# AOADMM-DataFusionFramework/Matlab-Code

Hardware: AMD Instinct MI355X
Metric: AO-ADMM outer iters/sec (+ mode-1 MTTKRP GFLOP/s), 2000^3 rank-20 CP (higher is better)
Workload: dtype f32

## Files before the change

### matlab-code_amd/csrc/contract.h

```cpp
#pragma once
#include "common.h"

namespace aoadmm {

struct DenseTensor {
  int prec = AOADMM_PREC_F64;
  int nd = 0;
  int64_t dims[8] = {0};
  int64_t pad0 = 0;
  DevBuf data;
  int64_t elems_padded() const {
    int64_t n = pad0;
    for (int i = 1; i < nd; ++i) n *= dims[i];
    return n;
  }
  size_t elem_size() const { return prec == AOADMM_PREC_F32 ? 4 : 8; }
};

struct ContractPlan {
  int64_t nbatch, batch_stride, M, ld, C;
  int R;
  int tprec = AOADMM_PREC_F64;
  int nchunk;
  bool lead = false;
  bool on_xp = false;
  bool on_xq = false;
  bool on_xc = false;
  int64_t trows() const { return nbatch * M; }
  size_t t_bytes() const { return (size_t)nchunk * trows() * R * (tprec == AOADMM_PREC_F32 ? 4 : 8); }
  size_t frag_bytes(int prec) const;
  double algorithmic_bytes(int prec) const {
    return (double)nbatch * M * C * (prec == AOADMM_PREC_F32 ? 4.0 : 8.0) + (double)t_bytes();
  }
  double flops() const { return 2.0 * nbatch * M * C * R; }
};

ContractPlan make_plan(int64_t nbatch, int64_t batch_stride, int64_t M, int64_t ld, int64_t C, int R,
                       int prec);

ContractPlan make_lead_plan(int64_t M, int64_t ld, int64_t C, int R);

void launch_contract(const void* X, int prec, const ContractPlan& pl, const double* F, int64_t ldF,
                     void* frag_ws, void* T, hipStream_t s, hipEvent_t ev0 = nullptr,
                     hipEvent_t ev1 = nullptr);

size_t reduce_factor_scratch_bytes(int64_t rows, int R);
struct SysBuild;
bool launch_reduce_inner(const void* T, int tprec, int nchunk, int64_t trows, int64_t A, int64_t Apad,
                         int64_t B, int R, const double* Fa, int64_t ldFa, double scale,
                         double* out, int64_t ldOut, double* ft_scratch, hipStream_t s,
                         const double* FaT = nullptr,
                         int rowmajor_out = 0,
                         const SysBuild* sys = nullptr);
size_t reduce_outer_scratch_bytes(int64_t A, int64_t B, int R);
bool launch_reduce_outer(const void* T, int tprec, int nchunk, int64_t trows, int64_t A, int64_t Apad,
                         int64_t B, int R, const double* Fb, int64_t ldFb, double scale,
                         double* out, int64_t ldOut, double* scratch, double* ft_scratch, hipStream_t s,
                         const double* FbT = nullptr, int rowmajor_out = 0, const SysBuild* sys = nullptr);
void launch_t_to_colmajor(const void* T, int tprec, int nchunk, int64_t trows, int64_t A, int R, double scale,
                          double* out, int64_t ldOut, hipStream_t s);

constexpr int64_t kSmallMttkrpElems = (int64_t)1 << 19;
struct SmallMttkrp {
  const void* X;
  int64_t sn, sa, sb;
  int Na, Nb, R;
  const double *Fa, *Fb;
  int64_t lda, ldb;
  double scale;
  double* out;
  int64_t ldOut;
};
bool small_mttkrp_ok(int64_t elems, int nd, const int64_t* dims, int R);
bool small_mttkrp(const SmallMttkrp& a, int prec, int64_t rows, hipStream_t s, const SysBuild* sys = nullptr);

}
```

### matlab-code_amd/csrc/contract.hip

```cpp
#include "contract.h"
#include "device_utils.h"
#include "small_dev.h"

#include <algorithm>
#include <cstdlib>

namespace aoadmm {

typedef float f32x4 __attribute__((ext_vector_type(4)));
typedef double f64x2 __attribute__((ext_vector_type(2)));
typedef double f64x4 __attribute__((ext_vector_type(4)));

static constexpr int kTileRows = 128;
static constexpr int kGroup = 8;

struct KArgs {
  const void* X;
  const void* frag;
  void* T;
  int64_t tiles_per_batch, ntiles, batch_stride, M, ld, C, Cg, trows;
  int groups_per_chunk, R;
  int flush_every;
};

typedef float f32x2 __attribute__((ext_vector_type(2)));

__global__ void pack_frag16_f32(const double* __restrict__ F, int64_t ldF, int64_t C, int R, int NT, int EX,
                                int64_t Cg, float* __restrict__ frag) {
  const int64_t idx = (int64_t)blockIdx.x * blockDim.x + threadIdx.x;
  const int64_t nmain = (int64_t)NT * Cg * 128;
  if (idx < nmain) {
    const int kk = idx & 1;
    const int lane = (idx >> 1) & 63;
    const int64_t g = (idx >> 7) % Cg;
    const int nt = (int)((idx >> 7) / Cg);
    const int64_t c = 8 * g + 4 * kk + (lane >> 4);
    const int r = 16 * nt + (lane & 15);
    frag[idx] = (c < C && r < R) ? (float)F[c + ldF * r] : 0.f;
  } else if (EX && idx < nmain + Cg * 32) {
    const int64_t j = idx - nmain;
    const int e = j & 3, q = (j >> 2) & 3, kk = (j >> 4) & 1;
    const int64_t g = j >> 5;
    const int64_t c = 8 * g + 4 * kk + q;
    const int r = 16 * NT + e;
    frag[idx] = (c < C && r < R) ? (float)F[c + ldF * r] : 0.f;
  }
}

__device__ __forceinline__ float quarter_sum4(float a, float b, float c, float d) {
  const auto ab = __builtin_amdgcn_permlane16_swap(__float_as_uint(a), __float_as_uint(b), false, false);
  const auto cd = __builtin_amdgcn_permlane16_swap(__float_as_uint(c), __float_as_uint(d), false, false);
  const float s_ab = __uint_as_float(ab[0]) + __uint_as_float(ab[1]);
  const float s_cd = __uint_as_float(cd[0]) + __uint_as_float(cd[1]);
  const auto x = __builtin_amdgcn_permlane32_swap(__float_as_uint(s_ab), __float_as_uint(s_cd), false, false);
  return __uint_as_float(x[0]) + __uint_as_float(x[1]);
}

constexpr int kFlushEvery = 3;
template <int NT, bool EX, bool L2 = false>
__global__ __launch_bounds__(256, NT <= 2 ? 2 : 1) void contract16_f32(KArgs a) {
  static_assert(!L2 || NT == 1, "two-level accumulation exists for one 16-column tile (R <= 20)");
  const int lane = threadIdx.x & 63;
  const int64_t wt = (int64_t)blockIdx.x * 4 + (threadIdx.x >> 6);
  if (wt >= a.ntiles) return;
  const int chunk = blockIdx.y;
  const int64_t b = wt / a.tiles_per_batch;
  const int64_t m0 = (wt - b * a.tiles_per_batch) * kTileRows;
  const int r16 = lane & 15, q = lane >> 4;
  int64_t row0 = m0 + 4 * r16, row1 = m0 + 64 + 4 * r16;
  if (row0 >= a.M) row0 = m0;
  if (row1 >= a.M) row1 = m0;
  const int64_t g0 = (int64_t)chunk * a.groups_per_chunk;
  int64_t g1 = g0 + a.groups_per_chunk;
  if (g1 > a.Cg) g1 = a.Cg;
  const int64_t gfull = (a.C / kGroup < g1) ? a.C / kGroup : g1;
  const float* X = reinterpret_cast<const float*>(a.X) + b * a.batch_stride;
  const float* xp0 = X + row0 + (kGroup * g0 + q) * a.ld;
  const float* xp1 = X + row1 + (kGroup * g0 + q) * a.ld;
  const int64_t ld4 = 4 * a.ld;
  const f32x2* fp = reinterpret_cast<const f32x2*>(a.frag) + g0 * 64 + lane;
  const int64_t fnt = a.Cg * 64;
  const f32x4* fe = reinterpret_cast<const f32x4*>(reinterpret_cast<const f32x2*>(a.frag) + (int64_t)NT * a.Cg * 64) + g0 * 8 + q;

  f32x4 acc[NT][2][4];
  f32x2 accE[2][4][2];
#define AO_PKFMA_LO(ACC, X2, E2) asm("v_pk_fma_f32 %0, %1, %2, %0 op_sel:[0,0,0] op_sel_hi:[0,1,1]" : "+v"(ACC) : "v"(X2), "v"(E2));
#define AO_PKFMA_HI(ACC, X2, E2) asm("v_pk_fma_f32 %0, %1, %2, %0 op_sel:[1,0,0] op_sel_hi:[1,1,1]" : "+v"(ACC) : "v"(X2), "v"(E2));
#pragma unroll
  for (int h = 0; h < 2; ++h)
#pragma unroll
    for (int v = 0; v < 4; ++v) {
      accE[h][v][0] = f32x2{0.f, 0.f};
      accE[h][v][1] = f32x2{0.f, 0.f};
#pragma unroll
      for (int nt = 0; nt < NT; ++nt) acc[nt][h][v] = f32x4{0.f, 0.f, 0.f, 0.f};
    }

  extern __shared__ __attribute__((aligned(16))) float t_lds[];
  double* l2 = reinterpret_cast<double*>(t_lds) + (threadIdx.x >> 6) * 2048 + lane;
  double accE2[2][4];
  if (L2) {
#pragma unroll
    for (int k = 0; k < 32; ++k) l2[k * 64] = 0.0;
#pragma unroll
    for (int h = 0; h < 2; ++h)
#pragma unroll
      for (int v = 0; v < 4; ++v) accE2[h][v] = 0.0;
  }
#define AO_FLUSH()                                                                                   \
  {                                                                                                  \
    _Pragma("unroll") for (int h = 0; h < 2; ++h) {                                                  \
      _Pragma("unroll") for (int vb = 0; vb < 4; vb += 2) {                                          \
        _Pragma("unroll") for (int v = vb; v < vb + 2; ++v)                                          \
          _Pragma("unroll") for (int i = 0; i < 4; ++i) {                                            \
            l2[((h * 4 + v) * 4 + i) * 64] += (double)acc[0][h][v][i];                               \
            acc[0][h][v][i] = 0.f;                                                                   \
          }                                                                                          \
        __builtin_amdgcn_sched_barrier(0);                                                           \
      }                                                                                              \
    }                                                                                                \
    if (EX) {       \
      _Pragma("unroll") for (int h = 0; h < 2; ++h)                                                  \
        _Pragma("unroll") for (int v = 0; v < 4; ++v) {                                              \
          accE2[h][v] += (double)quarter_sum4(accE[h][v][0][0], accE[h][v][0][1], accE[h][v][1][0], accE[h][v][1][1]); \
          accE[h][v][0] = f32x2{0.f, 0.f};                                                           \
          accE[h][v][1] = f32x2{0.f, 0.f};                                                           \
        }                                                                                            \
    }                                                                                                \
  }
  f32x4 x0[4], x1[4], x2[4], e0[2], e1[2], e2[2];
  f32x2 f0[NT], f1[NT], f2[NT];
  const int64_t ng = gfull > g0 ? gfull - g0 : 0;
  const int64_t gstep = kGroup * a.ld;
#define AO_LOAD1(XS, GI, S)                                                                          \
  XS[S] = __builtin_nontemporal_load(reinterpret_cast<const f32x4*>((((S) & 1) ? xp1 : xp0) + (GI) * gstep + ((S) >> 1) * ld4));
#define AO_LOADF(FS, ES, GI)                                                                         \
  {                                                                                                  \
    _Pragma("unroll") for (int nt = 0; nt < NT; ++nt) FS[nt] = fp[(GI) * 64 + nt * fnt];            \
    if (EX) { ES[0] = fe[(GI) * 8]; ES[1] = fe[(GI) * 8 + 4]; }                                      \
  }
#define AO_LOAD_STAGE(XS, FS, ES, GI)                                                                \
  { AO_LOAD1(XS, GI, 0) AO_LOAD1(XS, GI, 1) AO_LOAD1(XS, GI, 2) AO_LOAD1(XS, GI, 3) AO_LOADF(FS, ES, GI) }
#define AO_FMA_S(XS, FS, ES, S)                                                                      \
  {                                                                                                  \
    _Pragma("unroll") for (int v = 0; v < 4; ++v) {                                                  \
      _Pragma("unroll") for (int nt = 0; nt < NT; ++nt)                                              \
        acc[nt][(S) & 1][v] = __builtin_amdgcn_mfma_f32_16x16x4f32(XS[S][v], FS[nt][(S) >> 1], acc[nt][(S) & 1][v], 0, 0, 0); \
    }                                                                                                \
    if (EX) {       \
      const f32x2 xlo_ = __builtin_shufflevector(XS[S], XS[S], 0, 1), xhi_ = __builtin_shufflevector(XS[S], XS[S], 2, 3); \
      const f32x2 ea_ = __builtin_shufflevector(ES[(S) >> 1], ES[(S) >> 1], 0, 1);                   \
      const f32x2 eb_ = __builtin_shufflevector(ES[(S) >> 1], ES[(S) >> 1], 2, 3);                   \
      AO_PKFMA_LO(accE[(S) & 1][0][0], xlo_, ea_) AO_PKFMA_LO(accE[(S) & 1][0][1], xlo_, eb_)        \
      AO_PKFMA_HI(accE[(S) & 1][1][0], xlo_, ea_) AO_PKFMA_HI(accE[(S) & 1][1][1], xlo_, eb_)        \
      AO_PKFMA_LO(accE[(S) & 1][2][0], xhi_, ea_) AO_PKFMA_LO(accE[(S) & 1][2][1], xhi_, eb_)        \
      AO_PKFMA_HI(accE[(S) & 1][3][0], xhi_, ea_) AO_PKFMA_HI(accE[(S) & 1][3][1], xhi_, eb_)        \
    }                                                                                                \
  }
#define AO_COMPUTE_STAGE(XS, FS, ES) { AO_FMA_S(XS, FS, ES, 0) AO_FMA_S(XS, FS, ES, 1) AO_FMA_S(XS, FS, ES, 2) AO_FMA_S(XS, FS, ES, 3) }
#define AO_MIX_STAGE(XC, FC, EC, XL, FL, EL, GI)                                                     \
  {                                                                                                  \
    AO_FMA_S(XC, FC, EC, 0) AO_LOAD1(XL, GI, 0) __builtin_amdgcn_sched_barrier(0);                   \
    AO_FMA_S(XC, FC, EC, 1) AO_LOAD1(XL, GI, 1) __builtin_amdgcn_sched_barrier(0);                   \
    AO_FMA_S(XC, FC, EC, 2) AO_LOAD1(XL, GI, 2) __builtin_amdgcn_sched_barrier(0);                   \
    AO_FMA_S(XC, FC, EC, 3) AO_LOAD1(XL, GI, 3) AO_LOADF(FL, EL, GI) __builtin_amdgcn_sched_barrier(0); \
  }
  if (ng > 0) AO_LOAD_STAGE(x0, f0, e0, 0)
  if (ng > 1) AO_LOAD_STAGE(x1, f1, e1, 1)
  int64_t g = 0;
  int since_flush = 0;
  for (; g + 5 <= ng; g += 3) {
    AO_MIX_STAGE(x0, f0, e0, x2, f2, e2, g + 2)
    AO_MIX_STAGE(x1, f1, e1, x0, f0, e0, g + 3)
    AO_MIX_STAGE(x2, f2, e2, x1, f1, e1, g + 4)
    if (L2 && ++since_flush == a.flush_every) {
      since_flush = 0;
      AO_FLUSH()
    }
  }
  for (; g + 3 <= ng; g += 3) {
    if (g + 2 < ng) AO_LOAD_STAGE(x2, f2, e2, g + 2)
    AO_COMPUTE_STAGE(x0, f0, e0)
    if (g + 3 < ng) AO_LOAD_STAGE(x0, f0, e0, g + 3)
    AO_COMPUTE_STAGE(x1, f1, e1)
    if (g + 4 < ng) AO_LOAD_STAGE(x1, f1, e1, g + 4)
    AO_COMPUTE_STAGE(x2, f2, e2)
  }
  if (g < ng) AO_COMPUTE_STAGE(x0, f0, e0)
  if (g + 1 < ng) AO_COMPUTE_STAGE(x1, f1, e1)
  g = gfull > g0 ? gfull : g0;
  if (g < g1) {
#pragma unroll
    for (int s = 0; s < 4; ++s) {
      int64_t c = kGroup * g + 4 * (s >> 1) + q;
      if (c >= a.C) c = a.C - 1;
      x0[s] = *reinterpret_cast<const f32x4*>(X + ((s & 1) ? row1 : row0) + c * a.ld);
    }
    {
      const f32x2* fpt = reinterpret_cast<const f32x2*>(a.frag) + g * 64 + lane;
#pragma unroll
      for (int nt = 0; nt < NT; ++nt) f0[nt] = fpt[nt * fnt];
      if (EX) {
        const f32x4* fet = reinterpret_cast<const f32x4*>(reinterpret_cast<const f32x2*>(a.frag) + (int64_t)NT * a.Cg * 64) + g * 8 + q;
        e0[0] = fet[0]; e0[1] = fet[4];
      }
    }
    AO_COMPUTE_STAGE(x0, f0, e0)
  }
  if (L2) AO_FLUSH()
#undef AO_FLUSH
#undef AO_PKFMA_LO
#undef AO_PKFMA_HI
#undef AO_LOAD1
#undef AO_LOADF
#undef AO_LOAD_STAGE
#undef AO_FMA_S
#undef AO_COMPUTE_STAGE
#undef AO_MIX_STAGE
  float* tl = L2 ? t_lds + (threadIdx.x >> 6) * 4096 : t_lds + (threadIdx.x >> 6) * (kTileRows * a.R);
  if (L2) {
    double d2[32];
#pragma unroll
    for (int k = 0; k < 32; ++k) d2[k] = l2[k * 64];
    __builtin_amdgcn_sched_barrier(0);
#pragma unroll
    for (int h = 0; h < 2; ++h)
#pragma unroll
      for (int v = 0; v < 4; ++v)
#pragma unroll
        for (int i = 0; i < 4; ++i) acc[0][h][v][i] = (float)d2[(h * 4 + v) * 4 + i];
  }
#pragma unroll
  for (int nt = 0; nt < NT; ++nt) {
    const int r = 16 * nt + r16;
    if (r < a.R) {
#pragma unroll
      for (int h = 0; h < 2; ++h)
#pragma unroll
        for (int v = 0; v < 4; ++v)
#pragma unroll
          for (int i = 0; i < 4; ++i) tl[(64 * h + 4 * (4 * q + i) + v) * a.R + r] = acc[nt][h][v][i];
    }
  }
  if (EX) {
#pragma unroll
    for (int h = 0; h < 2; ++h)
#pragma unroll
      for (int v = 0; v < 4; ++v)
#pragma unroll
        for (int e = 0; e < 4; ++e) {
          if (L2) continue;
          float t = accE[h][v][e >> 1][e & 1];
          t += __shfl_xor(t, 16);
          t += __shfl_xor(t, 32);
          accE[h][v][e >> 1][e & 1] = t;
        }
    const int ne = a.R - 16 * NT;
    if (L2) {
      if (q < ne) {
#pragma unroll
        for (int h = 0; h < 2; ++h)
#pragma unroll
          for (int v = 0; v < 4; ++v) tl[(64 * h + 4 * r16 + v) * a.R + 16 * NT + q] = (float)accE2[h][v];
      }
    } else if (q == 0) {
#pragma unroll
      for (int h = 0; h < 2; ++h)
#pragma unroll
        for (int v = 0; v < 4; ++v)
#pragma unroll
          for (int e = 0; e < 4; ++e)
            if (e < ne) tl[(64 * h + 4 * r16 + v) * a.R + 16 * NT + e] = accE[h][v][e >> 1][e & 1];
    }
  }
  {
    const int64_t rows_here = (a.M - m0 < kTileRows) ? a.M - m0 : kTileRows;
    const int n16 = (int)(rows_here * a.R / 4);
    f32x4* dst = reinterpret_cast<f32x4*>(reinterpret_cast<float*>(a.T) + ((int64_t)chunk * a.trows + b * a.M + m0) * a.R);
    const f32x4* src = reinterpret_cast<const f32x4*>(tl);
    for (int c = lane; c < n16; c += 64) __builtin_nontemporal_store(src[c], dst + c);
  }
}

static constexpr int kLeadRows = 128;
static constexpr int kLeadKC = 64;
static constexpr int kLeadStride = 68;

struct LArgs {
  const float* X;
  const float* frag;
  float* T;
  int64_t M, ld, C, Cg;
  int chunks_per_slice;
  int R;
};

__global__ void pack_frag_lead16_f32(const double* __restrict__ F, int64_t ldF, int64_t C, int R, int NT,
                                     int64_t Cg16, float* __restrict__ frag) {
  const int64_t idx = (int64_t)blockIdx.x * blockDim.x + threadIdx.x;
  const int64_t nmain = (int64_t)NT * Cg16 * 256;
  if (idx < nmain) {
    const int t = idx & 3;
    const int lane = (idx >> 2) & 63;
    const int64_t g = (idx >> 8) % Cg16;
    const int nt = (int)((idx >> 8) / Cg16);
    const int64_t c = 16 * g + 4 * (lane >> 4) + t;
    const int r = 16 * nt + (lane & 15);
    frag[idx] = (c < C && r < R) ? (float)F[c + ldF * r] : 0.f;
  }
}

template <int NT>
__global__ __launch_bounds__(256, NT <= 2 ? 2 : 1) void contract_lead16_f32(LArgs a) {
  extern __shared__ __attribute__((aligned(16))) float lds[];
  const int tid = threadIdx.x, lane = tid & 63, w = tid >> 6;
  const int64_t m0 = (int64_t)blockIdx.x * kLeadRows;
  const int slice = blockIdx.y;
  const int64_t nchunks_total = (a.C + kLeadKC - 1) / kLeadKC;
  const int64_t c0 = (int64_t)slice * a.chunks_per_slice;
  int64_t c1 = c0 + a.chunks_per_slice;
  if (c1 > nchunks_total) c1 = nchunks_total;
  const int64_t Cg16 = (a.C + 15) / 16;
  const int srow = tid >> 4, scol = 4 * (tid & 15);
  const unsigned mlast = (unsigned)((a.M - 1 - m0 < kLeadRows - 1) ? (a.M - 1 - m0) : (kLeadRows - 1));
  const float* xblk = a.X + m0 * a.ld;
  const int64_t last4 = a.ld - 4;
  f32x4 acc[NT][8];
#pragma unroll
  for (int tl = 0; tl < 8; ++tl)
#pragma unroll
    for (int nt = 0; nt < NT; ++nt) acc[nt][tl] = f32x4{0.f, 0.f, 0.f, 0.f};
  const int r16 = lane & 15, q4 = lane >> 4;
  const f32x4* fbase = reinterpret_cast<const f32x4*>(a.frag) + lane;
  const int64_t fnt = (Cg16 + 1) * 64;
  f32x4 sA[8], sB[8];
  f32x4 fA[NT], fB[NT];
#define AO_LEAD_LOAD1(ST, CH, Q)                                                                     \
  {                                                                                                  \
    int64_t i_ = (CH) * kLeadKC + scol;                                                              \
    if (i_ > last4) i_ = last4;                                                                      \
    unsigned mq_ = srow + 16 * (Q);                                                                  \
    if (mq_ > mlast) mq_ = mlast;                                                                    \
    unsigned ldo_ = (unsigned)a.ld;                                                                  \
    asm volatile("" : "+s"(ldo_));                                                                   \
    ST[Q] = __builtin_nontemporal_load(reinterpret_cast<const f32x4*>(xblk + (uint64_t)mq_ * ldo_ + i_)); \
  }
#define AO_LEAD_LOAD(ST, CH) { _Pragma("unroll") for (int q_ = 0; q_ < 8; ++q_) AO_LEAD_LOAD1(ST, CH, q_) }
#define AO_LEAD_WRITE(ST, BUF)                                                                       \
  {                                                                                                  \
    float* base_ = lds + (BUF) * (kLeadRows * kLeadStride);                                          \
    _Pragma("unroll") for (int q_ = 0; q_ < 8; ++q_)                                                 \
      *reinterpret_cast<f32x4*>(base_ + (srow + 16 * q_) * kLeadStride + scol) = ST[q_];             \
  }
#define AO_LEAD_FRAG(FV, CH)                                                                         \
  {                                                                                                  \
    int64_t gg = (CH) * (kLeadKC / 16) + w;                                                          \
    if (gg > Cg16) gg = Cg16;                                           \
    _Pragma("unroll") for (int nt = 0; nt < NT; ++nt) FV[nt] = fbase[nt * fnt + gg * 64];            \
  }
#define AO_LEAD_TILE(XV, TL, FV)                                                                     \
  {                                                                                                  \
    _Pragma("unroll") for (int t = 0; t < 4; ++t)                                                    \
      _Pragma("unroll") for (int nt = 0; nt < NT; ++nt)                                              \
        acc[nt][TL] = __builtin_amdgcn_mfma_f32_16x16x4f32(XV[t], FV[nt][t], acc[nt][TL], 0, 0, 0);  \
  }
#define AO_LEAD_COMPUTE(BUF, CH, FV, FVN, NF, ST, CHN, PF)                                           \
  {                                                                                                  \
    const float* xs_ = lds + (BUF) * (kLeadRows * kLeadStride) + r16 * kLeadStride + 16 * w + 4 * q4; \
    if (NF) AO_LEAD_FRAG(FVN, (CH) + 1)                                                              \
    _Pragma("unroll") for (int hb = 0; hb < 2; ++hb) {                                               \
      f32x4 xv_[4];                                                                                  \
      _Pragma("unroll") for (int j_ = 0; j_ < 4; ++j_)            \
        xv_[j_] = *reinterpret_cast<const f32x4*>(xs_ + 16 * (4 * hb + j_) * kLeadStride);           \
      __builtin_amdgcn_sched_barrier(0);                                                             \
      _Pragma("unroll") for (int j_ = 0; j_ < 4; ++j_) {                                             \
        AO_LEAD_TILE(xv_[j_], 4 * hb + j_, FV)                                                       \
        if (PF) AO_LEAD_LOAD1(ST, CHN, 4 * hb + j_)                                                  \
        __builtin_amdgcn_sched_barrier(0);                                                           \
      }                                                                                              \
    }                                                                                                \
  }
  const int64_t n = c1 > c0 ? c1 - c0 : 0;
  if (n > 0) {
    AO_LEAD_LOAD(sA, c0)
    AO_LEAD_FRAG(fA, c0)
    AO_LEAD_WRITE(sA, 0)
  }
  if (n > 1) AO_LEAD_LOAD(sA, c0 + 1)
  if (n > 2) AO_LEAD_LOAD(sB, c0 + 2)
  __syncthreads();
#pragma nounroll
  for (int64_t k = 0; k < n; k += 2) {
    if (k + 1 < n) AO_LEAD_WRITE(sA, 1)
    if (k + 3 < n) AO_LEAD_COMPUTE(0, c0 + k, fA, fB, true, sA, c0 + k + 3, true)
    else if (k + 1 < n) AO_LEAD_COMPUTE(0, c0 + k, fA, fB, true, sA, c0, false)
    else AO_LEAD_COMPUTE(0, c0 + k, fA, fB, false, sA, c0, false)
    __syncthreads();
    if (k + 1 >= n) break;
    if (k + 2 < n) AO_LEAD_WRITE(sB, 0)
    if (k + 4 < n) AO_LEAD_COMPUTE(1, c0 + k + 1, fB, fA, true, sB, c0 + k + 4, true)
    else if (k + 2 < n) AO_LEAD_COMPUTE(1, c0 + k + 1, fB, fA, true, sB, c0, false)
    else AO_LEAD_COMPUTE(1, c0 + k + 1, fB, fA, false, sB, c0, false)
    __syncthreads();
  }
#undef AO_LEAD_LOAD1
#undef AO_LEAD_LOAD
#undef AO_LEAD_WRITE
#undef AO_LEAD_FRAG
#undef AO_LEAD_TILE
#undef AO_LEAD_COMPUTE
  __syncthreads();
  constexpr int kEpiStride = 17;
  float* Tc = a.T + (int64_t)slice * a.M * a.R + m0 * a.R;
  const int64_t rows_here = (a.M - m0 < kLeadRows) ? (a.M - m0) : kLeadRows;
#pragma unroll
  for (int nt = 0; nt < NT; ++nt) {
    float* reg = lds + w * (kLeadRows * kEpiStride);
#pragma unroll
    for (int tl = 0; tl < 8; ++tl)
#pragma unroll
      for (int i = 0; i < 4; ++i) reg[(16 * tl + 4 * q4 + i) * kEpiStride + r16] = acc[nt][tl][i];
    __syncthreads();
    int ncol = a.R - 16 * nt;
    if (ncol > 16) ncol = 16;
    const int total = (int)rows_here * ncol;
    for (int e = tid; e < total; e += 256) {
      const int row = e / ncol, col = e - row * ncol;
      const float* p = lds + row * kEpiStride + col;
      const float v = (p[0] + p[kLeadRows * kEpiStride]) + (p[2 * kLeadRows * kEpiStride] + p[3 * kLeadRows * kEpiStride]);
      Tc[(int64_t)row * a.R + 16 * nt + col] = v;
    }
    __syncthreads();
  }
// ... 116 lines not shown
    for (; g + 2 <= ng; g += 2) {
      AO_LOAD_STAGE(x1, f1, e1, g + 1)
      AO_COMPUTE_STAGE(x0, f0, e0)
      if (g + 2 < ng) AO_LOAD_STAGE(x0, f0, e0, g + 2)
      AO_COMPUTE_STAGE(x1, f1, e1)
    }
    if (g < ng) AO_COMPUTE_STAGE(x0, f0, e0)
  }
  g = gfull > g0 ? gfull : g0;
  if (g < g1) {
#pragma unroll
    for (int s = 0; s < 4; ++s) {
      int64_t c = kGroup * g + 4 * (s >> 1) + q;
      if (c >= a.C) c = a.C - 1;
      x0[s] = *reinterpret_cast<const f64x2*>(X + ((s & 1) ? row1 : row0) + c * a.ld);
    }
    {
      const f64x2* fpt = reinterpret_cast<const f64x2*>(a.frag) + g * 64 + lane;
#pragma unroll
      for (int nt = 0; nt < NT; ++nt) f0[nt] = fpt[nt * fnt];
      if (EX) {
        const f64x4* fet = reinterpret_cast<const f64x4*>(reinterpret_cast<const f64x2*>(a.frag) + (int64_t)NT * a.Cg * 64) + g * 8 + q;
        e0[0] = fet[0]; e0[1] = fet[4];
      }
    }
    AO_COMPUTE_STAGE(x0, f0, e0)
  }
#undef AO_LOAD1
#undef AO_LOADF
#undef AO_LOAD_STAGE
#undef AO_FMA_S
#undef AO_COMPUTE_STAGE
#undef AO_MIX_STAGE
  extern __shared__ __attribute__((aligned(16))) double t_lds64[];
  double* tl = t_lds64 + (threadIdx.x >> 6) * (kTileRows64 * a.R);
#pragma unroll
  for (int nt = 0; nt < NT; ++nt) {
    const int r = 16 * nt + r2;
    if (r < a.R) {
#pragma unroll
      for (int j = 0; j < 2; ++j)
#pragma unroll
        for (int v = 0; v < 2; ++v)
#pragma unroll
          for (int i = 0; i < 4; ++i) tl[(32 * j + 2 * (q + 4 * i) + v) * a.R + r] = acc[nt][j][v][i];
    }
  }
  if (EX) {
#pragma unroll
    for (int j = 0; j < 2; ++j)
#pragma unroll
      for (int v = 0; v < 2; ++v)
#pragma unroll
        for (int c = 0; c < 4; ++c) {
          double t = accE[j][v][c];
          t += __shfl_xor(t, 16);
          t += __shfl_xor(t, 32);
          accE[j][v][c] = t;
        }
    if (q == 0) {
      const int ne = a.R - 16 * NT;
#pragma unroll
      for (int j = 0; j < 2; ++j)
#pragma unroll
        for (int v = 0; v < 2; ++v)
#pragma unroll
          for (int c = 0; c < 4; ++c)
            if (c < ne) tl[(32 * j + 2 * r2 + v) * a.R + 16 * NT + c] = accE[j][v][c];
    }
  }
  {
    const int64_t rows_here = (a.M - m0 < kTileRows64) ? a.M - m0 : kTileRows64;
    const int n16 = (int)(rows_here * a.R / 2);
    f64x2* dst = reinterpret_cast<f64x2*>(reinterpret_cast<double*>(a.T) + ((int64_t)chunk * a.trows + b * a.M + m0) * a.R);
    const f64x2* src = reinterpret_cast<const f64x2*>(tl);
    for (int c = lane; c < n16; c += 64) __builtin_nontemporal_store(src[c], dst + c);
  }
}

static int nt_of(int R, int prec) {
  const int w = prec == AOADMM_PREC_F32 ? 32 : 16;
  return (R + w - 1) / w;
}
static int tile_rows(int prec) { return prec == AOADMM_PREC_F32 ? kTileRows : kTileRows64; }

size_t ContractPlan::frag_bytes(int prec) const {
  const int64_t Cg = cdiv(C, kGroup);
  return (size_t)(nt_of(R, prec) * 1024 + 1152) * Cg + 8192;
}

ContractPlan make_plan(int64_t nbatch, int64_t batch_stride, int64_t M, int64_t ld, int64_t C, int R,
                       int prec) {
  ContractPlan p;
  p.tprec = prec;
  p.nbatch = nbatch; p.batch_stride = batch_stride; p.M = M; p.ld = ld; p.C = C; p.R = R;
  const int64_t Cg = cdiv(C, kGroup);
  const int64_t ntiles = nbatch * cdiv(M, tile_rows(prec));
  int64_t nchunk = 1;
  if (prec == AOADMM_PREC_F32) nchunk = cdiv(Cg, 256);
  if (ntiles < 2048) {
    int64_t want = cdiv(2048, ntiles);
    int64_t maxc = Cg / 16 > 0 ? Cg / 16 : 1;
    if (want > maxc) want = maxc;
    if (want > nchunk) nchunk = want;
  }
  if (nchunk > 65535) nchunk = 65535;
  p.nchunk = (int)nchunk;
  return p;
}

ContractPlan make_lead_plan(int64_t M, int64_t ld, int64_t C, int R) {
  ContractPlan p;
  p.tprec = AOADMM_PREC_F32;
  p.nbatch = 1; p.batch_stride = 0; p.M = M; p.ld = ld; p.C = C; p.R = R;
  p.lead = true;
  const int64_t nch = cdiv(C, kLeadKC);
  p.nchunk = (int)cdiv(nch, 2048 / kLeadKC);
  return p;
}

static void launch_contract_lead(const void* X, const ContractPlan& pl, const double* F, int64_t ldF, void* frag_ws,
                                 void* T, hipStream_t s, hipEvent_t ev0, hipEvent_t ev1) {
  const int64_t Cg = cdiv(pl.C, kGroup);
  AO_REQUIRE(pl.ld % 4 == 0 && pl.ld >= 4, "f32 layout must be padded to 4");
  LArgs a;
  a.X = (const float*)X; a.frag = (const float*)frag_ws; a.T = (float*)T;
  a.M = pl.M; a.ld = pl.ld; a.C = pl.C; a.Cg = Cg; a.R = pl.R;
  a.chunks_per_slice = (int)cdiv(cdiv(pl.C, kLeadKC), pl.nchunk);
  const int64_t nblk = cdiv(pl.M, kLeadRows);
  AO_REQUIRE(nblk < (int64_t)2147483647, "tensor too large for one launch");
  dim3 grid((unsigned)nblk, (unsigned)pl.nchunk);
  const size_t sh = (size_t)2 * kLeadRows * kLeadStride * sizeof(float);
  const int nt16 = (pl.R + 15) / 16;
  const int64_t Cg16 = cdiv(pl.C, 16) + 1;
  const int64_t total = (int64_t)nt16 * Cg16 * 256;
  pack_frag_lead16_f32<<<(unsigned)cdiv(total, 256), 256, 0, s>>>(F, ldF, pl.C, pl.R, nt16, Cg16, (float*)frag_ws);
  AO_KERNEL_CHECK();
#define AO_SET(K) ensure_dynamic_lds(reinterpret_cast<const void*>(K), (int)sh);
  if (nt16 == 1) AO_SET(contract_lead16_f32<1>)
  else if (nt16 == 2) AO_SET(contract_lead16_f32<2>)
  else if (nt16 == 3) AO_SET(contract_lead16_f32<3>)
  else if (nt16 == 4) AO_SET(contract_lead16_f32<4>)
#undef AO_SET
  if (ev0) AO_HIP(hipEventRecord(ev0, s));
  if (nt16 == 1) contract_lead16_f32<1><<<grid, 256, sh, s>>>(a);
  else if (nt16 == 2) contract_lead16_f32<2><<<grid, 256, sh, s>>>(a);
  else if (nt16 == 3) contract_lead16_f32<3><<<grid, 256, sh, s>>>(a);
  else if (nt16 == 4) contract_lead16_f32<4><<<grid, 256, sh, s>>>(a);
  else throw Error(AOADMM_ERR_UNSUPPORTED, "rank > 64 not supported");
  if (ev1) AO_HIP(hipEventRecord(ev1, s));
  AO_KERNEL_CHECK();
}

void launch_contract(const void* X, int prec, const ContractPlan& pl, const double* F, int64_t ldF,
                     void* frag_ws, void* T, hipStream_t s, hipEvent_t ev0, hipEvent_t ev1) {
  AO_REQUIRE(pl.tprec == prec, "contraction plan and tensor precision disagree");
  AO_REQUIRE(pl.R >= 1 && pl.R <= kMaxRank, "rank %d outside [1,%d]", pl.R, kMaxRank);
  if (pl.lead) {
    AO_REQUIRE(prec == AOADMM_PREC_F32, "leading-mode contraction exists for fp32 tensors only");
    launch_contract_lead(X, pl, F, ldF, frag_ws, T, s, ev0, ev1);
    return;
  }
  const int64_t Cg = cdiv(pl.C, kGroup);
  KArgs a;
  a.X = X; a.frag = frag_ws; a.T = T;
  a.tiles_per_batch = cdiv(pl.M, tile_rows(prec));
  a.ntiles = pl.nbatch * a.tiles_per_batch;
  a.batch_stride = pl.batch_stride; a.M = pl.M; a.ld = pl.ld; a.C = pl.C; a.Cg = Cg;
  a.trows = pl.trows();
  a.groups_per_chunk = (int)cdiv(Cg, pl.nchunk);
  a.R = pl.R;
  AO_REQUIRE(a.ntiles > 0 && pl.C > 0, "empty contraction");
  dim3 grid((unsigned)cdiv(a.ntiles, 4), (unsigned)pl.nchunk);
  AO_REQUIRE(cdiv(a.ntiles, 4) < (int64_t)2147483647, "tensor too large for one launch");
  if (prec == AOADMM_PREC_F32) {
    AO_REQUIRE(pl.ld % 4 == 0 && pl.M % 4 == 0 && pl.batch_stride % 4 == 0, "f32 layout must be padded to 4");
    const int rem = pl.R % 16;
    const bool ex = pl.R > 16 && rem >= 1 && rem <= 4;
    const int nt16 = ex ? pl.R / 16 : (pl.R + 15) / 16;
    const int64_t total = (int64_t)nt16 * Cg * 128 + (ex ? Cg * 32 : 0);
    pack_frag16_f32<<<(unsigned)cdiv(total, 256), 256, 0, s>>>(F, ldF, pl.C, pl.R, nt16, ex ? 1 : 0, Cg, (float*)frag_ws);
    AO_KERNEL_CHECK();
    size_t tsh = (size_t)4 * kTileRows * pl.R * sizeof(float);
    a.flush_every = kFlushEvery;
    if (nt16 == 1) tsh = (size_t)4 * 16384;
#define AO_GO(K) { if (tsh > 65536) ensure_dynamic_lds(reinterpret_cast<const void*>(K), (int)tsh); if (ev0) AO_HIP(hipEventRecord(ev0, s)); K<<<grid, 256, tsh, s>>>(a); }
    if (nt16 == 1 && !ex) AO_GO((contract16_f32<1, false, true>))
    else if (nt16 == 1) AO_GO((contract16_f32<1, true, true>))
    else if (nt16 == 2 && !ex) AO_GO((contract16_f32<2, false>))
    else if (nt16 == 2) AO_GO((contract16_f32<2, true>))
    else if (nt16 == 3 && !ex) AO_GO((contract16_f32<3, false>))
    else if (nt16 == 3) AO_GO((contract16_f32<3, true>))
    else if (nt16 == 4) AO_GO((contract16_f32<4, false>))
    else throw Error(AOADMM_ERR_UNSUPPORTED, "rank > 64 not supported");
#undef AO_GO
  } else {
    AO_REQUIRE(pl.ld % 2 == 0 && pl.M % 2 == 0 && pl.batch_stride % 2 == 0, "f64 layout must be padded to 2");
    const int rem = pl.R % 16;
    const bool ex = pl.R > 16 && rem >= 1 && rem <= 4;
    const int nt16 = ex ? pl.R / 16 : (pl.R + 15) / 16;
    const int64_t total = (int64_t)nt16 * Cg * 128 + (ex ? Cg * 32 : 0);
    pack_frag_f64<<<(unsigned)cdiv(total, 256), 256, 0, s>>>(F, ldF, pl.C, pl.R, nt16, ex ? 1 : 0, Cg, (double*)frag_ws);
    AO_KERNEL_CHECK();
    const size_t tsh = (size_t)4 * kTileRows64 * pl.R * sizeof(double);
#define AO_GO(K) { if (tsh > 65536) ensure_dynamic_lds(reinterpret_cast<const void*>(K), (int)tsh); if (ev0) AO_HIP(hipEventRecord(ev0, s)); K<<<grid, 256, tsh, s>>>(a); }
    if (nt16 == 1 && !ex) AO_GO((contract_f64<1, false>))
    else if (nt16 == 1) AO_GO((contract_f64<1, true>))
    else if (nt16 == 2 && !ex) AO_GO((contract_f64<2, false>))
    else if (nt16 == 2) AO_GO((contract_f64<2, true>))
    else if (nt16 == 3 && !ex) AO_GO((contract_f64<3, false>))
    else if (nt16 == 3) AO_GO((contract_f64<3, true>))
    else if (nt16 == 4) AO_GO((contract_f64<4, false>))
    else throw Error(AOADMM_ERR_UNSUPPORTED, "rank > 64 not supported");
#undef AO_GO
  }
  if (ev1) AO_HIP(hipEventRecord(ev1, s));
  AO_KERNEL_CHECK();
}

__global__ void factor_rowmajor_k(const double* __restrict__ F, int64_t ldF, int64_t rows, int R,
                                  double* __restrict__ Ft) {
  const int64_t idx = (int64_t)blockIdx.x * blockDim.x + threadIdx.x;
  if (idx >= rows * R) return;
  const int r = (int)(idx / rows);
  const int64_t a = idx - (int64_t)r * rows;
  Ft[a * R + r] = F[a + ldF * r];
}
static void factor_rowmajor(const double* F, int64_t ldF, int64_t rows, int R, double* Ft, hipStream_t s) {
  factor_rowmajor_k<<<(unsigned)cdiv(rows * R, 256), 256, 0, s>>>(F, ldF, rows, R, Ft);
  AO_KERNEL_CHECK();
}

template <typename TT, int VEC> struct TVec;
template <> struct TVec<float, 4> { typedef float type __attribute__((ext_vector_type(4))); };
template <> struct TVec<float, 1> { typedef float type; };
template <> struct TVec<double, 2> { typedef double type __attribute__((ext_vector_type(2))); };
template <> struct TVec<double, 1> { typedef double type; };
template <typename TT, int VEC>
__device__ __forceinline__ void fma_vec(double (&acc)[VEC], const TT* __restrict__ tp, const double* __restrict__ fp) {
  typedef typename TVec<TT, VEC>::type V;
  const V tv = __builtin_nontemporal_load(reinterpret_cast<const V*>(tp));
  if constexpr (VEC == 1) {
    acc[0] += (double)tv * fp[0];
  } else {
#pragma unroll
    for (int v = 0; v < VEC; ++v) acc[v] += (double)tv[v] * fp[v];
  }
}

template <typename TT, int VEC>
struct RVec {
  typename TVec<TT, VEC>::type t;
  double f[VEC];
  __device__ __forceinline__ void load(const TT* __restrict__ tp, const double* __restrict__ fp) {
    t = __builtin_nontemporal_load(reinterpret_cast<const typename TVec<TT, VEC>::type*>(tp));
#pragma unroll
    for (int v = 0; v < VEC; ++v) f[v] = fp[v];
  }
  __device__ __forceinline__ void fma(double (&acc)[VEC]) const {
    if constexpr (VEC == 1) {
      acc[0] += (double)t * f[0];
    } else {
#pragma unroll
      for (int v = 0; v < VEC; ++v) acc[v] += (double)t[v] * f[v];
    }
  }
};

template <typename TT, int VEC>
__global__ void reduce_inner_k(const TT* __restrict__ T, int nchunk, int64_t trows, int64_t A, int64_t Apad, int R,
                               const double* __restrict__ FaT, double scale, double* __restrict__ out,
                               int64_t ldOut, int rowmajor, int has_sys, SysBuild sys) {
  extern __shared__ double sh[];
  if (has_sys && blockIdx.x == 0) { sys_build_rider(sys); return; }
  const int64_t b = (int64_t)blockIdx.x - has_sys;
  const int t = threadIdx.x;
  const int64_t n = A * R, step = (int64_t)blockDim.x * VEC;
  double s0[VEC], s1[VEC], s2[VEC], s3[VEC];
#pragma unroll
  for (int v = 0; v < VEC; ++v) { s0[v] = 0; s1[v] = 0; s2[v] = 0; s3[v] = 0; }
  for (int ch = 0; ch < nchunk; ++ch) {
    const TT* Tb = T + ((int64_t)ch * trows + Apad * b) * R;
    int64_t e = (int64_t)t * VEC;
    for (; e + 3 * step < n; e += 4 * step) {
      RVec<TT, VEC> q0, q1, q2, q3;
      q0.load(Tb + e, FaT + e);
      q1.load(Tb + e + step, FaT + e + step);
      q2.load(Tb + e + 2 * step, FaT + e + 2 * step);
      q3.load(Tb + e + 3 * step, FaT + e + 3 * step);
      __builtin_amdgcn_sched_barrier(0);
      q0.fma(s0); q1.fma(s1); q2.fma(s2); q3.fma(s3);
    }
    for (; e < n; e += step) fma_vec<TT, VEC>(s0, Tb + e, FaT + e);
  }
#pragma unroll
  for (int v = 0; v < VEC; ++v) sh[t * VEC + v] = (s0[v] + s1[v]) + (s2[v] + s3[v]);
  __syncthreads();
  if (t < R) {
    const int nA = blockDim.x * VEC / R;
    double tot = 0.0;
    for (int i = 0; i < nA; ++i) tot += sh[i * R + t];
    if (rowmajor) out[b * R + t] = scale * tot;
    else out[b + ldOut * t] = scale * tot;
  }
}

template <typename TT, int VEC>
__global__ void reduce_inner2_k(const TT* __restrict__ T, int nchunk, int64_t trows, int64_t A, int64_t Apad, int64_t B,
                                int R, const double* __restrict__ FaT, double scale, double* __restrict__ out,
                                int64_t ldOut, int rowmajor, int has_sys, SysBuild sys) {
  extern __shared__ double sh[];
  if (has_sys && blockIdx.x == 0) { sys_build_rider(sys); return; }
  const int64_t b0 = 2 * ((int64_t)blockIdx.x - has_sys);
  const bool two = b0 + 1 < B;
  const int64_t b1 = two ? b0 + 1 : b0;
  const int t = threadIdx.x;
  const int64_t n = A * R, step = (int64_t)blockDim.x * VEC;
  double a0[VEC], a1[VEC], c0[VEC], c1[VEC];
#pragma unroll
  for (int v = 0; v < VEC; ++v) { a0[v] = 0; a1[v] = 0; c0[v] = 0; c1[v] = 0; }
  for (int ch = 0; ch < nchunk; ++ch) {
    const TT* Ta = T + ((int64_t)ch * trows + Apad * b0) * R;
    const TT* Tc = T + ((int64_t)ch * trows + Apad * b1) * R;
    int64_t e = (int64_t)t * VEC;
    for (; e + step < n; e += 2 * step) {
      RVec<TT, VEC> q0, q1, p0, p1;
      q0.load(Ta + e, FaT + e);
      q1.load(Ta + e + step, FaT + e + step);
      p0.t = __builtin_nontemporal_load(reinterpret_cast<const typename TVec<TT, VEC>::type*>(Tc + e));
      p1.t = __builtin_nontemporal_load(reinterpret_cast<const typename TVec<TT, VEC>::type*>(Tc + e + step));
      __builtin_amdgcn_sched_barrier(0);
#pragma unroll
      for (int v = 0; v < VEC; ++v) { p0.f[v] = q0.f[v]; p1.f[v] = q1.f[v]; }
      q0.fma(a0); q1.fma(a1); p0.fma(c0); p1.fma(c1);
    }
    for (; e < n; e += step) {
      RVec<TT, VEC> q0, p0;
      q0.load(Ta + e, FaT + e);
      p0.t = __builtin_nontemporal_load(reinterpret_cast<const typename TVec<TT, VEC>::type*>(Tc + e));
#pragma unroll
      for (int v = 0; v < VEC; ++v) p0.f[v] = q0.f[v];
      q0.fma(a0); p0.fma(c0);
    }
  }
  const int nt = blockDim.x * VEC;
#pragma unroll
  for (int v = 0; v < VEC; ++v) { sh[t * VEC + v] = a0[v] + a1[v]; sh[nt + t * VEC + v] = c0[v] + c1[v]; }
  __syncthreads();
  if (t < 2 * R) {
    const int which = t / R, r = t % R;
    if (which == 0 || two) {
      const int nA = nt / R;
      double tot = 0.0;
      for (int i = 0; i < nA; ++i) tot += sh[which * nt + i * R + r];
      const int64_t b = which ? b1 : b0;
      if (rowmajor) out[b * R + r] = scale * tot;
      else out[b + ldOut * r] = scale * tot;
    }
  }
}

size_t reduce_factor_scratch_bytes(int64_t rows, int R) { return (size_t)rows * R * sizeof(double); }

template <typename TT, int VEC>
static void launch_inner_t(const void* T, int nchunk, int64_t trows, int64_t A, int64_t Apad, int64_t B, int R,
                           const double* FaT, double scale, double* out, int64_t ldOut, hipStream_t s, int rowmajor,
                           const SysBuild* sys) {
  const int hs = sys ? 1 : 0;
  const SysBuild sb = sys ? *sys : SysBuild();
  const int rq = R / VEC;
  int threads = 256 / rq * rq;
  if (threads < rq) threads = rq;
  if (threads * VEC < R) threads = (R + VEC - 1) / VEC;
  if (B >= 1024 && 2 * R <= threads) {
    reduce_inner2_k<TT, VEC><<<(unsigned)((B + 1) / 2 + hs), threads, (size_t)2 * threads * VEC * sizeof(double), s>>>(
        (const TT*)T, nchunk, trows, A, Apad, B, R, FaT, scale, out, ldOut, rowmajor, hs, sb);
    return;
  }
  reduce_inner_k<TT, VEC><<<(unsigned)(B + hs), threads, (size_t)threads * VEC * sizeof(double), s>>>(
      (const TT*)T, nchunk, trows, A, Apad, R, FaT, scale, out, ldOut, rowmajor, hs, sb);
}
// ... 4 lines not shown

bool launch_reduce_inner(const void* T, int tprec, int nchunk, int64_t trows, int64_t A, int64_t Apad,
                         int64_t B, int R, const double* Fa, int64_t ldFa, double scale,
                         double* out, int64_t ldOut, double* ft_scratch, hipStream_t s, const double* FaT,
                         int rowmajor_out, const SysBuild* sys) {
  AO_REQUIRE((int64_t)B < 2147483647ll, "reduce_inner: too many output rows for one launch");
  {
    const int vec = tprec == AOADMM_PREC_F32 ? (R % 4 == 0 ? 4 : 1) : (R % 2 == 0 ? 2 : 1);
    const int rq = R / vec;
    int threads = 256 / rq * rq;
    if (threads < rq) threads = rq;
    if (threads * vec < R) threads = (R + vec - 1) / vec;
    if (!sys_can_ride(sys, threads)) sys = nullptr;
  }
  if (FaT) ft_scratch = const_cast<double*>(FaT);
  else factor_rowmajor(Fa, ldFa, A, R, ft_scratch, s);
  if (tprec == AOADMM_PREC_F32) {
    if (R % 4 == 0) launch_inner_t<float, 4>(T, nchunk, trows, A, Apad, B, R, ft_scratch, scale, out, ldOut, s, rowmajor_out, sys);
    else launch_inner_t<float, 1>(T, nchunk, trows, A, Apad, B, R, ft_scratch, scale, out, ldOut, s, rowmajor_out, sys);
  } else {
    if (R % 2 == 0) launch_inner_t<double, 2>(T, nchunk, trows, A, Apad, B, R, ft_scratch, scale, out, ldOut, s, rowmajor_out, sys);
    else launch_inner_t<double, 1>(T, nchunk, trows, A, Apad, B, R, ft_scratch, scale, out, ldOut, s, rowmajor_out, sys);
  }
  AO_KERNEL_CHECK();
  return sys != nullptr;
}

static void outer_geometry(int64_t A, int64_t B, int R, int vec, int& TA, int64_t& nblkA, int& SB) {
  const int rq = (R + vec - 1) / vec;
  TA = 256 / rq;
  if (TA < 1) TA = 1;
  nblkA = cdiv(A, TA);
  int64_t sb = cdiv(2048, nblkA);
  if (sb > 64) sb = 64;
  if (sb > B) sb = B;
  if (sb < 1) sb = 1;
  SB = (int)sb;
}
static int outer_vec(int tprec, int R) {
  if (tprec == AOADMM_PREC_F32) return R % 4 == 0 ? 4 : 1;
  return R % 2 == 0 ? 2 : 1;
}

size_t reduce_outer_scratch_bytes(int64_t A, int64_t B, int R) {
  size_t worst = 0;
  for (int vec : {1, 2, 4}) {
    int TA, SB; int64_t nb;
    outer_geometry(A, B, R, vec, TA, nb, SB);
    worst = std::max(worst, (size_t)SB * A * R * sizeof(double));
  }
  return worst;
}

template <typename TT, int VEC>
__global__ void reduce_outer_k(const TT* __restrict__ T, int nchunk, int64_t trows, int64_t A,
                               int64_t Apad, int64_t B, int R, int TA, const double* __restrict__ FbT,
                               double* __restrict__ part, int has_sys, SysBuild sys) {
  if (has_sys && blockIdx.x == 0) {
    if (blockIdx.y == 0) sys_build_rider(sys);
    return;
  }
  const int t = threadIdx.x;
  const int rq = R / VEC;
  const int al = t / rq, r = (t - al * rq) * VEC;
  const int64_t a = ((int64_t)blockIdx.x - has_sys) * TA + al;
  const int SB = gridDim.y, sb = blockIdx.y;
  const int64_t bper = (B + SB - 1) / SB;
  const int64_t b0 = sb * bper;
  int64_t b1 = b0 + bper;
  if (b1 > B) b1 = B;
  if (al >= TA || a >= A) return;
  const int64_t bs = Apad * R;
  double s0[VEC], s1[VEC], s2[VEC], s3[VEC];
#pragma unroll
  for (int v = 0; v < VEC; ++v) { s0[v] = 0; s1[v] = 0; s2[v] = 0; s3[v] = 0; }
  for (int ch = 0; ch < nchunk; ++ch) {
    const TT* Tc = T + (int64_t)ch * trows * R + a * R + r;
    const double* Fr = FbT + r;
    int64_t b = b0;
    for (; b + 3 < b1; b += 4) {
      RVec<TT, VEC> q0, q1, q2, q3;
      q0.load(Tc + bs * b, Fr + b * R);
      q1.load(Tc + bs * (b + 1), Fr + (b + 1) * R);
      q2.load(Tc + bs * (b + 2), Fr + (b + 2) * R);
      q3.load(Tc + bs * (b + 3), Fr + (b + 3) * R);
      __builtin_amdgcn_sched_barrier(0);
      q0.fma(s0); q1.fma(s1); q2.fma(s2); q3.fma(s3);
    }
    for (; b < b1; ++b) fma_vec<TT, VEC>(s0, Tc + bs * b, Fr + b * R);
  }
#pragma unroll
  for (int v = 0; v < VEC; ++v) part[((int64_t)sb * A + a) * R + r + v] = (s0[v] + s1[v]) + (s2[v] + s3[v]);
}

__global__ void reduce_outer_fin(const double* __restrict__ part, int SB, int64_t A, int R, double scale,
                                 double* __restrict__ out, int64_t ldOut, int rowmajor) {
  int64_t idx = (int64_t)blockIdx.x * blockDim.x + threadIdx.x;
  if (idx >= A * R) return;
  const int64_t a = idx / R;
  const int r = (int)(idx - a * R);
  double t0 = 0.0, t1 = 0.0;
  int s = 0;
  const int64_t ar = A * R;
  for (; s + 7 < SB; s += 8) {
    const double v0 = part[(int64_t)s * ar + idx], v1 = part[(int64_t)(s + 1) * ar + idx];
    const double v2 = part[(int64_t)(s + 2) * ar + idx], v3 = part[(int64_t)(s + 3) * ar + idx];
    const double v4 = part[(int64_t)(s + 4) * ar + idx], v5 = part[(int64_t)(s + 5) * ar + idx];
    const double v6 = part[(int64_t)(s + 6) * ar + idx], v7 = part[(int64_t)(s + 7) * ar + idx];
    t0 += v0; t1 += v1; t0 += v2; t1 += v3; t0 += v4; t1 += v5; t0 += v6; t1 += v7;
  }
  for (; s + 1 < SB; s += 2) {
    t0 += part[(int64_t)s * ar + idx];
    t1 += part[(int64_t)(s + 1) * ar + idx];
  }
  if (s < SB) t0 += part[(int64_t)s * ar + idx];
  if (rowmajor) out[idx] = scale * (t0 + t1);
  else out[a + ldOut * r] = scale * (t0 + t1);
}

template <typename TT, int VEC>
static void launch_outer_t(const void* T, int nchunk, int64_t trows, int64_t A, int64_t Apad, int64_t B, int R,
                           const double* FbT, double* scratch, int& SB, hipStream_t s, const SysBuild* sys) {
  int TA; int64_t nb;
  outer_geometry(A, B, R, VEC, TA, nb, SB);
  int threads = TA * (R / VEC);
  threads = (threads + 63) / 64 * 64;
  const int hs = sys ? 1 : 0;
  reduce_outer_k<TT, VEC><<<dim3((unsigned)(nb + hs), (unsigned)SB), threads, 0, s>>>((const TT*)T, nchunk, trows, A, Apad, B,
                                                                                    R, TA, FbT, scratch, hs, sys ? *sys : SysBuild());
}

bool launch_reduce_outer(const void* T, int tprec, int nchunk, int64_t trows, int64_t A, int64_t Apad,
                         int64_t B, int R, const double* Fb, int64_t ldFb, double scale,
                         double* out, int64_t ldOut, double* scratch, double* ft_scratch, hipStream_t s,
                         const double* FbT, int rowmajor_out, const SysBuild* sys) {
  if (!sys_can_ride(sys)) sys = nullptr;
  if (FbT) ft_scratch = const_cast<double*>(FbT);
  else factor_rowmajor(Fb, ldFb, B, R, ft_scratch, s);
  int SB = 1;
  const int vec = outer_vec(tprec, R);
  if (tprec == AOADMM_PREC_F32) {
    if (vec == 4) launch_outer_t<float, 4>(T, nchunk, trows, A, Apad, B, R, ft_scratch, scratch, SB, s, sys);
    else launch_outer_t<float, 1>(T, nchunk, trows, A, Apad, B, R, ft_scratch, scratch, SB, s, sys);
  } else {
    if (vec == 2) launch_outer_t<double, 2>(T, nchunk, trows, A, Apad, B, R, ft_scratch, scratch, SB, s, sys);
    else launch_outer_t<double, 1>(T, nchunk, trows, A, Apad, B, R, ft_scratch, scratch, SB, s, sys);
  }
  AO_KERNEL_CHECK();
  reduce_outer_fin<<<(unsigned)cdiv(A * R, 256), 256, 0, s>>>(scratch, SB, A, R, scale, out, ldOut, rowmajor_out);
  AO_KERNEL_CHECK();
  return sys != nullptr;
}

template <typename TT, int RMAX>
__global__ __launch_bounds__(256) void small_mttkrp_k(SmallMttkrp a, int has_sys, SysBuild sys) {
  extern __shared__ double sf[];
  if (has_sys && blockIdx.x == 0) { sys_build_rider(sys); return; }
  const int row = (int)blockIdx.x - has_sys;
  const int R = a.R, Na = a.Na, Nb = a.Nb;
  double* fa = sf;
  double* fb = sf + (size_t)Na * R;
  double* red = fb + (size_t)(Nb > 0 ? Nb : 1) * R;
  for (int e = threadIdx.x; e < Na * R; e += 256) { const int i = e / R, r = e - i * R; fa[e] = a.Fa[i + a.lda * r]; }
  for (int e = threadIdx.x; e < Nb * R; e += 256) { const int i = e / R, r = e - i * R; fb[e] = a.Fb ? a.Fb[i + a.ldb * r] : 1.0; }
  __syncthreads();
  const TT* X = reinterpret_cast<const TT*>(a.X) + (int64_t)row * a.sn;
  double acc[RMAX];
#pragma unroll
  for (int r = 0; r < RMAX; ++r) acc[r] = 0.0;
  const int npairs = Na * Nb;
  for (int p = threadIdx.x; p < npairs; p += 256) {
    const int ia = p % Na, ib = p / Na;
    const double x = (double)X[(int64_t)ia * a.sa + (int64_t)ib * a.sb];
#pragma unroll
    for (int r = 0; r < RMAX; ++r)
      if (r < R) acc[r] += x * (fa[ia * R + r] * fb[ib * R + r]);
  }
  const int lane = threadIdx.x & 63, w = threadIdx.x >> 6;
#pragma unroll
  for (int r = 0; r < RMAX; ++r) {
    const double v = wave_sum(acc[r]);
    if (lane == 0) red[w * RMAX + r] = v;
  }
  __syncthreads();
  if ((int)threadIdx.x < R) {
    const int r = threadIdx.x;
    const double tot = (red[r] + red[RMAX + r]) + (red[2 * RMAX + r] + red[3 * RMAX + r]);
    a.out[row + a.ldOut * r] = a.scale * tot;
  }
}

bool small_mttkrp_ok(int64_t elems, int nd, const int64_t* dims, int R) {
  const bool off = getenv("AOADMM_NO_SMALL_MTTKRP") != nullptr;
  if (off || elems > kSmallMttkrpElems || !(nd == 2 || nd == 3) || R > 16) return false;
  int64_t sum = 0;
  for (int i = 0; i < nd; ++i) sum += dims[i];
  return (size_t)(sum * R + 64) * sizeof(double) <= 40 * 1024;
}

bool small_mttkrp(const SmallMttkrp& a, int prec, int64_t rows, hipStream_t s, const SysBuild* sys) {
  if (!sys_can_ride(sys)) sys = nullptr;
  const int hs = sys ? 1 : 0;
  const SysBuild sb = sys ? *sys : SysBuild();
  AO_REQUIRE(a.R >= 1 && a.R <= 16 && rows >= 1 && a.Na >= 1 && a.Nb >= 1, "small_mttkrp: bad sizes");
  const int rmax = a.R <= 4 ? 4 : (a.R <= 8 ? 8 : 16);
  const size_t lds = ((size_t)(a.Na + a.Nb) * a.R + 4 * rmax) * sizeof(double);
  AO_REQUIRE(lds <= 48 * 1024, "small_mttkrp: factors do not fit LDS");
#define AO_SM(TT, RM) small_mttkrp_k<TT, RM><<<(unsigned)(rows + hs), 256, lds, s>>>(a, hs, sb)
  if (prec == AOADMM_PREC_F32) { if (rmax == 4) AO_SM(float, 4); else if (rmax == 8) AO_SM(float, 8); else AO_SM(float, 16); }
  else { if (rmax == 4) AO_SM(double, 4); else if (rmax == 8) AO_SM(double, 8); else AO_SM(double, 16); }
#undef AO_SM
  AO_KERNEL_CHECK();
  return sys != nullptr;
}

template <typename TT>
__global__ void t_to_colmajor_k(const TT* __restrict__ T, int nchunk, int64_t trows, int64_t A, int R,
                                double scale, double* __restrict__ out, int64_t ldOut) {
  int64_t idx = (int64_t)blockIdx.x * blockDim.x + threadIdx.x;
  if (idx >= A * R) return;
  const int64_t a = idx / R;
  const int r = (int)(idx - a * R);
  double tot = 0.0;
  for (int ch = 0; ch < nchunk; ++ch) tot += (double)T[(int64_t)ch * trows * R + idx];
  out[a + ldOut * r] = scale * tot;
}

void launch_t_to_colmajor(const void* T, int tprec, int nchunk, int64_t trows, int64_t A, int R, double scale,
                          double* out, int64_t ldOut, hipStream_t s) {
  const unsigned nb = (unsigned)cdiv(A * R, 256);
  if (tprec == AOADMM_PREC_F32) t_to_colmajor_k<float><<<nb, 256, 0, s>>>((const float*)T, nchunk, trows, A, R, scale, out, ldOut);
  else t_to_colmajor_k<double><<<nb, 256, 0, s>>>((const double*)T, nchunk, trows, A, R, scale, out, ldOut);
  AO_KERNEL_CHECK();
}

}
```

### matlab-code_amd/csrc/misc.hip

```cpp
#include "misc.h"

#include <map>
#include <mutex>
#include <utility>

namespace aoadmm {

void ensure_dynamic_lds(const void* kernel, int bytes) {
  static std::mutex mu;
  static std::map<std::pair<int, const void*>, int> granted;
  int dev = 0;
  AO_HIP(hipGetDevice(&dev));
  std::lock_guard<std::mutex> lk(mu);
  int& have = granted[std::make_pair(dev, kernel)];
  if (have >= bytes) return;
  AO_HIP(hipFuncSetAttribute(kernel, hipFuncAttributeMaxDynamicSharedMemorySize, bytes));
  have = bytes;
}


template <typename T>
__global__ void pad_convert_k(T* dst, int64_t pad_rows, const double* src, int64_t rows, int64_t cols,
                              int64_t dst_col0) {
  const int64_t total = pad_rows * cols;
// ... 74 lines not shown
  const double t = block_reduce256(acc, sh);
  if (threadIdx.x == 0) ws[blockIdx.x] = t;
}
__global__ void sum_ws_k(double* slot, const double* ws, int nb, int stride, int nout) {
  if ((int)threadIdx.x < nout) {
    double t = 0.0;
    for (int b = 0; b < nb; ++b) t += ws[(int64_t)b * stride + threadIdx.x];
    slot[threadIdx.x] = t;
  }
}
void tensor_sumsq(double* slot, const void* X, int prec, int64_t n, double* ws, hipStream_t s) {
  if (prec == AOADMM_PREC_F32) tensor_sumsq_k<float><<<kNormBlocks, 256, 0, s>>>(ws, (const float*)X, n);
  else tensor_sumsq_k<double><<<kNormBlocks, 256, 0, s>>>(ws, (const double*)X, n);
  AO_KERNEL_CHECK();
  sum_ws_k<<<1, 64, 0, s>>>(slot, ws, kNormBlocks, 1, 1);
  AO_KERNEL_CHECK();
}

__device__ __forceinline__ uint64_t mix64(uint64_t z) {
  z += 0x9E3779B97F4A7C15ull;
  z = (z ^ (z >> 30)) * 0xBF58476D1CE4E5B9ull;
  z = (z ^ (z >> 27)) * 0x94D049BB133111EBull;
  return z ^ (z >> 31);
}
__device__ __forceinline__ double u01(uint64_t seed, uint64_t stream, uint64_t idx) {
  const uint64_t h = mix64(mix64(seed ^ (stream * 0xD1B54A32D192ED03ull)) + idx);
  return (double)(h >> 11) * (1.0 / 9007199254740992.0);
}
__device__ __forceinline__ double gauss01(uint64_t seed, uint64_t idx) {
  const double u1 = 1.0 - u01(seed, 101, idx);
  const double u2 = u01(seed, 102, idx);
  return sqrt(-2.0 * log(u1)) * cospi(2.0 * u2);
}

__global__ void fill_uniform_k(double* x, int64_t n, uint64_t seed, uint64_t stream) {
  for (int64_t i = (int64_t)blockIdx.x * blockDim.x + threadIdx.x; i < n; i += (int64_t)gridDim.x * blockDim.x)
    x[i] = u01(seed, stream, (uint64_t)i);
}
void synth_factors(double* A, double* B, double* C, const SynthArgs& a, hipStream_t s) {
  fill_uniform_k<<<256, 256, 0, s>>>(A, a.I_full * a.R, a.seed, 1);
  fill_uniform_k<<<256, 256, 0, s>>>(B, a.J * a.R, a.seed, 2);
  fill_uniform_k<<<256, 256, 0, s>>>(C, a.K * a.R, a.seed, 3);
  AO_KERNEL_CHECK();
}

static constexpr int kSynthBlocks = 4096;
size_t synth_ws_bytes() { return (size_t)kSynthBlocks * 3 * sizeof(double); }

template <int PASS, typename T>
__global__ void synth_k(T* X, double* ws, const double* A, const double* B, const double* C, SynthArgs a,
                        double sigma, double inv_norm) {
  __shared__ double bc[kMaxRank];
  __shared__ double sh[256];
  double s_cc = 0, s_nn = 0, s_cn = 0;
  const int64_t Kl = a.K_loc < 0 ? a.K : a.K_loc;
  const int64_t ncol = a.J * Kl;
  for (int64_t lcol = blockIdx.x; lcol < ncol; lcol += gridDim.x) {
    const int64_t j = lcol % a.J, k = lcol / a.J + a.k0;
    const int64_t col = j + a.J * k;
    __syncthreads();
    if ((int)threadIdx.x < a.R) bc[threadIdx.x] = B[j + a.J * threadIdx.x] * C[k + a.K * threadIdx.x];
    __syncthreads();
    for (int64_t i = threadIdx.x; i < a.I_pad; i += blockDim.x) {
      double clean = 0.0, nz = 0.0;
      if (i < a.I_loc) {
        const int64_t ig = i + a.row0;
        for (int r = 0; r < a.R; ++r) clean += A[ig + a.I_full * r] * bc[r];
        nz = gauss01(a.seed, (uint64_t)(ig + a.I_full * col));
      }
      if (PASS == 1) {
        s_cc += clean * clean; s_nn += nz * nz; s_cn += clean * nz;
      } else {
        X[i + a.I_pad * lcol] = (T)((clean + sigma * nz) * inv_norm);
      }
    }
  }
  if (PASS == 1) {
    const double t0 = block_reduce256(s_cc, sh);
    const double t1 = block_reduce256(s_nn, sh);
    const double t2 = block_reduce256(s_cn, sh);
    if (threadIdx.x == 0) {
      ws[(int64_t)blockIdx.x * 3 + 0] = t0;
      ws[(int64_t)blockIdx.x * 3 + 1] = t1;
      ws[(int64_t)blockIdx.x * 3 + 2] = t2;
    }
  }
}
void synth_norms(double* out3, const double* A, const double* B, const double* C, const SynthArgs& a,
                 double* ws, hipStream_t s) {
  synth_k<1, double><<<kSynthBlocks, 256, 0, s>>>(nullptr, ws, A, B, C, a, 0.0, 1.0);
  AO_KERNEL_CHECK();
  sum_ws_k<<<1, 64, 0, s>>>(out3, ws, kSynthBlocks, 3, 3);
  AO_KERNEL_CHECK();
}
void synth_write(void* X, int prec, const double* A, const double* B, const double* C, const SynthArgs& a,
                  double sigma, double inv_norm, hipStream_t s) {
  if (prec == AOADMM_PREC_F32)
    synth_k<2, float><<<kSynthBlocks * 4, 256, 0, s>>>((float*)X, nullptr, A, B, C, a, sigma, inv_norm);
  else
    synth_k<2, double><<<kSynthBlocks * 4, 256, 0, s>>>((double*)X, nullptr, A, B, C, a, sigma, inv_norm);
  AO_KERNEL_CHECK();
}

__global__ __launch_bounds__(1024) void reg_value_k(double* slot, int type, double eta, const double* X, int64_t rows, int R) {
  __shared__ double sh[1024];
  double acc = 0.0;
  const int64_t n = rows * R;
  if (type == AOADMM_C_L2_REG) {
    double tot = 0.0;
    for (int r = 0; r < R; ++r) {
      double a = 0.0;
      for (int64_t i = threadIdx.x; i < rows; i += blockDim.x) { const double v = X[i + rows * r]; a += v * v; }
      tot += sqrt(block_reduce_n(a, sh));
    }
    if (threadIdx.x == 0) slot[0] = eta * tot;
    return;
  }
  for (int64_t e = threadIdx.x; e < n; e += blockDim.x) {
    const double v = X[e];
    const int64_t i = e % rows;
    switch (type) {
      case AOADMM_C_L1_REG: acc += fabs(v); break;
      case AOADMM_C_L0_REG: acc += (v != 0.0) ? 1.0 : 0.0; break;
      case AOADMM_C_RIDGE: acc += v * v; break;
      case AOADMM_C_TV: if (i + 1 < rows) acc += X[e + 1] - v; break;
      case AOADMM_C_GL_SMOOTH: if (i + 1 < rows) { const double d = X[e + 1] - v; acc += d * d; } break;
      default: break;
    }
  }
  const double t = block_reduce_n(acc, sh);
  if (threadIdx.x == 0) slot[0] = eta * t;
}
void reg_value(double* slot, int type, double p0, const double* X, int64_t rows, int R, double* ws,
               hipStream_t s) {
  (void)ws;
  reg_value_k<<<1, 1024, 0, s>>>(slot, type, p0, X, rows, R);
  AO_KERNEL_CHECK();
}

template <typename T>
__global__ __launch_bounds__(256) void block_copy_k(const T* __restrict__ X, T* __restrict__ D, int64_t M, int64_t Mpad,
                                                   int64_t K, int64_t MB) {
  const int64_t k = blockIdx.y;
  constexpr int V = 16 / sizeof(T);
  typedef T VT __attribute__((ext_vector_type(V)));
  for (int64_t m = ((int64_t)blockIdx.x * 256 + threadIdx.x) * V; m < Mpad; m += (int64_t)gridDim.x * 256 * V) {
    VT v;
#pragma unroll
    for (int e = 0; e < V; ++e) v[e] = (T)0;
    if (m < M) v = *reinterpret_cast<const VT*>(X + M * k + m);
    *reinterpret_cast<VT*>(D + (m / MB) * MB * K + k * MB + m % MB) = v;
  }
}
template <typename T, int WHICH>
__global__ __launch_bounds__(256) void block_permute_k(const T* __restrict__ X, T* __restrict__ D, int64_t I, int64_t Ip,
                                                      int64_t J, int64_t K, int64_t Tp, int64_t MB) {
  __shared__ T tile[32][33];
  const int64_t u = blockIdx.z;
  const int64_t i0 = (int64_t)blockIdx.x * 32, t0 = (int64_t)blockIdx.y * 32;
  const int tx = threadIdx.x & 31, ty = threadIdx.x >> 5;
  const int64_t nT = WHICH == 1 ? J : K;
  const int64_t st = WHICH == 1 ? Ip : Ip * J, su = WHICH == 1 ? Ip * J : Ip;
#pragma unroll
  for (int q = 0; q < 4; ++q) {
    const int64_t i = i0 + tx, t = t0 + ty + 8 * q;
    tile[ty + 8 * q][tx] = (i < I && t < nT) ? X[i + st * t + su * u] : (T)0;
  }
  __syncthreads();
  const int64_t C = WHICH == 1 ? I : J;
#pragma unroll
  for (int q = 0; q < 4; ++q) {
    const int64_t t = t0 + tx, i = i0 + ty + 8 * q;
    if (t < Tp && i < I) {
      const int64_t m = WHICH == 1 ? t + Tp * u : t + Tp * i;
      const int64_t c = WHICH == 1 ? i : u;
      D[(m / MB) * MB * C + c * MB + m % MB] = tile[tx][ty + 8 * q];
    }
  }
}
bool block_layout_copy(const void* X, void* D, int which, int prec, int64_t I, int64_t Ip, int64_t J, int64_t K,
                       int64_t Tp, hipStream_t s) {
  const int64_t MB = kRowBlockElems;
  const size_t es = prec == AOADMM_PREC_F32 ? 4 : 8;
  if (which == 0) {
    if (K > 65535) return false;
    const int64_t M = Ip * J, Mpad = round_up(M, MB);
    const int V = (int)(16 / es);
    int64_t gx = cdiv(Mpad, (int64_t)256 * V);
    if (gx > 65535) gx = 65535;
    const dim3 grid((unsigned)gx, (unsigned)K);
    if (prec == AOADMM_PREC_F32) block_copy_k<float><<<grid, 256, 0, s>>>((const float*)X, (float*)D, M, Mpad, K, MB);
    else block_copy_k<double><<<grid, 256, 0, s>>>((const double*)X, (double*)D, M, Mpad, K, MB);
    AO_KERNEL_CHECK();
    return true;
  }
  const int64_t nU = which == 1 ? K : J, C = which == 1 ? I : J;
  const int64_t M = which == 1 ? Tp * K : Tp * I, Mpad = round_up(M, MB);
  if (nU > 65535 || cdiv(Tp, 32) > 65535) return false;
  if (Mpad > M)
    AO_HIP(hipMemsetAsync((char*)D + (size_t)(Mpad / MB - 1) * MB * C * es, 0, (size_t)MB * C * es, s));
  const dim3 grid((unsigned)cdiv(I, 32), (unsigned)cdiv(Tp, 32), (unsigned)nU);
#define AO_BP(TT, W) block_permute_k<TT, W><<<grid, 256, 0, s>>>((const TT*)X, (TT*)D, I, Ip, J, K, Tp, MB)
  if (prec == AOADMM_PREC_F32) { if (which == 1) AO_BP(float, 1); else AO_BP(float, 2); }
  else { if (which == 1) AO_BP(double, 1); else AO_BP(double, 2); }
#undef AO_BP
  AO_KERNEL_CHECK();
  return true;
}

template <typename T>
__global__ __launch_bounds__(256) void unfold_gram_k(UnfoldGramArgs a, double* ws) {
  __shared__ double As[16][65], Bs[16][65];
  const T* X = reinterpret_cast<const T*>(a.X);
  const int tid = threadIdx.x, tx = tid & 15, ty = tid >> 4;
  const int64_t a0 = (int64_t)blockIdx.x * 64, b0 = (int64_t)blockIdx.y * 64;
  const int64_t nch1 = (a.n1 + 15) / 16, nchunks = nch1 * a.n2;
  const int64_t per = (nchunks + gridDim.z - 1) / gridDim.z;
  const int64_t c_lo = (int64_t)blockIdx.z * per;
  int64_t c_hi = c_lo + per;
  if (c_hi > nchunks) c_hi = nchunks;
  double acc[4][4];
#pragma unroll
  for (int i = 0; i < 4; ++i)
#pragma unroll
    for (int j = 0; j < 4; ++j) acc[i][j] = 0.0;
  const bool row_contig = a.sa == 1;
  for (int64_t c = c_lo; c < c_hi; ++c) {
    const int64_t t2 = c / nch1, t1_0 = (c - t2 * nch1) * 16;
    const int64_t base = t2 * a.s2;
#pragma unroll
    for (int q = 0; q < 4; ++q) {
      int aa, tt;
      if (row_contig) { aa = tid & 63; tt = (tid >> 6) + 4 * q; }
      else { tt = tid & 15; aa = (tid >> 4) + 16 * q; }
      const int64_t t1 = t1_0 + tt;
      const bool tv = t1 < a.n1;
      const int64_t off = base + (tv ? t1 : 0) * a.s1;
      const int64_t ra = a0 + aa, rb = b0 + aa;
      As[tt][aa] = (tv && ra < a.n) ? (double)X[ra * a.sa + off] : 0.0;
      Bs[tt][aa] = (tv && rb < a.n) ? (double)X[rb * a.sa + off] : 0.0;
    }
    __syncthreads();
#pragma unroll
    for (int tt = 0; tt < 16; ++tt) {
      double av[4], bv[4];
#pragma unroll
      for (int i = 0; i < 4; ++i) { av[i] = As[tt][ty * 4 + i]; bv[i] = Bs[tt][tx * 4 + i]; }
#pragma unroll
      for (int i = 0; i < 4; ++i)
#pragma unroll
        for (int j = 0; j < 4; ++j) acc[i][j] += av[i] * bv[j];
    }
    __syncthreads();
  }
  double* W = ws + (int64_t)blockIdx.z * a.n * a.n;
#pragma unroll
  for (int i = 0; i < 4; ++i)
#pragma unroll
    for (int j = 0; j < 4; ++j) {
      const int64_t ra = a0 + ty * 4 + i, rb = b0 + tx * 4 + j;
      if (ra < a.n && rb < a.n) W[ra + a.n * rb] = acc[i][j];
    }
}
__global__ void unfold_gram_sum_k(const double* ws, int64_t nn, int nz, double* out) {
  const int64_t e = (int64_t)blockIdx.x * blockDim.x + threadIdx.x;
  if (e >= nn) return;
  double t = 0.0;
  for (int z = 0; z < nz; ++z) t += ws[(int64_t)z * nn + e];
  out[e] = t;
}
static int unfold_gram_splits(const UnfoldGramArgs& a) {
  const int64_t tiles = cdiv(a.n, 64) * cdiv(a.n, 64);
  const int64_t nchunks = cdiv(a.n1, 16) * a.n2;
  int64_t z = cdiv(2048, tiles);
  if (z > nchunks) z = nchunks;
  if (z > 1024) z = 1024;
  while (z > 1 && z * a.n * a.n * 8 > (int64_t)(1ll << 30)) z /= 2;
  return (int)(z < 1 ? 1 : z);
}
size_t unfold_gram_ws_bytes(const UnfoldGramArgs& a) { return (size_t)unfold_gram_splits(a) * a.n * a.n * sizeof(double); }
void unfold_gram(const UnfoldGramArgs& a, int prec, double* ws, double* out, hipStream_t s) {
  AO_REQUIRE(a.n > 0 && a.n1 > 0 && a.n2 > 0, "unfold_gram: bad sizes");
  AO_REQUIRE(cdiv(a.n, 64) <= 65535, "unfold_gram: mode too long");
  const int nz = unfold_gram_splits(a);
  const dim3 grid((unsigned)cdiv(a.n, 64), (unsigned)cdiv(a.n, 64), (unsigned)nz);
  if (prec == AOADMM_PREC_F32) unfold_gram_k<float><<<grid, 256, 0, s>>>(a, ws);
  else unfold_gram_k<double><<<grid, 256, 0, s>>>(a, ws);
  AO_KERNEL_CHECK();
  unfold_gram_sum_k<<<(unsigned)cdiv(a.n * a.n, 256), 256, 0, s>>>(ws, a.n * a.n, nz, out);
  AO_KERNEL_CHECK();
}

__global__ void kr_merge_k(double* out, const double* Fa, int64_t lda, int64_t A, const double* Fb, int64_t ldb, int64_t B,
                           int R) {
  const int64_t n = A * B * R;
  for (int64_t e = (int64_t)blockIdx.x * blockDim.x + threadIdx.x; e < n; e += (int64_t)gridDim.x * blockDim.x) {
    const int64_t ab = e % (A * B);
    const int r = (int)(e / (A * B));
    out[e] = Fa[ab % A + lda * r] * Fb[ab / A + ldb * r];
  }
}
void kr_merge(double* out, const double* Fa, int64_t lda, int64_t A, const double* Fb, int64_t ldb, int64_t B, int R,
              hipStream_t s) {
  int64_t nb = cdiv(A * B * R, 256);
  if (nb > 4096) nb = 4096;
  kr_merge_k<<<(unsigned)nb, 256, 0, s>>>(out, Fa, lda, A, Fb, ldb, B, R);
  AO_KERNEL_CHECK();
}

}
```

### matlab-code_amd/csrc/solver.h

```cpp
#pragma once
#include <atomic>
#include <memory>
#include <mutex>
#include <vector>

#include "admm.h"
#include "common.h"
#include "contract.h"
#include "misc.h"
#include "par2.h"
#include "small.h"
#include "sparse.h"

typedef struct ncclComm* ncclComm_t;

namespace aoadmm {

struct FactorRef {
  const double* p;
  int64_t ld;
  uint64_t version;
  const double* pT = nullptr;
};

struct CpBlock {
  DenseTensor X;
  DenseTensor Xt;
  DevBuf Xp;
  DevBuf emkr, emkr2;
  int64_t Jp = 0;
  bool has_xp = false, xp_refused = false;
  bool xp_ksharded = false;
  int64_t xp_k0 = 0, xp_kloc = 0;
  DevBuf Xq;
  int64_t Kp = 0;
  bool has_xq = false, xq_refused = false;
  DevBuf Xc;
  bool has_xc = false, xc_refused = false;
  int nd = 0;
  int64_t dims[8] = {0};
  int64_t full0 = 0;
  int64_t row0 = 0;
  bool has_data = false;
  bool x_released = false;
  int cached_mode = -1;
  uint64_t cached_version = 0;
  ContractPlan plan;
  DevBuf T, frag, scratch, ft, tmpA, tmpB;
  DevBuf own[2];
  size_t own_bytes[2] = {0, 0};
  int64_t own_row0[2] = {-1, -1};
  DevBuf mask, maskT;
  bool has_mask = false;
  bool sparse = false;
  CooBlock coo;
};

struct ModeInfo {
  bool defined = false;
  int64_t rows = 0;
  int R = 0;
  bool slabs = false;
  int K = 0;
  std::vector<int64_t> rows_k, off_k;
  int tensor = -1, pos = -1;
  int coupling = -1;
  bool constrained = false;
  ProxSpec prox;
  DevBuf H, H2, Ht, H2t;
  DevBuf HHt;
  DevBuf eU, eUt, eLam;
  DevBuf eV, eMu;
  std::vector<double> H_host;
  int64_t img_rows = 0, img_cols = 0;
  QuadPrep quad;
  int64_t hr = 0, hc = 0, h2r = 0, h2c = 0;
  double ridge = 0.0;
  DevBuf fac, Z, mu, muD;
  DevBuf facT;
  uint64_t facT_version = 0;
  bool has_fac = false, has_Z = false, has_mu = false, has_muD = false;
  int64_t muD_rows = 0, muD_cols = 0;
  uint64_t version = 1;
  DevBuf A, Ab, gram, C, Bsys, L, Binv, rho, Zold, V, Znew, part, proxws, RHS, TD, TF, tmp, W1, W2;
  const double* Aeff = nullptr;
};

struct Par2Block {
  int K = 0, I = 0, R = 0;
  std::vector<int64_t> off_h;
  DevBuf off_d;
  int64_t Jtot = 0;
  int Jmax = 0;
  DevBuf X;
  DevBuf mask;
  bool has_mask = false;
  std::vector<char> have_slab;
  DevBuf DeltaB, DeltaBold, P, Pold, muDB;
  bool has_DeltaB = false;
  std::vector<char> have_P, have_mu;
  DevBuf W, T1, GB, Ak, Lk, rhok, part, norms, res, q, regv, Csys, ac, Lc, rhoc, rhomax;
  DevBuf Jrot;
  bool slab_sharded = false;
  int k0 = 0, k1 = 0;
  DevBuf psum;
  DevBuf rhosum, HtH, Mbig, Minv, Hs;
  bool have_HtH = false, hth_diag = false;
  P2Dims dims() const {
    P2Dims d;
    d.K = K; d.I = I; d.R = R; d.off = off_d.as<int64_t>(); d.off_h = off_h.data(); d.Jtot = Jtot; d.Jmax = Jmax;
    d.k0 = slab_sharded ? k0 : 0; d.k1 = slab_sharded ? k1 : K;
    return d;
  }
  P2Dims dims_all() const {
    P2Dims d = dims();
    d.k0 = 0; d.k1 = K;
    return d;
  }
};

struct TensorInfo {
  bool defined = false;
  bool par2 = false;
  Par2Block p2;
  int nmodes = 0;
  int modes[8] = {0};
  double weight = 1.0;
  CpBlock blk;
  double normsq = 0.0;
  bool normsq_valid = false;
  int last_pos = -1;
  bool eval_shortcut = false;
};

struct CouplingInfo {
  int type = -1;
  std::vector<int> modes;
  DevBuf Delta, DeltaOld, BB, AA, LAA, dD, tmp, coef, rho_ptrs;
  std::vector<const double*> rho_ptrs_host;
  int64_t rows = 0, cols = 0;
  bool has_state = false;
};

struct KernelStats {
  std::vector<std::pair<hipEvent_t, hipEvent_t>> pending;
  double ms = 0.0, bytes = 0.0, flops = 0.0;
  int64_t launches = 0, timed = 0;
};

struct LocalGroup;

class Engine {
 public:
  explicit Engine(int device);
  ~Engine();

  void model_begin(int n_modes, int n_tensors, int n_couplings);
  void set_mode(int mode, int64_t rows, int rank);
  void set_mode_slabs(int mode, int K, const int64_t* rows_k, int rank);
  void add_cp(int p, int n, const int* modes, double weight);
  void add_par2(int p, const int* modes3, double weight);
  void set_constraint(int mode, int type, const double* params, int np, const double* Lmat);
  void set_coupling(int mode, int coupling, const double* H, int64_t hr, int64_t hc, const double* H2,
                    int64_t h2r, int64_t h2c);
  void set_coupling_type(int coupling, int type);
  void set_ridge(const double* ridge);
  void model_end();

  void tensor_upload(int p, const double* data, int prec, int64_t row0, int64_t local_rows);
  void tensor_upload_coo(int p, int64_t nnz, const int64_t* subs, const double* vals);
  void tensor_synth(int p, int rank, uint64_t seed, double noise, int prec);
  void par2_slab_upload(int p, int k, const double* Xk);
  void tensor_mask_upload(int p, const uint8_t* mask);
  void par2_slab_mask_upload(int p, int k, const uint8_t* mask);
  double tensor_normsq(int p);

  void state_set(int field, int index, int slab, const double* host, int64_t rows, int64_t cols);
  void state_get(int field, int index, int slab, double* host, int64_t rows, int64_t cols);

  void solve(const aoadmm_options& opt, aoadmm_result* out);
  void resident_mttkrp(int p, int pos, double* out_host, float* ms);
  void resident_unfold_gram(int p, int pos, int slab, double* out_host);
  void kernel_stats(int which, int reset, double* ms, int64_t* launches, double* bytes, double* flops);

  void comm_init(const char id[128], int rank, int world, bool share_only = false);
  void comm_init_local(int key, int rank, int world);
  void comm_abort();
  void comm_info(int* nccl_version, int* comm_ranks, char* lib_path, int cap) const;
  void set_progress(aoadmm_progress_fn fn, void* user, int every) { progress_fn_ = fn; progress_user_ = user; progress_every_ = every; }
  void par2_gather_slabs(TensorInfo& t);
  bool sharded() const { return world_ > 1 || comm_ != nullptr || local_ != nullptr; }
  void require_usable() const;
  bool share_only() const { return share_only_; }
  bool small_direct(const CpBlock& b, int R) const { return !sharded() && small_mttkrp_ok(b.X.elems_padded(), b.nd, b.dims, R); }
  int rank() const { return rank_; }
  int world() const { return world_; }

  hipStream_t stream() const { return stream_; }
  int device() const { return device_; }

  void ensure_contraction(CpBlock& b, int pos, const FactorRef* facs, int R, bool use_cache, const int* update_seq,
                          int nseq);
  bool ensure_permuted_copy(CpBlock& b);
  bool ensure_permuted_copy2(CpBlock& b);
  bool ensure_blocked_copy(CpBlock& b);
  void adopt_ksharded_xp(CpBlock& b, const void* slab, int64_t k0, int64_t kloc);
  bool want_ksharded_xp(const CpBlock& b, int64_t K, int64_t* k0, int64_t* kloc) const;
  void drop_permuted_copies(CpBlock& b);
  void maybe_release_natural(TensorInfo& t);
  bool prefetch_next_contraction(const aoadmm_options& opt);
  void block_mttkrp(CpBlock& b, int pos, const FactorRef* facs, int R, double scale, double* out,
                    int64_t ldOut, bool use_cache, const int* update_seq, int nseq, bool collective = true,
                    bool tensor_pass = false, const SysBuild* sys = nullptr, bool* sys_done = nullptr);
  void block_upload(CpBlock& b, int nd, const int64_t* dims, const double* host, int prec, int64_t row0,
                    int64_t local_rows, const double* full_array = nullptr);
  void allreduce(double* buf, int64_t n);
  void allreduce_from(const double* send, double* recv, int64_t n);
  double* scratch_slots() { return slots_.d(); }
  double* red_ws() { return redws_.d(); }

 private:
  void check_mode(int m) const;
  void compute_gram(ModeInfo& mi, const LoopEnd* close = nullptr);
  FactorRef factor_ref(const ModeInfo& o) const {
    return FactorRef{o.fac.d(), o.rows, o.version, o.facT_version == o.version ? o.facT.d() : nullptr};
  }
  void update_uncoupled_cp_mode(int m, const aoadmm_options& opt);
  void prepare_mode_system(int m, int nrho, const aoadmm_options& opt);
  void coupled_admm(int c, const aoadmm_options& opt);
  void eval_objective_enqueue(bool first);
  bool has_missing() const;
  void em_pass_enqueue(int p, int update, bool fuse_next_pass = false);
  void prepare_next_first_mode(const aoadmm_options& opt);
  double* em_slot(int p) const;
  void ensure_mode_work(ModeInfo& mi);
  void par2_ensure_work(TensorInfo& t);
  void par2_prepare_modeA(int m, int nrho, const aoadmm_options& opt);
  void par2_update_B(int m, const aoadmm_options& opt, int iter);
  void par2_update_C(int m, const aoadmm_options& opt);
  void par2_prepare_C_coupled(int m, int ctype, const aoadmm_options& opt);
  void par2_objective_enqueue(TensorInfo& t);
  double* resid_slots(int m);
  std::vector<int> update_sequence(int p) const;

  int device_ = 0;
  hipStream_t stream_ = nullptr;
  hipStream_t side_ = nullptr;
  hipEvent_t side_ev_ = nullptr;
  int n_modes_ = 0, n_tensors_ = 0, n_couplings_ = 0;
  bool model_done_ = false;
  bool has_ridge_ = false;
  std::vector<ModeInfo> modes_;
  std::vector<TensorInfo> tensors_;
  std::vector<CouplingInfo> couplings_;
  DevBuf readback_;
  DevBuf ctls_;
  DevBuf slots_;
  DevBuf redws_;
  DevBuf ones_;
  DevBuf emws_;
  bool allow_xp_ = true;
  DevBuf atbws_;
  DevBuf staging_;
  std::vector<hipEvent_t> event_pool_;
  hipEvent_t take_event();
  void fold_finished(KernelStats& ks);
  KernelStats kstats_[4];
  int prepared_mode_ = -1;
  bool profile_ = true;
  bool profile_reductions_ = false;
  ncclComm_t comm_ = nullptr;
  mutable std::mutex comm_mu_;
  std::atomic<bool> aborted_{false};
  std::shared_ptr<LocalGroup> local_;
  int rank_ = 0, world_ = 1;
  bool share_only_ = false;
  aoadmm_progress_fn progress_fn_ = nullptr;
  void* progress_user_ = nullptr;
  int progress_every_ = 0;

  AdmmCtl* ctl_of_mode(int m) { return ctls_.as<AdmmCtl>() + m; }
  AdmmCtl* ctl_of_coupling(int c) { return ctls_.as<AdmmCtl>() + n_modes_ + c; }
  void sparse_mttkrp(CpBlock& b, int pos, const FactorRef* facs, int R, double scale, double* out, int64_t ldOut);
  void timed_contract(const void* X, int prec, const ContractPlan& pl, const double* F, int64_t ldF,
                      void* frag, void* T);
};

}
```

### matlab-code_amd/csrc/solver.hip

```cpp
#include "solver.h"
#include "device_utils.h"
#include "em.h"
#include "hosteig.h"
#include "prox_dev.h"

#include <rccl/rccl.h>
#include <dlfcn.h>

#include <algorithm>
#include <chrono>
#include <cmath>
#include <cstdlib>
#include <condition_variable>
#include <cstring>
#include <map>
#include <mutex>
#include <set>

namespace aoadmm {

#define AO_NCCL(expr)                                                                          \
  do {                                                                                         \
    ncclResult_t r__ = (expr);                                                                 \
    if (r__ != ncclSuccess)                                                                    \
      throw Error(AOADMM_ERR_RCCL, fmt("%s failed: %s", #expr, ncclGetErrorString(r__)));      \
  } while (0)

static constexpr int kSlotsPerMode = 8;
static constexpr int kResidPerMode = 8;

Engine::Engine(int device) : device_(device) {
  int n = 0;
  hipError_t e = hipGetDeviceCount(&n);
  if (e != hipSuccess || n <= 0)
    throw Error(AOADMM_ERR_HIP, "no HIP device available: this library has no CPU fallback");
  if (device < 0 || device >= n) throw Error(AOADMM_ERR_INVALID, fmt("device %d out of range [0,%d)", device, n));
  AO_HIP(hipSetDevice(device));
  AO_HIP(hipStreamCreateWithFlags(&stream_, hipStreamNonBlocking));
  AO_HIP(hipStreamCreateWithFlags(&side_, hipStreamNonBlocking));
  AO_HIP(hipEventCreateWithFlags(&side_ev_, hipEventDisableTiming));
  redws_.alloc(4096 * sizeof(double));
  ones_.alloc(sizeof(double));
  const double one = 1.0;
  AO_HIP(hipMemcpy(ones_.p, &one, sizeof one, hipMemcpyHostToDevice));
}

Engine::~Engine() {
  (void)hipSetDevice(device_);
  for (auto& ks : kstats_)
    for (auto& pr : ks.pending) { (void)hipEventDestroy(pr.first); (void)hipEventDestroy(pr.second); }
  for (hipEvent_t e : event_pool_) (void)hipEventDestroy(e);
  if (comm_) (void)ncclCommDestroy(comm_);
  if (side_ev_) (void)hipEventDestroy(side_ev_);
  if (side_) (void)hipStreamDestroy(side_);
  if (stream_) (void)hipStreamDestroy(stream_);
}

void Engine::comm_init(const char id[128], int rank, int world, bool share_only) {
  AO_REQUIRE(world >= 1 && rank >= 0 && rank < world, "bad rank/world %d/%d", rank, world);
  AO_REQUIRE(id != nullptr || world == 1, "a communicator of %d ranks needs the id from aoadmm_comm_unique_id", world);
  AO_HIP(hipSetDevice(device_));
  if (comm_) { (void)ncclCommDestroy(comm_); comm_ = nullptr; }
  local_.reset();
  if (id != nullptr) {
    ncclUniqueId uid;
    static_assert(sizeof(uid) <= 128, "unique id larger than the ABI buffer");
    std::memcpy(&uid, id, sizeof(uid));
    if (share_only) AO_NCCL(ncclCommInitRank(&comm_, 1, uid, 0));
    else AO_NCCL(ncclCommInitRank(&comm_, world, uid, rank));
  }
  rank_ = rank;
  world_ = world;
  share_only_ = share_only;
  aborted_ = false;
}

struct LocalGroup {
  std::mutex m;
  std::condition_variable cv;
  int world = 0, arrived = 0, joined = 0;
  uint64_t gen = 0;
  bool aborted = false;
  std::vector<std::vector<double>> stage;
  void barrier() {
    std::unique_lock<std::mutex> lk(m);
    if (aborted) throw Error(AOADMM_ERR_RCCL, "local group: aborted after a failure on another rank");
    const uint64_t g = gen;
    if (++arrived == world) {
      arrived = 0;
      ++gen;
      cv.notify_all();
      return;
    }
    if (!cv.wait_for(lk, std::chrono::seconds(120), [&] { return gen != g || aborted; }))
      throw Error(AOADMM_ERR_RCCL, "local group: a rank did not reach the collective within 120 s");
    if (gen == g) throw Error(AOADMM_ERR_RCCL, "local group: aborted after a failure on another rank");
  }
  void abort() {
    std::lock_guard<std::mutex> lk(m);
    aborted = true;
    cv.notify_all();
  }
};
static std::mutex g_groups_mutex;
static std::map<int, std::shared_ptr<LocalGroup>> g_groups;

void Engine::comm_init_local(int key, int rank, int world) {
  AO_REQUIRE(world >= 1 && rank >= 0 && rank < world, "bad rank/world %d/%d", rank, world);
  if (comm_) { (void)ncclCommDestroy(comm_); comm_ = nullptr; }
  std::lock_guard<std::mutex> lk(g_groups_mutex);
  std::shared_ptr<LocalGroup>& g = g_groups[key];
  if (!g || g->joined == g->world) {
    g = std::make_shared<LocalGroup>();
    g->world = world;
    g->stage.resize(world);
  }
  AO_REQUIRE(g->world == world, "local group %d was created for %d ranks, not %d", key, g->world, world);
  g->joined++;
  local_ = g;
  rank_ = rank;
  world_ = world;
  aborted_ = false;
}

void Engine::comm_abort() {
  aborted_ = true;
  if (local_) local_->abort();
  ncclComm_t c = nullptr;
  {
    std::lock_guard<std::mutex> lk(comm_mu_);
    c = comm_;
    comm_ = nullptr;
  }
  if (c) (void)ncclCommAbort(c);
}

void Engine::require_usable() const {
  if (aborted_) throw Error(AOADMM_ERR_RCCL, "context unusable: its communicator was aborted after a failure on another rank");
}

void Engine::comm_info(int* nccl_version, int* comm_ranks, char* lib_path, int cap) const {
  if (nccl_version) {
    int v = 0;
    AO_NCCL(ncclGetVersion(&v));
    *nccl_version = v;
  }
  if (comm_ranks) {
    int n = local_ ? world_ : 0;
    std::lock_guard<std::mutex> lk(comm_mu_);
    if (comm_) AO_NCCL(ncclCommCount(comm_, &n));
    *comm_ranks = n;
  }
  if (lib_path && cap > 0) {
    lib_path[0] = 0;
    Dl_info di;
    if (dladdr(reinterpret_cast<const void*>(&ncclGetVersion), &di) && di.dli_fname) {
      std::strncpy(lib_path, di.dli_fname, (size_t)cap - 1);
      lib_path[cap - 1] = 0;
    }
  }
}

void Engine::allreduce(double* buf, int64_t n) { allreduce_from(buf, buf, n); }

void Engine::allreduce_from(const double* send, double* buf, int64_t n) {
  if (n <= 0) return;
  if (aborted_) throw Error(AOADMM_ERR_RCCL, "communicator aborted after a failure on another rank");
  if (local_) {
    LocalGroup& g = *local_;
    std::vector<double>& mine = g.stage[rank_];
    mine.resize((size_t)n);
    AO_HIP(hipMemcpyAsync(mine.data(), send, (size_t)n * sizeof(double), hipMemcpyDeviceToHost, stream_));
    AO_HIP(hipStreamSynchronize(stream_));
    g.barrier();
    std::vector<double> tot((size_t)n, 0.0);
    for (int r = 0; r < g.world; ++r) {
      AO_REQUIRE((int64_t)g.stage[r].size() == n, "local group: rank %d brought %lld values, rank %d brought %lld", r,
                 (long long)g.stage[r].size(), rank_, (long long)n);
      for (int64_t i = 0; i < n; ++i) tot[i] += g.stage[r][i];
    }
    g.barrier();
    AO_HIP(hipMemcpyAsync(buf, tot.data(), (size_t)n * sizeof(double), hipMemcpyHostToDevice, stream_));
    AO_HIP(hipStreamSynchronize(stream_));
    return;
  }
  ncclComm_t c = nullptr;
  {
    std::lock_guard<std::mutex> lk(comm_mu_);
    if (aborted_) throw Error(AOADMM_ERR_RCCL, "communicator aborted after a failure on another rank");
    c = comm_;
  }
  if (!c) {
    if (world_ > 1) throw Error(AOADMM_ERR_RCCL, fmt("rank %d of %d has no communicator", rank_, world_));
    if (send != buf) AO_HIP(hipMemcpyAsync(buf, send, (size_t)n * sizeof(double), hipMemcpyDeviceToDevice, stream_));
    return;
  }
  AO_NCCL(ncclAllReduce(send, buf, (size_t)n, ncclDouble, ncclSum, c, stream_));
}

void Engine::check_mode(int m) const {
  AO_REQUIRE(m >= 0 && m < n_modes_, "mode %d out of range [0,%d)", m, n_modes_);
}

void Engine::model_begin(int n_modes, int n_tensors, int n_couplings) {
  AO_REQUIRE(n_modes > 0 && n_tensors > 0 && n_couplings >= 0, "model_begin: bad counts");
  AO_HIP(hipSetDevice(device_));
// ... 195 lines not shown
        need_H(ci.modes[0]);
        ci.rows = m0.rows; ci.cols = m0.hr;
        for (int m : ci.modes) {
          need_H(m);
          AO_REQUIRE(modes_[m].rows == ci.rows && modes_[m].hr == ci.cols && modes_[m].hc == modes_[m].R,
                     "coupling type 4: transformation matrix of mode %d has the wrong shape", m + 1);
          modes_[m].img_rows = modes_[m].rows; modes_[m].img_cols = modes_[m].R;
        }
        AO_REQUIRE(ci.cols <= kMaxRank, "coupling type 4: Delta has more than %d columns", kMaxRank);
        break;
      default:
        need_H(ci.modes[0]);
        AO_REQUIRE(m0.h2r > 0, "Coupling matrix H2 for mode %d is missing.", ci.modes[0] + 1);
        ci.rows = m0.hr; ci.cols = m0.h2r;
        for (int m : ci.modes) {
          need_H(m);
          AO_REQUIRE(modes_[m].h2r > 0, "Coupling matrix H2 for mode %d is missing.", m + 1);
          AO_REQUIRE(modes_[m].hc == modes_[m].rows && modes_[m].hr == ci.rows && modes_[m].h2r == ci.cols &&
                     modes_[m].h2c == modes_[m].R, "coupling type 5: transformation matrices of mode %d have the wrong shape", m + 1);
          modes_[m].img_rows = ci.rows; modes_[m].img_cols = modes_[m].R;
        }
        AO_REQUIRE(ci.cols <= kMaxRank, "coupling type 5: Delta has more than %d columns", kMaxRank);
        break;
    }
    for (int m : ci.modes) {
      ModeInfo& mi = modes_[m];
      if (ci.type == 2) {
        std::vector<double> hh((size_t)mi.R * mi.R, 0.0);
        for (int a = 0; a < mi.R; ++a)
          for (int b2 = 0; b2 < mi.R; ++b2) {
            double acc = 0.0;
            for (int64_t c2 = 0; c2 < mi.hc; ++c2) acc += mi.H_host[(size_t)a + (size_t)mi.hr * c2] * mi.H_host[(size_t)b2 + (size_t)mi.hr * c2];
            hh[(size_t)a + (size_t)mi.R * b2] = acc;
          }
        upload_small(mi.HHt, hh.data(), (int64_t)mi.R * mi.R, stream_);
      }
      if (ci.type == 1 || ci.type == 5) {
        const int64_t n = mi.rows;
        if (n > 4096) throw Error(AOADMM_ERR_UNSUPPORTED, "coupling types 1/5: modes beyond 4096 rows are not diagonalised on the host");
        std::vector<double> hth((size_t)n * n, 0.0), lam, U;
        for (int64_t a = 0; a < n; ++a)
          for (int64_t b2 = a; b2 < n; ++b2) {
            double acc = 0.0;
            for (int64_t q = 0; q < mi.hr; ++q) acc += mi.H_host[(size_t)q + (size_t)mi.hr * a] * mi.H_host[(size_t)q + (size_t)mi.hr * b2];
            hth[(size_t)a + (size_t)n * b2] = acc; hth[(size_t)b2 + (size_t)n * a] = acc;
          }
        AO_REQUIRE(host_sym_eig(n, hth, lam, U) >= 0, "eigendecomposition of H'*H (mode %d) did not converge", m + 1);
        std::vector<double> Ut((size_t)n * n);
        for (int64_t j = 0; j < n; ++j)
          for (int64_t i = 0; i < n; ++i) Ut[(size_t)j + (size_t)n * i] = U[(size_t)i + (size_t)n * j];
        upload_small(mi.eU, U.data(), n * n, stream_);
        upload_small(mi.eUt, Ut.data(), n * n, stream_);
        upload_small(mi.eLam, lam.data(), n, stream_);
      }
    }
  }
  {
    const size_t nsl = (size_t)(n_modes_ * (kSlotsPerMode + kResidPerMode) + 2 * n_tensors_ + 16 + 4 * n_tensors_) * sizeof(double);
    const size_t nct = (size_t)(n_modes_ + n_couplings_ + 1) * sizeof(AdmmCtl);
    const size_t off_ctl = (size_t)round_up((int64_t)nsl, 64);
    size_t tot = (size_t)round_up((int64_t)(off_ctl + nct), 64);
    std::vector<size_t> off_p2(n_tensors_, 0);
    for (int p = 0; p < n_tensors_; ++p)
      if (tensors_[p].par2) { off_p2[p] = tot; tot += ((size_t)6 * tensors_[p].p2.K + 1) * sizeof(double); }
    for (int p = 0; p < n_tensors_; ++p)
      if (tensors_[p].par2) { tensors_[p].p2.res.release(); tensors_[p].p2.q.release(); tensors_[p].p2.regv.release(); }
    ctls_.release(); slots_.release();
    readback_.alloc(tot);
    AO_HIP(hipMemsetAsync(readback_.p, 0, readback_.bytes, stream_));
    char* base = readback_.as<char>();
    slots_.view(base, nsl);
    ctls_.view(base + off_ctl, nct);
    for (int p = 0; p < n_tensors_; ++p) {
      if (!tensors_[p].par2) continue;
      Par2Block& b = tensors_[p].p2;
      char* q = base + off_p2[p];
      b.res.view(q, (size_t)(b.K + 1) * 8);
      b.q.view(q + (size_t)(b.K + 1) * 8, (size_t)b.K * 4 * 8);
      b.regv.view(q + (size_t)(5 * b.K + 1) * 8, (size_t)b.K * 8);
    }
  }
  AO_HIP(hipStreamSynchronize(stream_));
  model_done_ = true;
}

static int64_t pad_of(int prec, int64_t n) { return round_up(n, prec == AOADMM_PREC_F32 ? 4 : 2); }
static size_t blocked_bytes(int64_t M, int64_t C, size_t es) { return (size_t)round_up(M, kRowBlockElems) * C * es; }

void Engine::block_upload(CpBlock& b, int nd, const int64_t* dims, const double* host, int prec, int64_t row0,
                          int64_t local_rows, const double* full_array) {
  AO_REQUIRE(nd >= 2 && nd <= 8, "tensor order %d unsupported", nd);
  AO_REQUIRE(prec == AOADMM_PREC_F64 || prec == AOADMM_PREC_F32, "bad precision id %d", prec);
  AO_REQUIRE(row0 >= 0 && local_rows > 0 && row0 + local_rows <= dims[0], "bad row block [%lld,+%lld) of %lld",
             (long long)row0, (long long)local_rows, (long long)dims[0]);
  AO_HIP(hipSetDevice(device_));
  b.nd = nd;
  b.full0 = dims[0];
  b.row0 = row0;
  b.dims[0] = local_rows;
  int64_t ncols = 1;
  for (int i = 1; i < nd; ++i) { b.dims[i] = dims[i]; ncols *= dims[i]; }
  b.X.prec = prec; b.X.nd = nd;
  for (int i = 0; i < nd; ++i) b.X.dims[i] = b.dims[i];
  b.X.pad0 = pad_of(prec, local_rows);
  b.X.data.alloc((size_t)b.X.elems_padded() * b.X.elem_size());
  const int64_t chunk_cols = std::max<int64_t>(1, (int64_t)(64ll << 20) / local_rows);
  staging_.ensure((size_t)std::min(chunk_cols, ncols) * local_rows * sizeof(double));
  for (int64_t c0 = 0; c0 < ncols; c0 += chunk_cols) {
    const int64_t nc = std::min(chunk_cols, ncols - c0);
    AO_HIP(hipMemcpyAsync(staging_.p, host + c0 * local_rows, (size_t)nc * local_rows * sizeof(double),
                          hipMemcpyHostToDevice, stream_));
    pad_convert(b.X.data.p, prec, b.X.pad0, staging_.d(), local_rows, nc, c0, stream_);
    AO_HIP(hipStreamSynchronize(stream_));
  }
  if (nd == 2) {
    b.Xt.prec = prec; b.Xt.nd = 2;
    b.Xt.dims[0] = dims[1]; b.Xt.dims[1] = local_rows;
    b.Xt.pad0 = pad_of(prec, dims[1]);
    b.Xt.data.alloc((size_t)b.Xt.pad0 * local_rows * b.Xt.elem_size());
    AO_REQUIRE(ncols * local_rows <= (int64_t)(1ll << 28), "matrix block too large for the transposed copy");
    staging_.ensure((size_t)ncols * local_rows * sizeof(double));
    AO_HIP(hipMemcpyAsync(staging_.p, host, (size_t)ncols * local_rows * sizeof(double), hipMemcpyHostToDevice, stream_));
    transpose_convert(b.Xt.data.p, prec, b.Xt.pad0, staging_.d(), local_rows, ncols, stream_);
    AO_HIP(hipStreamSynchronize(stream_));
  }
  b.has_data = true;
  b.x_released = false;
  b.cached_mode = -1;
  b.has_xp = false; b.xp_refused = false; b.has_xq = false; b.xq_refused = false; b.has_xc = false; b.xc_refused = false;
  b.xp_ksharded = false;
  if (nd == 3 && full_array != nullptr) {
    int64_t k0 = 0, kloc = 0;
    if (want_ksharded_xp(b, dims[2], &k0, &kloc)) {
      const int64_t I = dims[0], J = dims[1], Ipf = pad_of(prec, I);
      DevBuf slab;
      slab.alloc((size_t)Ipf * J * kloc * b.X.elem_size());
      const double* src = full_array + (size_t)I * J * k0;
      const int64_t ncs = J * kloc;
      const int64_t cc = std::max<int64_t>(1, (int64_t)(64ll << 20) / I);
      staging_.ensure((size_t)std::min(cc, ncs) * I * sizeof(double));
      for (int64_t c0 = 0; c0 < ncs; c0 += cc) {
        const int64_t nc = std::min(cc, ncs - c0);
        AO_HIP(hipMemcpyAsync(staging_.p, src + c0 * I, (size_t)nc * I * sizeof(double), hipMemcpyHostToDevice, stream_));
        pad_convert(slab.p, prec, Ipf, staging_.d(), I, nc, c0, stream_);
        AO_HIP(hipStreamSynchronize(stream_));
      }
      adopt_ksharded_xp(b, slab.p, k0, kloc);
      AO_HIP(hipStreamSynchronize(stream_));
    }
  }
  if (nd == 3) { (void)ensure_permuted_copy2(b); (void)ensure_blocked_copy(b); }
}

void Engine::tensor_upload(int p, const double* data, int prec, int64_t row0, int64_t local_rows) {
  require_usable();
  AO_REQUIRE(model_done_, "call aoadmm_model_end first");
  AO_REQUIRE(p >= 0 && p < n_tensors_, "tensor %d out of range", p);
  TensorInfo& t = tensors_[p];
  AO_REQUIRE(!t.par2, "tensor %d is PARAFAC2: use aoadmm_par2_slab_upload", p);
  AO_REQUIRE(local_rows < 0 || !t.blk.sparse, "tensor %d holds sparse data: a row block cannot replace it (use aoadmm_tensor_upload)", p);
  if (t.blk.sparse) { t.blk.coo.clear(); t.blk.sparse = false; }
  int64_t dims[8];
  for (int i = 0; i < t.nmodes; ++i) dims[i] = modes_[t.modes[i]].rows;
  if (local_rows < 0) {
    int64_t I = dims[0];
    int64_t per = cdiv(I, world_);
    row0 = std::min<int64_t>(I, per * rank_);
    local_rows = std::min<int64_t>(I, row0 + per) - row0;
    AO_REQUIRE(per * (world_ - 1) < I, "tensor %d: first mode of %lld rows cannot be split over %d ranks (the last rank would own no rows)",
               p, (long long)I, world_);
    if (world_ == 1) {
      block_upload(t.blk, t.nmodes, dims, data, prec, 0, I);
    } else {
      int64_t ncols = 1;
      for (int i = 1; i < t.nmodes; ++i) ncols *= dims[i];
      std::vector<double> blk((size_t)local_rows * ncols);
      for (int64_t c = 0; c < ncols; ++c)
        std::memcpy(&blk[(size_t)c * local_rows], data + c * I + row0, (size_t)local_rows * sizeof(double));
      block_upload(t.blk, t.nmodes, dims, blk.data(), prec, row0, local_rows, data);
    }
  } else {
    block_upload(t.blk, t.nmodes, dims, data, prec, row0, local_rows);
  }
  t.normsq_valid = false;
}

void Engine::tensor_upload_coo(int p, int64_t nnz, const int64_t* subs, const double* vals) {
  require_usable();
  AO_REQUIRE(model_done_, "call aoadmm_model_end first");
  AO_REQUIRE(p >= 0 && p < n_tensors_, "tensor %d out of range", p);
  TensorInfo& t = tensors_[p];
  AO_REQUIRE(!t.par2, "tensor %d is PARAFAC2: sparse slabs are not supported", p);
  AO_REQUIRE(t.nmodes >= 2 && t.nmodes <= kCooMaxModes, "tensor %d: order %d unsupported for sparse data", p, t.nmodes);
  int64_t dims[8];
  for (int i = 0; i < t.nmodes; ++i) dims[i] = modes_[t.modes[i]].rows;
  AO_HIP(hipSetDevice(device_));
  CooBlock coo;
  coo_build(coo, t.nmodes, dims, nnz, subs, vals, stream_);
  CpBlock& b = t.blk;
  drop_permuted_copies(b);
  b.X.data.release(); b.Xt.data.release();
  b.emkr.release(); b.emkr2.release(); b.T.release(); b.frag.release(); b.scratch.release(); b.ft.release();
  b.tmpA.release(); b.tmpB.release(); b.mask.release(); b.maskT.release();
  for (int i = 0; i < 2; ++i) { b.own[i].release(); b.own_bytes[i] = 0; b.own_row0[i] = -1; }
  b.coo = std::move(coo);
  b.sparse = true;
  b.nd = t.nmodes;
  for (int i = 0; i < t.nmodes; ++i) b.dims[i] = dims[i];
  b.full0 = dims[0]; b.row0 = 0;
  b.has_data = true; b.has_mask = false; b.x_released = false;
  b.cached_mode = -1;
  b.has_xp = b.xp_refused = b.has_xq = b.xq_refused = b.has_xc = b.xc_refused = false;
  b.xp_ksharded = false;
  t.normsq_valid = false;
}

double Engine::tensor_normsq(int p) {
  require_usable();
  AO_REQUIRE(p >= 0 && p < n_tensors_, "tensor %d out of range", p);
  if (const char* fi = getenv("AOADMM_FAULT_INJECT"))
    if (std::strncmp(fi, "normsq:", 7) == 0 && std::atoi(fi + 7) == rank_ && world_ > 1)
      throw Error(AOADMM_ERR_HIP, "injected fault (AOADMM_FAULT_INJECT)");
  TensorInfo& t = tensors_[p];
  AO_REQUIRE(t.blk.has_data, "tensor %d has no data", p);
  if (!t.normsq_valid) {
    AO_HIP(hipSetDevice(device_));
    DevBuf ws;
    ws.alloc(1024 * sizeof(double) + 64);
    double* slot = slots_.d() + n_modes_ * (kSlotsPerMode + kResidPerMode) + 2 * n_tensors_;
    if (t.par2 ? t.p2.has_mask : t.blk.has_mask) {
      em_pass_enqueue(p, 0);
      double h4[4];
      AO_HIP(hipMemcpyAsync(h4, em_slot(p), sizeof h4, hipMemcpyDeviceToHost, stream_));
      AO_HIP(hipStreamSynchronize(stream_));
      t.normsq = h4[3];
      t.normsq_valid = true;
      return t.normsq;
    }
    if (t.par2) {
      tensor_sumsq(slot, t.p2.X.p, AOADMM_PREC_F64, (int64_t)t.p2.I * t.p2.Jtot, ws.d(), stream_);
    } else if (t.blk.sparse) {
      tensor_sumsq(slot, t.blk.coo.mode[0].val.p, AOADMM_PREC_F64, t.blk.coo.nnz, ws.d(), stream_);
    } else {
      AO_REQUIRE(!t.blk.x_released, "internal: ||X||^2 of tensor %d asked for after its natural-layout array was released", p);
      tensor_sumsq(slot, t.blk.X.data.p, t.blk.X.prec, t.blk.X.elems_padded(), ws.d(), stream_);
      allreduce(slot, 1);
    }
    double v = 0;
    AO_HIP(hipMemcpyAsync(&v, slot, sizeof(double), hipMemcpyDeviceToHost, stream_));
    AO_HIP(hipStreamSynchronize(stream_));
    t.normsq = v;
    t.normsq_valid = true;
  }
  return t.normsq;
}

void Engine::tensor_synth(int p, int rank, uint64_t seed, double noise, int prec) {
  require_usable();
  AO_REQUIRE(model_done_, "call aoadmm_model_end first");
  AO_REQUIRE(p >= 0 && p < n_tensors_, "tensor %d out of range", p);
  TensorInfo& t = tensors_[p];
  AO_REQUIRE(!t.par2 && t.nmodes == 3, "synthetic generator handles 3-way CP blocks");
  AO_REQUIRE(!t.blk.sparse, "tensor %d holds sparse data: the synthetic generator writes dense blocks (upload dense data first)", p);
  AO_REQUIRE(rank > 0 && rank <= kMaxRank, "bad rank");
  AO_HIP(hipSetDevice(device_));
  const int64_t I = modes_[t.modes[0]].rows, J = modes_[t.modes[1]].rows, K = modes_[t.modes[2]].rows;
  const int64_t per = cdiv(I, world_);
  const int64_t row0 = std::min<int64_t>(I, per * rank_);
  const int64_t loc = std::min<int64_t>(I, row0 + per) - row0;
  AO_REQUIRE(per * (world_ - 1) < I, "tensor %d: first mode of %lld rows cannot be split over %d ranks (the last rank would own no rows)",
             p, (long long)I, world_);
  CpBlock& b = t.blk;
  b.nd = 3; b.full0 = I; b.row0 = row0;
  b.dims[0] = loc; b.dims[1] = J; b.dims[2] = K;
  b.X.prec = prec; b.X.nd = 3;
  b.X.dims[0] = loc; b.X.dims[1] = J; b.X.dims[2] = K;
  b.X.pad0 = pad_of(prec, loc);
  b.X.data.alloc((size_t)b.X.elems_padded() * b.X.elem_size());
  DevBuf A, B, C, ws;
  A.alloc((size_t)I * rank * 8); B.alloc((size_t)J * rank * 8); C.alloc((size_t)K * rank * 8);
  ws.alloc(synth_ws_bytes());
  SynthArgs a;
  a.I_loc = loc; a.I_pad = b.X.pad0; a.J = J; a.K = K; a.row0 = row0; a.I_full = I; a.R = rank; a.seed = seed;
  synth_factors(A.d(), B.d(), C.d(), a, stream_);
  double* slot = slots_.d() + n_modes_ * (kSlotsPerMode + kResidPerMode) + 2 * n_tensors_;
  synth_norms(slot, A.d(), B.d(), C.d(), a, ws.d(), stream_);
  allreduce(slot, 3);
  double h[3];
  AO_HIP(hipMemcpyAsync(h, slot, 3 * sizeof(double), hipMemcpyDeviceToHost, stream_));
  AO_HIP(hipStreamSynchronize(stream_));
  const double sigma = h[1] > 0 ? noise * std::sqrt(h[0]) / std::sqrt(h[1]) : 0.0;
  const double nsq = h[0] + 2.0 * sigma * h[2] + sigma * sigma * h[1];
  synth_write(b.X.data.p, prec, A.d(), B.d(), C.d(), a, sigma, 1.0 / std::sqrt(nsq), stream_);
  AO_HIP(hipStreamSynchronize(stream_));
  b.has_data = true;
  b.x_released = false;
  b.cached_mode = -1;
  b.has_xp = false; b.xp_refused = false; b.has_xq = false; b.xq_refused = false; b.has_xc = false; b.xc_refused = false;
  b.xp_ksharded = false;
  {
    int64_t k0 = 0, kloc = 0;
    if (want_ksharded_xp(b, K, &k0, &kloc)) {
      SynthArgs ak = a;
      ak.I_loc = I; ak.I_pad = pad_of(prec, I); ak.row0 = 0; ak.k0 = k0; ak.K_loc = kloc;
      DevBuf slab;
      slab.alloc((size_t)ak.I_pad * J * kloc * b.X.elem_size());
      synth_write(slab.p, prec, A.d(), B.d(), C.d(), ak, sigma, 1.0 / std::sqrt(nsq), stream_);
      adopt_ksharded_xp(b, slab.p, k0, kloc);
      AO_HIP(hipStreamSynchronize(stream_));
    }
  }
  (void)ensure_permuted_copy2(b);
  (void)ensure_blocked_copy(b);
  AO_HIP(hipStreamSynchronize(stream_));
  t.normsq_valid = false;
}

void Engine::tensor_mask_upload(int p, const uint8_t* mask) {
  require_usable();
  AO_REQUIRE(p >= 0 && p < n_tensors_ && !tensors_[p].par2, "tensor %d is not a CP block", p);
  AO_REQUIRE(mask != nullptr, "null mask");
  TensorInfo& t = tensors_[p];
  CpBlock& b = t.blk;
  AO_REQUIRE(b.has_data, "upload Z.object{%d} before Z.miss{%d}", p + 1, p + 1);
  AO_REQUIRE(!b.sparse, "Missing data (Z.miss) not supported for sptensor objects. Convert to tensor first. (Z.object{%d}, cmtf_AOADMM.m:78-79)", p + 1);
  AO_REQUIRE(!b.x_released, "Z.object{%d} was released after its pass copies were built: upload it again before Z.miss{%d}", p + 1, p + 1);
  AO_HIP(hipSetDevice(device_));
  const int64_t Iloc = b.dims[0], Ip = b.X.pad0, Ifull = b.full0;
  int64_t ncols = 1;
  for (int i = 1; i < b.nd; ++i) ncols *= b.dims[i];
  DevBuf bytes;
  bytes.alloc((size_t)Ip * ncols);
  AO_HIP(hipMemsetAsync(bytes.p, 1, (size_t)Ip * ncols, stream_));
  AO_HIP(hipMemcpy2DAsync(bytes.p, (size_t)Ip, mask + b.row0, (size_t)Ifull, (size_t)Iloc, (size_t)ncols,
                          hipMemcpyHostToDevice, stream_));
  b.mask.alloc(em_mask_bits_bytes(Ip * ncols));
  em_mask_pack(bytes.as<uint8_t>(), b.mask.as<uint8_t>(), Ip * ncols, stream_);
  if (b.nd == 2) {
    const int64_t J = b.dims[1], Jp = b.Xt.pad0;
    std::vector<uint8_t> mt((size_t)Jp * Iloc, 1);
    for (int64_t i = 0; i < Iloc; ++i)
      for (int64_t j = 0; j < J; ++j) mt[(size_t)j + (size_t)Jp * i] = mask[b.row0 + i + Ifull * j];
    DevBuf bytesT;
    bytesT.alloc(mt.size());
    AO_HIP(hipMemcpyAsync(bytesT.p, mt.data(), mt.size(), hipMemcpyHostToDevice, stream_));
    b.maskT.alloc(em_mask_bits_bytes((int64_t)mt.size()));
    em_mask_pack(bytesT.as<uint8_t>(), b.maskT.as<uint8_t>(), (int64_t)mt.size(), stream_);
    AO_HIP(hipStreamSynchronize(stream_));
  }
  AO_HIP(hipStreamSynchronize(stream_));
  b.has_mask = true;
  drop_permuted_copies(b);
  t.normsq_valid = false;
}

bool Engine::has_missing() const {
  for (int p = 0; p < n_tensors_; ++p)
    if (tensors_[p].par2 ? tensors_[p].p2.has_mask : tensors_[p].blk.has_mask) return true;
  return false;
}

double* Engine::em_slot(int p) const {
  return slots_.d() + n_modes_ * (kSlotsPerMode + kResidPerMode) + 2 * n_tensors_ + 16 + 4 * p;
}

static int next_update_distance(int pos, int c, const int* seq, int n);

void Engine::em_pass_enqueue(int p, int update, bool fuse_next_pass) {
  TensorInfo& t = tensors_[p];
  if (t.par2) {
    Par2Block& b = t.p2;
    EmPar2Args a;
    a.X = b.X.d(); a.mask = b.mask.as<uint8_t>();
    a.A = modes_[t.modes[0]].fac.d(); a.B = modes_[t.modes[1]].fac.d(); a.C = modes_[t.modes[2]].fac.d();
    a.off = b.off_d.as<int64_t>(); a.K = b.K; a.I = b.I; a.R = b.R; a.update = update;
    emws_.ensure((size_t)b.K * 4 * sizeof(double));
    em_par2_pass(a, emws_.d(), em_slot(p), stream_);
    return;
  }
  CpBlock& b = t.blk;
  const ModeInfo& m0 = modes_[t.modes[0]];
  const ModeInfo& m1 = modes_[t.modes[1]];
  EmCpArgs a;
  a.X = b.X.data.p; a.mask = b.mask.as<uint8_t>();
  a.A = m0.fac.d() + (sharded() ? b.row0 : 0); a.ldA = m0.rows;
  a.B = m1.fac.d(); a.ldB = m1.rows;
  a.C = nullptr; a.ldC = 0;
  a.I = b.dims[0]; a.Ipad = b.X.pad0; a.J = b.dims[1]; a.K = 1; a.R = m0.R; a.update = update;
  if (b.nd == 3) {
    const ModeInfo& m2 = modes_[t.modes[2]];
    a.C = m2.fac.d(); a.ldC = m2.rows; a.K = b.dims[2];
  } else if (b.nd > 3) {
    int64_t Km = 1;
    for (int i = 2; i < b.nd; ++i) Km *= b.dims[i];
    b.emkr.ensure((size_t)Km * a.R * 8); b.emkr2.ensure((size_t)Km * a.R * 8);
    const ModeInfo& m2 = modes_[t.modes[2]];
    const double* cur = m2.fac.d();
    int64_t curK = b.dims[2], ld = m2.rows;
    double* bufs[2] = {b.emkr.d(), b.emkr2.d()};
    for (int i = 3; i < b.nd; ++i) {
      const ModeInfo& mn = modes_[t.modes[i]];
      double* dst = bufs[(i - 3) & 1];
      kr_merge(dst, cur, ld, curK, mn.fac.d(), mn.rows, b.dims[i], a.R, stream_);
      cur = dst; curK *= b.dims[i]; ld = curK;
    }
    a.C = cur; a.ldC = curK; a.K = curK;
  }
  emws_.ensure(em_cp_ws_bytes(a.Ipad, a.J, a.K));
  int fused_c = -1;
  ContractPlan fpl;
  FactorRef facs[8];
  if (fuse_next_pass && update && b.nd == 3 && em_cp_can_fuse(a, b.X.prec) && b.dims[1] <= 65535 &&
      b.dims[2] <= 65535 && !small_direct(b, a.R)) {
    for (int i = 0; i < t.nmodes; ++i) facs[i] = factor_ref(modes_[t.modes[i]]);
    const std::vector<int> seq = update_sequence(p);
    const int pos0 = seq.empty() ? 0 : seq[0];
    int best = -1;
    for (int cand = 2; cand >= 1; --cand) {
      if (cand == pos0) continue;
      const int dist = next_update_distance(pos0, cand, seq.data(), (int)seq.size());
      if (dist > best) { best = dist; fused_c = cand; }
    }
    if (getenv("AOADMM_EM_FUSE_SECOND_MODE") != nullptr && pos0 != 1) fused_c = 1;
    const int64_t J = b.dims[1], K = b.dims[2];
    a.walk = fused_c == 1 ? 1 : 2;
    fpl = fused_c == 2 ? make_plan(1, 0, a.Ipad * J, a.Ipad * J, K, a.R, b.X.prec)
                       : make_plan(K, a.Ipad * J, a.Ipad, a.Ipad, J, a.R, b.X.prec);
    fpl.nchunk = em_cp_fused_chunks(a, b.X.prec);
    b.T.ensure(fpl.t_bytes());
    a.T = b.T.p;
    a.t_chunk_stride = fpl.trows() * a.R;
  }
  em_cp_pass(a, b.X.prec, emws_.d(), em_slot(p), stream_);
  if (b.nd == 2 && update) {
    EmCpArgs at = a;
    at.X = b.Xt.data.p; at.mask = b.maskT.as<uint8_t>();
    at.A = m1.fac.d(); at.ldA = m1.rows; at.B = m0.fac.d() + (sharded() ? b.row0 : 0); at.ldB = m0.rows;
    at.I = b.dims[1]; at.Ipad = b.Xt.pad0; at.J = b.dims[0];
    const size_t wsb = em_cp_ws_bytes(at.Ipad, at.J, 1);
    emws_.ensure(wsb + 64);
    em_cp_pass(at, b.Xt.prec, emws_.d(), emws_.d() + wsb / sizeof(double), stream_);
  }
  allreduce(em_slot(p), 4);
  if (update) b.cached_mode = -1;
  if (fused_c >= 0) { b.cached_mode = fused_c; b.cached_version = facs[fused_c].version; b.plan = fpl; }
}

struct StateLoc {
  double* p;
  int64_t rows, cols;
};
static StateLoc slab_loc(DevBuf& buf, const ModeInfo& mB, int slab) {
  buf.ensure((size_t)mB.rows * mB.R * sizeof(double));
  if (slab == AOADMM_ALL_SLABS) return StateLoc{buf.d(), mB.rows, (int64_t)mB.R};
  AO_REQUIRE(slab >= 0 && slab < mB.K, "slab %d out of range [0,%d)", slab, mB.K);
  return StateLoc{buf.d() + mB.off_k[slab] * mB.R, mB.rows_k[slab], (int64_t)mB.R};
}

void Engine::state_set(int field, int index, int slab, const double* host, int64_t rows, int64_t cols) {
  AO_REQUIRE(model_done_, "call aoadmm_model_end first");
  AO_REQUIRE(host != nullptr && rows > 0 && cols > 0, "state_set: empty array");
  AO_HIP(hipSetDevice(device_));
  StateLoc loc{nullptr, 0, 0};
  if (field == AOADMM_F_COUPLING_FAC) {
    AO_REQUIRE(index >= 0 && index < n_couplings_, "coupling %d out of range", index);
    CouplingInfo& ci = couplings_[index];
    ci.Delta.ensure((size_t)ci.rows * ci.cols * sizeof(double));
    loc = StateLoc{ci.Delta.d(), ci.rows, ci.cols};
    ci.has_state = true;
  } else if (field == AOADMM_F_DELTAB || field == AOADMM_F_P || field == AOADMM_F_MU_DELTAB) {
    AO_REQUIRE(index >= 0 && index < n_tensors_ && tensors_[index].par2, "tensor %d is not a PARAFAC2 block", index);
    TensorInfo& t = tensors_[index];
    Par2Block& b = t.p2;
    const ModeInfo& mB = modes_[t.modes[1]];
    if (field == AOADMM_F_DELTAB) {
      b.DeltaB.ensure((size_t)b.R * b.R * sizeof(double));
      loc = StateLoc{b.DeltaB.d(), (int64_t)b.R, (int64_t)b.R};
      b.has_DeltaB = true;
    } else if (field == AOADMM_F_P) {
      loc = slab_loc(b.P, mB, slab);
      if (slab == AOADMM_ALL_SLABS) b.have_P.assign(b.K, 1); else b.have_P[slab] = 1;
    } else {
      loc = slab_loc(b.muDB, mB, slab);
      if (slab == AOADMM_ALL_SLABS) b.have_mu.assign(b.K, 1); else b.have_mu[slab] = 1;
    }
  } else {
    check_mode(index);
    ModeInfo& mi = modes_[index];
    auto whole = [&](DevBuf& buf, int64_t r, int64_t c) {
      buf.ensure((size_t)r * c * sizeof(double));
      return StateLoc{buf.d(), r, c};
    };
    switch (field) {
      case AOADMM_F_FAC:
        loc = mi.slabs ? slab_loc(mi.fac, mi, slab) : whole(mi.fac, mi.rows, mi.R);
        mi.has_fac = true; mi.version++;
        break;
      case AOADMM_F_CONSTRAINT_FAC:
        loc = mi.slabs ? slab_loc(mi.Z, mi, slab) : whole(mi.Z, mi.rows, mi.R);
        mi.has_Z = true;
        break;
      case AOADMM_F_CONSTRAINT_DUAL:
        loc = mi.slabs ? slab_loc(mi.mu, mi, slab) : whole(mi.mu, mi.rows, mi.R);
        mi.has_mu = true;
        break;
      case AOADMM_F_COUPLING_DUAL:
        AO_REQUIRE(!mi.slabs, "the PARAFAC2 B_k mode cannot be coupled");
        loc = whole(mi.muD, rows, cols);
        mi.has_muD = true; mi.muD_rows = rows; mi.muD_cols = cols;
        break;
      default: throw Error(AOADMM_ERR_INVALID, fmt("unknown state field %d", field));
    }
  }
  AO_REQUIRE(rows == loc.rows && cols == loc.cols, "state field %d index %d slab %d must be %lld x %lld, got %lld x %lld", field,
             index + 1, slab + 1, (long long)loc.rows, (long long)loc.cols, (long long)rows, (long long)cols);
  AO_HIP(hipMemcpyAsync(loc.p, host, (size_t)rows * cols * sizeof(double), hipMemcpyHostToDevice, stream_));
  AO_HIP(hipStreamSynchronize(stream_));
}

void Engine::state_get(int field, int index, int slab, double* host, int64_t rows, int64_t cols) {
  AO_REQUIRE(host != nullptr, "state_get: null destination");
  AO_HIP(hipSetDevice(device_));
  StateLoc loc{nullptr, 0, 0};
  if (field == AOADMM_F_COUPLING_FAC) {
    AO_REQUIRE(index >= 0 && index < n_couplings_, "coupling %d out of range", index);
    AO_REQUIRE(couplings_[index].has_state, "coupling_fac{%d} was never set", index + 1);
    loc = StateLoc{couplings_[index].Delta.d(), couplings_[index].rows, couplings_[index].cols};
  } else if (field == AOADMM_F_DELTAB || field == AOADMM_F_P || field == AOADMM_F_MU_DELTAB) {
    AO_REQUIRE(index >= 0 && index < n_tensors_ && tensors_[index].par2, "tensor %d is not a PARAFAC2 block", index);
    TensorInfo& t = tensors_[index];
    Par2Block& b = t.p2;
    const ModeInfo& mB = modes_[t.modes[1]];
    AO_REQUIRE(b.has_DeltaB, "DeltaB{%d} was never set", index + 1);
    if (field == AOADMM_F_DELTAB) loc = StateLoc{b.DeltaB.d(), (int64_t)b.R, (int64_t)b.R};
    else if (field == AOADMM_F_P) loc = slab_loc(b.P, mB, slab);
    else loc = slab_loc(b.muDB, mB, slab);
  } else {
    check_mode(index);
    ModeInfo& mi = modes_[index];
    switch (field) {
      case AOADMM_F_FAC:
        AO_REQUIRE(mi.has_fac, "fac{%d} was never set", index + 1);
        loc = mi.slabs ? slab_loc(mi.fac, mi, slab) : StateLoc{mi.fac.d(), mi.rows, (int64_t)mi.R};
        break;
      case AOADMM_F_CONSTRAINT_FAC:
        AO_REQUIRE(mi.has_Z, "constraint_fac{%d} was never set", index + 1);
        loc = mi.slabs ? slab_loc(mi.Z, mi, slab) : StateLoc{mi.Z.d(), mi.rows, (int64_t)mi.R};
        break;
      case AOADMM_F_CONSTRAINT_DUAL:
        AO_REQUIRE(mi.has_mu, "constraint_dual_fac{%d} was never set", index + 1);
        loc = mi.slabs ? slab_loc(mi.mu, mi, slab) : StateLoc{mi.mu.d(), mi.rows, (int64_t)mi.R};
        break;
      case AOADMM_F_COUPLING_DUAL:
        AO_REQUIRE(mi.has_muD, "coupling_dual_fac{%d} was never set", index + 1);
        loc = StateLoc{mi.muD.d(), mi.muD_rows, mi.muD_cols};
        break;
      default: throw Error(AOADMM_ERR_UNSUPPORTED, fmt("state field %d not available", field));
    }
  }
  AO_REQUIRE(rows == loc.rows && cols == loc.cols, "state_get: destination is %lld x %lld, field is %lld x %lld", (long long)rows,
             (long long)cols, (long long)loc.rows, (long long)loc.cols);
  AO_HIP(hipMemcpyAsync(host, loc.p, (size_t)rows * cols * sizeof(double), hipMemcpyDeviceToHost, stream_));
  AO_HIP(hipStreamSynchronize(stream_));
}

hipEvent_t Engine::take_event() {
  if (event_pool_.empty()) {
    for (int i = 0; i < 64; ++i) {
      hipEvent_t e = nullptr;
      AO_HIP(hipEventCreate(&e));
      event_pool_.push_back(e);
    }
  }
  hipEvent_t e = event_pool_.back();
  event_pool_.pop_back();
  return e;
}

void Engine::timed_contract(const void* X, int prec, const ContractPlan& pl, const double* F, int64_t ldF,
                            void* frag, void* T) {
  KernelStats& ks = kstats_[pl.lead ? 1 : 0];
  hipEvent_t e0 = nullptr, e1 = nullptr;
  static const bool no_events = getenv("AOADMM_NO_PASS_EVENTS") != nullptr;
  static const int every = [] { const char* e = getenv("AOADMM_PASS_EVENT_EVERY"); const int v = e ? atoi(e) : 4; return v < 1 ? 1 : v; }();
  if (profile_ && !no_events && ks.launches % every == 0) {
    if (ks.pending.size() >= 512) fold_finished(ks);
    if (ks.pending.size() < 4096) {
      e0 = take_event();
      e1 = take_event();
    }
  }
  launch_contract(X, prec, pl, F, ldF, frag, T, stream_, e0, e1);
  if (e0) { ks.pending.emplace_back(e0, e1); ks.timed++; }
  ks.launches++;
  ks.bytes += pl.algorithmic_bytes(prec);
  ks.flops += pl.flops();
}

void Engine::fold_finished(KernelStats& ks) {
  size_t keep = 0;
  for (size_t i = 0; i < ks.pending.size(); ++i) {
    auto& pr = ks.pending[i];
    float t = 0.f;
    if (hipEventQuery(pr.second) == hipSuccess && hipEventElapsedTime(&t, pr.first, pr.second) == hipSuccess) {
      ks.ms += t;
      event_pool_.push_back(pr.first);
      event_pool_.push_back(pr.second);
    } else {
      ks.pending[keep++] = pr;
    }
  }
  ks.pending.resize(keep);
}

void Engine::kernel_stats(int which, int reset, double* ms, int64_t* launches, double* bytes, double* flops) {
  AO_REQUIRE(which >= 0 && which <= 3, "kernel_stats: which must be 0, 1, 2 or 3");
  if (which == 2) profile_reductions_ = true;
  AO_HIP(hipSetDevice(device_));
  AO_HIP(hipStreamSynchronize(stream_));
  KernelStats& ks = kstats_[which];
  for (auto& pr : ks.pending) {
    float t = 0.f;
    AO_HIP(hipEventElapsedTime(&t, pr.first, pr.second));
    ks.ms += t;
    event_pool_.push_back(pr.first);
    event_pool_.push_back(pr.second);
  }
  ks.pending.clear();
  if (ms) *ms = (ks.timed > 0 && ks.timed < ks.launches) ? ks.ms * (double)ks.launches / (double)ks.timed : ks.ms;
  if (launches) *launches = ks.launches;
  if (bytes) *bytes = ks.bytes;
  if (flops) *flops = ks.flops;
  if (reset) { ks.ms = 0; ks.launches = 0; ks.timed = 0; ks.bytes = 0; ks.flops = 0; }
}

static int next_update_distance(int pos, int c, const int* seq, int n) {
  if (!seq || n <= 0) return c;
  int at = -1;
  for (int i = 0; i < n; ++i)
    if (seq[i] == pos) at = i;
  if (at < 0) return c;
  for (int d = 1; d <= n; ++d)
    if (seq[(at + d) % n] == c) return d;
  return n + 1;
}


static bool room_for(size_t bytes) {
  size_t free_b = 0, total_b = 0;
  return hipMemGetInfo(&free_b, &total_b) == hipSuccess && free_b >= bytes + (size_t)(4ull << 30);
}

bool Engine::want_ksharded_xp(const CpBlock& b, int64_t K, int64_t* k0, int64_t* kloc) const {
  if (!sharded() || world_ <= 1 || !allow_xp_ || b.has_mask || b.nd != 3) return false;
  const int64_t per = cdiv(K, world_);
  if (per * (world_ - 1) >= K) return false;
  *k0 = per * rank_;
  *kloc = std::min<int64_t>(K, *k0 + per) - *k0;
  return true;
}
void Engine::adopt_ksharded_xp(CpBlock& b, const void* slab, int64_t k0, int64_t kloc) {
  const int64_t Ifull = b.full0, J = b.dims[1];
  const int prec = b.X.prec;
  const int64_t Ipf = round_up(Ifull, prec == AOADMM_PREC_F32 ? 4 : 2);
  const int64_t Jp = round_up(J, prec == AOADMM_PREC_F32 ? 4 : 2);
  b.Xp.alloc(blocked_bytes(Jp * kloc, Ifull, b.X.elem_size()));
  b.Jp = Jp;
  AO_REQUIRE(block_layout_copy(slab, b.Xp.p, 1, prec, Ifull, Ipf, J, kloc, Jp, stream_), "tensor mode too long for the copy kernels");
  b.has_xp = true; b.xp_ksharded = true; b.xp_k0 = k0; b.xp_kloc = kloc;
}

bool Engine::ensure_permuted_copy(CpBlock& b) {
  if (b.has_xp) return true;
  if (b.xp_refused || !allow_xp_ || b.has_mask || b.nd != 3) return false;
  const int64_t I = b.dims[0], J = b.dims[1], K = b.dims[2];
  const int64_t Jp = round_up(J, b.X.prec == AOADMM_PREC_F32 ? 4 : 2);
  const size_t bytes = blocked_bytes(Jp * K, I, b.X.elem_size());
  if (!room_for(bytes)) { b.xp_refused = true; return false; }
  b.Xp.alloc(bytes);
  b.Jp = Jp;
  if (!block_layout_copy(b.X.data.p, b.Xp.p, 1, b.X.prec, I, b.X.pad0, J, K, Jp, stream_)) {
    b.Xp.release(); b.xp_refused = true; return false;
  }
  b.has_xp = true;
  return true;
}

bool Engine::ensure_permuted_copy2(CpBlock& b) {
  if (b.has_xq) return true;
  if (b.xq_refused || !ensure_permuted_copy(b)) return false;
  const int64_t I = b.dims[0], J = b.dims[1], K = b.dims[2];
  const int64_t Kp = round_up(K, b.X.prec == AOADMM_PREC_F32 ? 4 : 2);
  const size_t bytes = blocked_bytes(Kp * I, J, b.X.elem_size());
  if (!room_for(bytes)) { b.xq_refused = true; return false; }
  b.Xq.alloc(bytes);
  b.Kp = Kp;
  if (!block_layout_copy(b.X.data.p, b.Xq.p, 2, b.X.prec, I, b.X.pad0, J, K, Kp, stream_)) {
    b.Xq.release(); b.xq_refused = true; return false;
  }
  b.has_xq = true;
  return true;
}

bool Engine::ensure_blocked_copy(CpBlock& b) {
  if (b.has_xc) return true;
  if (b.xc_refused || !allow_xp_ || b.has_mask || b.nd != 3) return false;
  const int64_t I = b.dims[0], J = b.dims[1], K = b.dims[2];
  const size_t bytes = blocked_bytes(b.X.pad0 * J, K, b.X.elem_size());
  if (!room_for(bytes)) { b.xc_refused = true; return false; }
  b.Xc.alloc(bytes);
  if (!block_layout_copy(b.X.data.p, b.Xc.p, 0, b.X.prec, I, b.X.pad0, J, K, 0, stream_)) {
    b.Xc.release(); b.xc_refused = true; return false;
  }
  b.has_xc = true;
  return true;
}
void Engine::maybe_release_natural(TensorInfo& t) {
  CpBlock& b = t.blk;
  if (b.sparse || b.x_released || b.nd != 3 || !(b.has_xc && b.has_xp && b.has_xq) || b.has_mask || !t.normsq_valid || !b.X.data.p) return;
  const char* pe = getenv("AOADMM_RELEASE_NATURAL");
  const int policy = pe ? (atoi(pe) != 0 ? 1 : -1) : 0;
  if (policy < 0) return;
  if (policy == 0) {
    size_t free_b = 0, total_b = 0;
    const size_t mine = (size_t)b.X.elems_padded() * b.X.elem_size();
    if (hipMemGetInfo(&free_b, &total_b) != hipSuccess || free_b >= mine) return;
  }
  AO_HIP(hipStreamSynchronize(stream_));
  b.X.data.release();
  b.x_released = true;
}

void Engine::drop_permuted_copies(CpBlock& b) {
  if (b.has_xp) { b.Xp.release(); b.has_xp = false; b.xp_ksharded = false; b.cached_mode = -1; }
  if (b.has_xq) { b.Xq.release(); b.has_xq = false; b.cached_mode = -1; }
  if (b.has_xc) { b.Xc.release(); b.has_xc = false; b.cached_mode = -1; }
}

void Engine::ensure_contraction(CpBlock& b, int pos, const FactorRef* facs, int R, bool use_cache,
                                const int* update_seq, int nseq) {
  const int prec = b.X.prec;
  const int64_t I = b.dims[0], Ip = b.X.pad0, J = b.dims[1], K = b.dims[2];
  if (b.x_released) use_cache = true;
  const bool hit = use_cache && b.cached_mode >= 0 && b.cached_mode != pos &&
                   facs[b.cached_mode].version == b.cached_version;
  if (hit) return;
  int c = -1, best = -1;
  for (int cand = 2; cand >= 0; --cand) {
    if (cand == pos) continue;
    if (cand == 0 && !(use_cache && (prec == AOADMM_PREC_F32 || ensure_permuted_copy(b)))) continue;
    const int dist = next_update_distance(pos, cand, update_seq, nseq);
    if (dist > best) { best = dist; c = cand; }
  }
  ContractPlan pl;
  const double* Fc = facs[c].p;
  auto blocked_plan = [&](int64_t M, int64_t C) {
    const int64_t MB = kRowBlockElems;
    return make_plan(round_up(M, MB) / MB, MB * C, MB, MB, C, R, prec);
  };
  if (c == 2) {
    if (use_cache && ensure_blocked_copy(b)) {
      pl = blocked_plan(Ip * J, K);
      pl.on_xc = true;
    } else {
      pl = make_plan(1, 0, Ip * J, Ip * J, K, R, prec);
    }
  } else if (c == 1) {
    if (use_cache && ensure_permuted_copy2(b)) {
      pl = blocked_plan(b.Kp * I, J);
      pl.on_xq = true;
    } else {
      pl = make_plan(K, Ip * J, Ip, Ip, J, R, prec);
    }
  } else {
    Fc = facs[0].p + (sharded() ? b.row0 : 0);
    if (ensure_permuted_copy(b)) {
      if (b.xp_ksharded) { pl = blocked_plan(b.Jp * b.xp_kloc, b.full0); Fc = facs[0].p; }
      else pl = blocked_plan(b.Jp * K, I);
      pl.on_xp = true;
    } else {
      pl = make_lead_plan(J * K, Ip, I, R);
    }
  }
  b.T.ensure(pl.t_bytes()); b.frag.ensure(pl.frag_bytes(prec));
  timed_contract(pl.on_xp ? b.Xp.p : (pl.on_xq ? b.Xq.p : (pl.on_xc ? b.Xc.p : b.X.data.p)), prec, pl, Fc, facs[c].ld, b.frag.p,
                 b.T.p);
  b.cached_mode = c; b.cached_version = facs[c].version; b.plan = pl;
}

bool Engine::prefetch_next_contraction(const aoadmm_options& opt) {
  if (!opt.use_dimtree) return false;
  for (int cid = -1; cid < n_couplings_; ++cid) {
    for (int p = 0; p < n_tensors_; ++p)
      for (int m = 0; m < n_modes_; ++m) {
        const ModeInfo& mi = modes_[m];
        if (mi.coupling != cid || mi.tensor != p) continue;
        TensorInfo& t = tensors_[p];
        if (t.par2 || t.blk.sparse || t.blk.nd != 3 || small_direct(t.blk, mi.R)) return false;
        FactorRef facs[8];
        for (int i = 0; i < t.nmodes; ++i) {
          const ModeInfo& o = modes_[t.modes[i]];
          facs[i] = factor_ref(o);
        }
        std::vector<int> seq = update_sequence(p);
        const int64_t before = kstats_[0].launches + kstats_[1].launches;
        ensure_contraction(t.blk, mi.pos, facs, mi.R, true, seq.data(), (int)seq.size());
        return kstats_[0].launches + kstats_[1].launches > before;
      }
  }
  return false;
}

void Engine::block_mttkrp(CpBlock& b, int pos, const FactorRef* facs, int R, double scale, double* out,
                          int64_t ldOut, bool use_cache, const int* update_seq, int nseq, bool collective,
                          bool tensor_pass, const SysBuild* sys, bool* sys_done) {
  if (sys_done) *sys_done = false;
  AO_REQUIRE(b.has_data, "tensor has no data");
  AO_REQUIRE(pos >= 0 && pos < b.nd, "mttkrp: mode %d out of range", pos);
  if (b.sparse) {
    sparse_mttkrp(b, pos, facs, R, scale, out, ldOut);
    return;
  }
  const int prec = b.X.prec;
  const int64_t I = b.dims[0], Ip = b.X.pad0;
  const bool sharded = collective && this->sharded();
  double* out_local = out;
  const int64_t out_rows_full = (pos == 0) ? b.full0 : b.dims[pos];
  const double* send = nullptr;
  int64_t ld_local = ldOut;
  auto own_rows_buffer = [&](int which, int64_t rows_full, int64_t row_first) {
    DevBuf& ob = b.own[which];
    const size_t need = (size_t)rows_full * R * sizeof(double);
    if (b.own_bytes[which] != need || b.own_row0[which] != row_first) {
      if (b.own_bytes[which] != need) ob.alloc(need);
      AO_HIP(hipMemsetAsync(ob.p, 0, need, stream_));
      b.own_bytes[which] = need;
      b.own_row0[which] = row_first;
    }
    send = ob.d();
    ld_local = rows_full;
    out_local = ob.d() + row_first;
  };
  if (sharded && pos == 0) own_rows_buffer(0, out_rows_full, b.row0);
  const double* F0 = facs[0].p + (sharded ? b.row0 : 0);

  if (!tensor_pass && small_direct(b, R)) {
    const int64_t J = b.dims[1], K = b.nd == 3 ? b.dims[2] : 1;
    const int64_t st[3] = {1, Ip, Ip * J};
    const int64_t ext[3] = {I, J, K};
    int ia = pos == 0 ? 1 : 0, ib = pos == 2 ? 1 : 2;
    SmallMttkrp sm;
    sm.X = b.X.data.p;
    sm.sn = st[pos]; sm.sa = st[ia]; sm.Na = (int)ext[ia];
    sm.Fa = facs[ia].p; sm.lda = facs[ia].ld;
    if (b.nd == 3) { sm.sb = st[ib]; sm.Nb = (int)ext[ib]; sm.Fb = facs[ib].p; sm.ldb = facs[ib].ld; }
    else { sm.sb = 0; sm.Nb = 1; sm.Fb = nullptr; sm.ldb = 0; }
    sm.R = R; sm.scale = scale; sm.out = out; sm.ldOut = ldOut;
    const bool rode = small_mttkrp(sm, prec, ext[pos], stream_, sys);
    if (sys_done) *sys_done = rode;
    return;
  }
  if (b.nd == 2) {
    const int64_t J = b.dims[1];
    if (pos == 0) {
      ContractPlan pl = make_plan(1, 0, Ip, Ip, J, R, prec);
      b.T.ensure(pl.t_bytes()); b.frag.ensure(pl.frag_bytes(prec));
      timed_contract(b.X.data.p, prec, pl, facs[1].p, facs[1].ld, b.frag.p, b.T.p);
      launch_t_to_colmajor(b.T.p, pl.tprec, pl.nchunk, pl.trows(), I, R, scale, out_local, ld_local, stream_);
    } else {
      const int64_t Jp = b.Xt.pad0;
      ContractPlan pl = make_plan(1, 0, Jp, Jp, I, R, prec);
      b.T.ensure(pl.t_bytes()); b.frag.ensure(pl.frag_bytes(prec));
      timed_contract(b.Xt.data.p, prec, pl, F0, facs[0].ld, b.frag.p, b.T.p);
      launch_t_to_colmajor(b.T.p, pl.tprec, pl.nchunk, pl.trows(), J, R, scale, out_local, ld_local, stream_);
    }
    b.cached_mode = -1;
  } else if (b.nd == 3) {
    const int64_t J = b.dims[1], K = b.dims[2];
    ensure_contraction(b, pos, facs, R, use_cache, update_seq, nseq);
    const int c = b.cached_mode;
    const ContractPlan& pl = b.plan;
    const bool ksh = sharded && pl.on_xp && b.xp_ksharded;
    int ia = c == 0 ? 1 : 0, ib = c == 2 ? 1 : 2;
    if (pl.on_xq) { ia = 2; ib = 0; }
    const int64_t ext[3] = {I, J, ksh ? b.xp_kloc : K};
    const int64_t An = ext[ia], Bn = ext[ib];
    const int64_t Apad = pl.on_xq ? b.Kp : (ia == 0 ? Ip : (pl.on_xp ? b.Jp : J));
    auto fac_p = [&](int m) { return m == 0 ? F0 : (m == 2 && ksh ? facs[2].p + b.xp_k0 : facs[m].p); };
    auto fac_pT = [&](int m) -> const double* {
      if (!facs[m].pT) return nullptr;
      if (m == 2 && ksh) return facs[2].pT + b.xp_k0 * R;
      return facs[m].pT + ((m == 0 && sharded) ? b.row0 * R : 0);
    };
    if (ksh && pos == 2) own_rows_buffer(1, K, b.xp_k0);
    KernelStats& rs = kstats_[2];
    hipEvent_t e0 = nullptr, e1 = nullptr;
    if (profile_ && profile_reductions_) {
      if (rs.pending.size() >= 512) fold_finished(rs);
      if (rs.pending.size() < 4096) {
        e0 = take_event();
        e1 = take_event();
        AO_HIP(hipEventRecord(e0, stream_));
      }
    }
    if (pos == ia) {
      b.scratch.ensure(reduce_outer_scratch_bytes(An, Bn, R));
      b.ft.ensure(reduce_factor_scratch_bytes(Bn, R));
      const bool rode = launch_reduce_outer(b.T.p, pl.tprec, pl.nchunk, pl.trows(), An, Apad, Bn, R, fac_p(ib), facs[ib].ld, scale,
                                            out_local, ld_local, b.scratch.d(), b.ft.d(), stream_, fac_pT(ib), 0, sys);
      if (sys_done) *sys_done = rode;
    } else {
      AO_REQUIRE(pos == ib, "internal: cached contraction cannot serve this mode");
      b.ft.ensure(reduce_factor_scratch_bytes(An, R));
      const bool rode = launch_reduce_inner(b.T.p, pl.tprec, pl.nchunk, pl.trows(), An, Apad, Bn, R, fac_p(ia), facs[ia].ld, scale,
                                            out_local, ld_local, b.ft.d(), stream_, fac_pT(ia), 0, sys);
      if (sys_done) *sys_done = rode;
    }
    if (e0) {
      AO_HIP(hipEventRecord(e1, stream_));
      rs.pending.emplace_back(e0, e1);
      rs.timed++;
    }
    rs.launches++;
    rs.bytes += (double)pl.t_bytes();
  } else {
    const int N = b.nd;
    const int c = pos == N - 1 ? N - 2 : N - 1;
    int64_t lead = Ip;
    for (int m = 1; m < c; ++m) lead *= b.dims[m];
    ContractPlan pl = (c == N - 1) ? make_plan(1, 0, lead, lead, b.dims[c], R, prec)
                                   : make_plan(b.dims[N - 1], lead * b.dims[c], lead, lead, b.dims[c], R, prec);
    b.T.ensure(pl.t_bytes()); b.frag.ensure(pl.frag_bytes(prec));
    timed_contract(b.X.data.p, prec, pl, c == 0 ? F0 : facs[c].p, facs[c].ld, b.frag.p, b.T.p);
    int rem[8], nrem = 0;
    int64_t ext[8];
    for (int m = 0; m < N; ++m)
      if (m != c) { rem[nrem] = m; ext[nrem] = m == 0 ? Ip : b.dims[m]; ++nrem; }
    const void* Tin = b.T.p;
    int tprec = pl.tprec, nchunk = pl.nchunk;
    int64_t trows = pl.trows();
    int flip = 0;
    auto tbuf = [&](int64_t rows) {
      DevBuf& d = flip ? b.tmpB : b.tmpA;
      flip ^= 1;
      d.ensure((size_t)rows * R * sizeof(double));
      return d.d();
    };
    while (nrem > 1 && rem[nrem - 1] != pos) {
      const int mb = rem[nrem - 1];
      int64_t Arows = 1;
      for (int q = 0; q < nrem - 1; ++q) Arows *= ext[q];
      const bool last = nrem == 2;
      double* dst = last ? out_local : tbuf(Arows);
      const int64_t An = last ? (rem[0] == 0 ? I : b.dims[rem[0]]) : Arows;
      b.scratch.ensure(reduce_outer_scratch_bytes(An, b.dims[mb], R));
      b.ft.ensure(reduce_factor_scratch_bytes(b.dims[mb], R));
      launch_reduce_outer(Tin, tprec, nchunk, trows, An, Arows, b.dims[mb], R, facs[mb].p, facs[mb].ld,
                          last ? scale : 1.0, dst, last ? ld_local : 0, b.scratch.d(), b.ft.d(), stream_, nullptr, last ? 0 : 1);
      if (last) { nrem = 1; break; }
      Tin = dst; tprec = AOADMM_PREC_F64; nchunk = 1; trows = Arows;
      --nrem;
    }
    while (nrem > 1) {
      const int ma = rem[0];
      int64_t Brows = 1;
      for (int q = 1; q < nrem; ++q) Brows *= ext[q];
      const bool last = nrem == 2;
      double* dst = last ? out_local : tbuf(Brows);
      const int64_t An = ma == 0 ? I : b.dims[ma];
      b.ft.ensure(reduce_factor_scratch_bytes(An, R));
      launch_reduce_inner(Tin, tprec, nchunk, trows, An, ext[0], Brows, R, ma == 0 ? F0 : facs[ma].p, facs[ma].ld,
                          last ? scale : 1.0, dst, last ? ld_local : 0, b.ft.d(), stream_, nullptr, last ? 0 : 1);
      Tin = dst; tprec = AOADMM_PREC_F64; nchunk = 1; trows = Brows;
      for (int q = 0; q + 1 < nrem; ++q) { rem[q] = rem[q + 1]; ext[q] = ext[q + 1]; }
      --nrem;
    }
    b.cached_mode = -1;
  }
  if (sharded) {
    if (send) {
      if (ldOut == out_rows_full) allreduce_from(send, out, out_rows_full * R);
      else for (int r = 0; r < R; ++r) allreduce_from(send + out_rows_full * r, out + ldOut * r, out_rows_full);
    } else if (ldOut == out_rows_full) allreduce(out, out_rows_full * R);
    else for (int r = 0; r < R; ++r) allreduce(out + ldOut * r, out_rows_full);
  }
}

void Engine::sparse_mttkrp(CpBlock& b, int pos, const FactorRef* facs, int R, double scale, double* out, int64_t ldOut) {
  CooFactor f[kCooMaxModes];
  int k = 0;
  for (int m = 0; m < b.nd; ++m) {
    if (m == pos) continue;
    f[k++] = facs[m].pT ? CooFactor{facs[m].pT, (int64_t)R, 1} : CooFactor{facs[m].p, 1, facs[m].ld};
  }
  KernelStats& ks = kstats_[3];
  hipEvent_t e0 = nullptr, e1 = nullptr;
  if (profile_) {
    if (ks.pending.size() >= 512) fold_finished(ks);
    if (ks.pending.size() < 4096) {
      e0 = take_event();
      e1 = take_event();
      AO_HIP(hipEventRecord(e0, stream_));
    }
  }
  coo_mttkrp(b.coo, pos, f, R, scale, out, ldOut, stream_);
  if (e0) {
    AO_HIP(hipEventRecord(e1, stream_));
    ks.pending.emplace_back(e0, e1);
    ks.timed++;
  }
  ks.launches++;
  ks.bytes += coo_mttkrp_bytes(b.coo, pos, R);
  ks.flops += coo_mttkrp_flops(b.coo, R);
}

std::vector<int> Engine::update_sequence(int p) const {
  std::vector<int> seq;
  const TensorInfo& t = tensors_[p];
  for (int cid = -1; cid < n_couplings_; ++cid)
    for (int i = 0; i < t.nmodes; ++i)
      if (modes_[t.modes[i]].coupling == cid) seq.push_back(i);
  return seq;
}

void Engine::ensure_mode_work(ModeInfo& mi) {
  const size_t nR = (size_t)mi.rows * mi.R * sizeof(double), RR = (size_t)mi.R * mi.R * sizeof(double);
  mi.A.ensure(nR); mi.Ab.ensure(nR);
  mi.gram.ensure(RR); mi.C.ensure(RR); mi.Bsys.ensure(RR); mi.L.ensure(RR); mi.Binv.ensure(RR);
  mi.rho.ensure(64);
  mi.Zold.ensure(nR); mi.V.ensure(nR); mi.Znew.ensure(nR); mi.RHS.ensure(nR); mi.TD.ensure(nR); mi.tmp.ensure(nR);
  mi.part.ensure((size_t)admm_partials(mi.rows) * 4 * sizeof(double));
  if (mi.constrained) mi.proxws.ensure(prox_ws_bytes(mi.prox.type, mi.rows, mi.R));
  atbws_.ensure(atb_ws_bytes(mi.rows, mi.R, mi.R));
}

void Engine::compute_gram(ModeInfo& mi, const LoopEnd* close) {
  mi.facT.ensure((size_t)mi.rows * mi.R * sizeof(double));
  atb_small(mi.gram.d(), mi.fac.d(), mi.rows, mi.fac.d(), mi.rows, mi.rows, mi.R, mi.R, atbws_.d(), nullptr, stream_,
            mi.facT.d(), close);
  mi.facT_version = mi.version;
}

void Engine::prepare_mode_system(int m, int nrho, const aoadmm_options& opt) {
  ModeInfo& mi = modes_[m];
  TensorInfo& t = tensors_[mi.tensor];
  if (t.par2) {
    AO_REQUIRE(mi.pos == 0, "internal: only the first PARAFAC2 mode goes through the CP-style system");
    par2_prepare_modeA(m, nrho, opt);
    return;
  }
  FactorRef facs[8];
  for (int i = 0; i < t.nmodes; ++i) {
    const ModeInfo& o = modes_[t.modes[i]];
    facs[i] = factor_ref(o);
  }
  std::vector<int> seq = update_sequence(mi.tensor);
  SysBuild sb;
  sb.ngram = 0;
  for (int i = 0; i < t.nmodes; ++i)
    if (i != mi.pos) sb.grams[sb.ngram++] = modes_[t.modes[i]].gram.d();
  sb.Cpre = nullptr;
  sb.w = t.weight;
  sb.ridge = has_ridge_ ? mi.ridge : 0.0;
  sb.bsum_half = opt.bsum ? opt.bsum_weight / 2 : 0.0;
  sb.rho_scale = 1.0;
  sb.nrho = nrho;
  sb.R = mi.R;
  sb.C = mi.C.d(); sb.rho = mi.rho.d(); sb.Bsys = mi.Bsys.d(); sb.L = mi.L.d();
  sb.Binv = nrho > 0 ? mi.Binv.d() : nullptr;
  sb.ctl = ctl_of_mode(m);
  const int cty = mi.coupling >= 0 ? couplings_[mi.coupling].type : -1;
  if (cty == 2) sb.Madd = mi.HHt.d();
  bool rode = false;
  block_mttkrp(t.blk, mi.pos, facs, mi.R, t.weight, mi.A.d(), mi.rows, opt.use_dimtree != 0, seq.data(), (int)seq.size(), true,
               false, &sb, &rode);
  if (!rode) sys_build(sb, stream_);
  if (cty == 1 || cty == 5) {
// ... 1282 lines not shown
    }
    admm_finalize_generic(fa, ctl, stream_);
  }
}

void Engine::eval_objective_enqueue(bool first) {
  double* S = slots_.d();
  ReduceBatch rb;
  auto add = [&](int kind, double* slot, const double* x, const double* y, int64_t n) {
    ReduceTask k;
    k.kind = kind; k.slot = slot; k.x = x; k.y = y; k.n = n;
    rb.add(k);
  };
  for (int p = 0; p < n_tensors_; ++p) {
    TensorInfo& t = tensors_[p];
    const bool masked = t.par2 ? t.p2.has_mask : t.blk.has_mask;
    if (masked && first) em_pass_enqueue(p, 0);
    if (t.par2) {
      par2_objective_enqueue(t);
      t.eval_shortcut = !masked && !first && t.last_pos == 0;
      if (t.eval_shortcut) {
        ModeInfo& lm = modes_[t.modes[0]];
        double* sp = S + n_modes_ * kSlotsPerMode + 2 * p;
        add(RT_DOT, sp + 0, lm.A.d(), lm.fac.d(), lm.rows * lm.R);
        add(RT_DOT, sp + 1, lm.C.d(), lm.gram.d(), (int64_t)lm.R * lm.R);
      }
      continue;
    }
    if (masked) continue;
    if (first) {
      ModeInfo& m0 = modes_[t.modes[0]];
      FactorRef facs[8];
      for (int i = 0; i < t.nmodes; ++i) {
        const ModeInfo& o = modes_[t.modes[i]];
        facs[i] = factor_ref(o);
      }
      std::vector<int> seq = update_sequence(p);
      block_mttkrp(t.blk, 0, facs, m0.R, t.weight, m0.A.d(), m0.rows, true, seq.data(), (int)seq.size());
      SysBuild sb;
      sb.ngram = 0;
      for (int i = 1; i < t.nmodes; ++i) sb.grams[sb.ngram++] = modes_[t.modes[i]].gram.d();
      sb.Cpre = nullptr; sb.w = t.weight; sb.ridge = 0; sb.bsum_half = 0; sb.rho_scale = 1; sb.nrho = 1; sb.R = m0.R;
      sb.C = m0.C.d(); sb.rho = m0.rho.d(); sb.Bsys = m0.Bsys.d(); sb.L = m0.L.d(); sb.ctl = nullptr;
      sys_build(sb, stream_);
      t.last_pos = 0;
    }
    ModeInfo& lm = modes_[t.modes[t.last_pos]];
    double* sp = S + n_modes_ * kSlotsPerMode + 2 * p;
    add(RT_DOT, sp + 0, lm.A.d(), lm.fac.d(), lm.rows * lm.R);
    add(RT_DOT, sp + 1, lm.C.d(), lm.gram.d(), (int64_t)lm.R * lm.R);
  }
  for (int m = 0; m < n_modes_; ++m) {
    ModeInfo& mi = modes_[m];
    if (mi.slabs) continue;
    double* sm = S + (int64_t)m * kSlotsPerMode;
    const int64_t nm = mi.rows * mi.R;
    add(RT_SUMSQ_DIFF, sm + 0, mi.fac.d(), nullptr, nm);
    if (mi.constrained) {
      add(RT_SUMSQ_DIFF, sm + 1, mi.fac.d(), mi.Z.d(), nm);
      const int ty = mi.prox.type;
      if (ty == AOADMM_C_L2_REG) {
        reg_value(sm + 3, ty, mi.prox.p0, mi.fac.d(), mi.rows, mi.R, redws_.d(), stream_);
      } else if (ty == AOADMM_C_QUADRATIC) {
        gemm_small(mi.proxws.d(), mi.rows, mi.prox.Lmat, mi.rows, mi.fac.d(), mi.rows, mi.rows, (int)mi.rows, mi.R, 0,
                   coef(1.0), 0.0, nullptr, stream_);
        ReduceTask k;
        k.kind = RT_DOT; k.slot = sm + 3; k.x = mi.fac.d(); k.y = mi.proxws.d(); k.n = nm; k.scale = mi.prox.p0;
        rb.add(k);
      } else if (ty == AOADMM_C_L1_REG || ty == AOADMM_C_L0_REG || ty == AOADMM_C_RIDGE || ty == AOADMM_C_GL_SMOOTH ||
                 ty == AOADMM_C_TV) {
        ReduceTask k;
        k.kind = RT_REG; k.aux = ty; k.slot = sm + 3; k.x = mi.fac.d(); k.rows = mi.rows; k.R = mi.R; k.scale = mi.prox.p0;
        rb.add(k);
      }
    }
    if (mi.coupling >= 0) {
      CouplingInfo& ci = couplings_[mi.coupling];
      const size_t nimg = (size_t)std::max(nm, mi.img_rows * mi.img_cols) * sizeof(double);
      mi.TD.ensure(nimg); mi.TF.ensure(nimg);
      const double* td = image_d(mi.TD.d(), ci, ci.Delta.d(), mi, nullptr, stream_);
      const double* tf = image_f(mi.TF.d(), ci, mi.fac.d(), mi, nullptr, stream_);
      add(RT_SUMSQ_DIFF, sm + 2, tf, td, mi.img_rows * mi.img_cols);
      if (tf != mi.fac.d()) add(RT_SUMSQ_DIFF, sm + 4, tf, nullptr, mi.img_rows * mi.img_cols);
    }
    if (rb.n >= kReduceBatchMax - 4) {
      reduce_batch(rb, redws_.d(), stream_);
      rb = ReduceBatch();
    }
  }
  reduce_batch(rb, redws_.d(), stream_);
}

static bool stop_one(double f, double fo, const aoadmm_options& o) {
  const double rel = fo > 0 ? std::fabs(fo - f) / fo : std::fabs(fo - f);
  return f < o.AbsFuncTol || rel < o.OuterRelTol;
}

void Engine::solve(const aoadmm_options& opt, aoadmm_result* out) {
  require_usable();
  AO_REQUIRE(model_done_, "call aoadmm_model_end first");
  AO_REQUIRE(out != nullptr, "null result");
  AO_REQUIRE(opt.MaxOuterIters >= 0 && opt.MaxInnerIters >= 1, "bad iteration limits");
  AO_HIP(hipSetDevice(device_));
  prepared_mode_ = -1;
  allow_xp_ = opt.no_permuted_copy == 0;
  if (!allow_xp_)
    for (int p = 0; p < n_tensors_; ++p)
      drop_permuted_copies(tensors_[p].blk);
  for (int p = 0; p < n_tensors_; ++p) {
    AO_REQUIRE(tensors_[p].blk.has_data, "tensor %d has no data (Z.object{%d})", p, p + 1);
  }
  for (int m = 0; m < n_modes_; ++m) {
    ModeInfo& mi = modes_[m];
    AO_REQUIRE(mi.has_fac, "G.fac{%d} missing", m + 1);
    if (mi.constrained) AO_REQUIRE(mi.has_Z && mi.has_mu, "G.constraint_fac{%d} / constraint_dual_fac{%d} missing", m + 1, m + 1);
    if (mi.coupling >= 0) {
      AO_REQUIRE(mi.has_muD && mi.muD_rows == mi.img_rows && mi.muD_cols == mi.img_cols, "G.coupling_dual_fac{%d} missing or mis-sized", m + 1);
      AO_REQUIRE(couplings_[mi.coupling].has_state, "G.coupling_fac{%d} missing", mi.coupling + 1);
    }
    ensure_mode_work(mi);
    if (!mi.slabs) compute_gram(mi);
  }
  for (int p = 0; p < n_tensors_; ++p) {
    TensorInfo& t = tensors_[p];
    if (t.par2) {
      for (int k = 0; k < t.p2.K; ++k)
        AO_REQUIRE(t.p2.have_P[k] && t.p2.have_mu[k], "G.P{%d}{%d} / G.mu_DeltaB{%d}{%d} missing", p + 1, k + 1, p + 1, k + 1);
    }
    (void)tensor_normsq(p);
  }
  const bool has_miss = has_missing();
  for (int p = 0; p < n_tensors_; ++p) {
    TensorInfo& t = tensors_[p];
    if (!t.par2) continue;
    Par2Block& b = t.p2;
    AO_REQUIRE(b.has_DeltaB, "G.DeltaB{%d} missing", p + 1);
    for (int k = 0; k < b.K; ++k) AO_REQUIRE(b.have_P[k] && b.have_mu[k], "G.P{%d}{%d} / G.mu_DeltaB{%d}{%d} missing", p + 1, k + 1, p + 1, k + 1);
    par2_ensure_work(t);
    {
      const ModeInfo& mB = modes_[t.modes[1]];
      const bool can = sharded() && world_ > 1 && !b.has_mask && !(mB.constrained && mB.prox.type == AOADMM_C_TPARAFAC2) &&
                       modes_[t.modes[2]].coupling < 0;
      const bool want = opt.par2_slab_sharding > 0 || (opt.par2_slab_sharding == 0 && b.K / world_ >= 1024);
      const int per = (int)cdiv(b.K, world_);
      b.slab_sharded = can && want && (int64_t)per * (world_ - 1) < b.K;
      b.k0 = std::min(b.K, per * rank_);
      b.k1 = std::min(b.K, b.k0 + per);
    }
    par2_gram(modes_[t.modes[1]].fac.d(), b.dims(), b.GB.d(), stream_);
    t.last_pos = 2;
  }
  const int nctl = n_modes_ + n_couplings_;
  const int nslots = n_modes_ * kSlotsPerMode + 2 * n_tensors_;
  struct Pinned {
    void* p = nullptr; hipEvent_t ev = nullptr;
    ~Pinned() { if (p) (void)hipHostFree(p); if (ev) (void)hipEventDestroy(ev); }
  } pin;
  const char* rb_base = readback_.as<char>();
  auto in_arena = [&](const DevBuf& d) {
    return !d.owned && static_cast<const char*>(d.p) >= rb_base && static_cast<const char*>(d.p) + d.bytes <= rb_base + readback_.bytes;
  };
  AO_REQUIRE(in_arena(slots_) && in_arena(ctls_), "read-back arena: slots / loop-control blocks are not views of it");
  AO_HIP(hipHostMalloc(&pin.p, readback_.bytes, hipHostMallocDefault));
  AO_HIP(hipEventCreateWithFlags(&pin.ev, hipEventDisableTiming));
  char* hb = static_cast<char*>(pin.p);
  double* hs = reinterpret_cast<double*>(hb + (slots_.as<char>() - rb_base));
  double* hem = hs + (em_slot(0) - slots_.d());
  AdmmCtl* hctl = reinterpret_cast<AdmmCtl*>(hb + (ctls_.as<char>() - rb_base));
  std::vector<double*> hp2v(n_tensors_, nullptr);
  for (int p = 0; p < n_tensors_; ++p) {
    if (!tensors_[p].par2) continue;
    Par2Block& b = tensors_[p].p2;
    AO_REQUIRE(in_arena(b.res) && in_arena(b.q) && in_arena(b.regv) && b.q.d() == b.res.d() + b.K + 1 &&
               b.regv.d() == b.res.d() + 5 * b.K + 1, "read-back arena: PARAFAC2 block %d keeps its sums elsewhere", p);
    hp2v[p] = reinterpret_cast<double*>(hb + (b.res.as<char>() - rb_base));
  }
  (void)nslots;

  auto enqueue_readback = [&]() {
    AO_HIP(hipMemcpyAsync(hb, readback_.p, readback_.bytes, hipMemcpyDeviceToHost, stream_));
    AO_HIP(hipEventRecord(pin.ev, stream_));
  };
  auto finish_eval = [&](double f[4]) {
    AO_HIP(hipEventSynchronize(pin.ev));
    for (int i = 0; i < nctl; ++i)
      if (hctl[i].notpd)
        throw Error(AOADMM_ERR_NOT_PD, "Cholesky failed: system matrix is not positive definite (chol in cmtf_fun_AOADMM.m:142/273/362)");
    double ft = 0.0, fpar = 0.0, fcon = 0.0;
    int ncon = 0;
    for (int p = 0; p < n_tensors_; ++p) {
      TensorInfo& t = tensors_[p];
      const double* sp = hs + n_modes_ * kSlotsPerMode + 2 * p;
      const bool masked = t.par2 ? t.p2.has_mask : t.blk.has_mask;
      if (t.par2) {
        Par2Block& b = t.p2;
        const double* res = hp2v[p];
        const double* q = res + b.K + 1;
        if (b.slab_sharded && res[b.K] > 0)
          throw Error(AOADMM_ERR_NOT_PD, "Cholesky failed in a PARAFAC2 slab system on another rank (chol in cmtf_fun_AOADMM.m:212/240)");
        double fp = 0.0;
        if (masked) fp = hem[4 * p + 2];
        else if (t.eval_shortcut) fp = t.normsq - 2.0 * (sp[0] / t.weight) + sp[1];
        else for (int k = 0; k < b.K; ++k) fp += res[k];
        ft += t.weight * fp;
        const ModeInfo& mB = modes_[t.modes[1]];
        double gp = 0.0, gz = 0.0, nb2 = 0.0;
        for (int k = 0; k < b.K; ++k) {
          const double nb = std::sqrt(q[4 * k + 1]);
          gp += std::sqrt(q[4 * k]) / nb;
          gz += std::sqrt(q[4 * k + 2]) / nb;
          nb2 += q[4 * k + 1];
        }
        fpar += gp;
        if (mB.constrained && mB.prox.type == AOADMM_C_TPARAFAC2) {
          double pen = 0.0;
          for (int k = 1; k < b.K; ++k) pen += q[4 * k + 3];
          ft += mB.prox.p0 * pen;
        }
        if (mB.constrained && prox_has_reg_value(mB.prox.type)) {
          const double* rv = res + 5 * b.K + 1;
          for (int k = 0; k < b.K; ++k) ft += rv[k];
        }
        if (mB.constrained) {
          const double g = gz / b.K;
          fcon += g;
          if (g != 0.0) ++ncon;
          if (has_ridge_) ft += mB.ridge * nb2;
        }
      } else if (masked) {
        ft += t.weight * hem[4 * p + 2];
      } else {
        const double f2 = sp[0] / t.weight;
        ft += t.weight * (t.normsq - 2.0 * f2 + sp[1]);
      }
    }
    if (fpar > 0) {
      const TensorInfo& tl = tensors_[n_tensors_ - 1];
      fpar /= tl.par2 ? tl.p2.K : 1;
    }
    std::vector<double> cp(n_couplings_, 0.0);
    for (int m = 0; m < n_modes_; ++m) {
      const ModeInfo& mi = modes_[m];
      if (mi.slabs) continue;
      const double* sm = hs + (int64_t)m * kSlotsPerMode;
      const double nf = std::sqrt(sm[0]);
      if (mi.constrained) {
        const int ty = mi.prox.type;
        if (prox_has_reg_value(ty)) ft += sm[3];
        const double g = std::sqrt(sm[1]) / nf;
        fcon += g;
        if (g != 0.0) ++ncon;
      }
      if (has_ridge_) ft += mi.ridge * sm[0];
      if (mi.coupling >= 0) {
        const int cty = couplings_[mi.coupling].type;
        const double den = (cty == 1 || cty == 2 || cty == 5) ? std::sqrt(sm[4]) : nf;
        cp[mi.coupling] += std::sqrt(sm[2]) / den;
      }
    }
    double fc = 0.0; int nc = 0;
    for (double v : cp) { fc += v; if (v != 0.0) ++nc; }
    if (fc > 0) fc /= nc;
    if (fcon > 0) fcon /= ncon;
    f[0] = ft; f[1] = fc; f[2] = fcon; f[3] = fpar;
  };

  double f[4], fo[4];
  eval_objective_enqueue(true);
  enqueue_readback();
  finish_eval(f);
  if (out->func_val_conv) out->func_val_conv[0] = f[0];
  if (out->func_coupl_conv) out->func_coupl_conv[0] = f[1];
  if (out->func_constr_conv) out->func_constr_conv[0] = f[2];
  if (out->func_PAR2_coupl) out->func_PAR2_coupl[0] = f[3];
  if (out->time_at_it) out->time_at_it[0] = 0.0;
  double f_rel_missing = std::nan("");
  if (out->func_rel_missing) out->func_rel_missing[0] = f_rel_missing;
  const bool report = progress_fn_ != nullptr && progress_every_ > 0;
  if (report) progress_fn_(progress_user_, 0, f, f_rel_missing);
  const auto t0 = std::chrono::steady_clock::now();

  int iter = 1;
  bool stop = false;
  while (iter <= opt.MaxOuterIters && !stop) {
    for (ModeInfo& mq : modes_) mq.quad.dirty = true;
    if (iter == 3)
      for (int p = 0; p < n_tensors_; ++p)
        if (!tensors_[p].par2) maybe_release_natural(tensors_[p]);
    for (int cid = -1; cid < n_couplings_; ++cid) {
      std::vector<int> cm;
      for (int m = 0; m < n_modes_; ++m)
        if (modes_[m].coupling == cid) cm.push_back(m);
      if (cm.empty()) continue;
      std::set<int> ps;
      for (int m : cm) ps.insert(modes_[m].tensor);
      for (int p : ps)
        for (int m : cm)
          if (modes_[m].tensor == p) {
            const bool par2 = tensors_[p].par2;
            if (par2 && modes_[m].pos == 1) par2_update_B(m, opt, iter);
            else if (par2 && modes_[m].pos == 2 && cid < 0) par2_update_C(m, opt);
            else if (par2 && modes_[m].pos == 2) par2_prepare_C_coupled(m, couplings_[cid].type, opt);
            else if (cid < 0) update_uncoupled_cp_mode(m, opt);
            else {
              const int cty = couplings_[cid].type;
              const int con = modes_[m].constrained ? 1 : 0;
              prepare_mode_system(m, (cty == 0 || cty == 3 || cty == 4) ? 1 + con : (cty == 2 ? con : 0), opt);
            }
          }
      if (cid >= 0) {
        coupled_admm(cid, opt);
        for (int m : cm) { modes_[m].version++; compute_gram(modes_[m]); }
      }
    }
    if (has_miss)
      for (int p = 0; p < n_tensors_; ++p)
        if (tensors_[p].par2 ? tensors_[p].p2.has_mask : tensors_[p].blk.has_mask)
// ... 143 lines not shown
```

Before: 129.5.

## Fuse slow-role MTTKRP into contraction epilogue and pick copy orders by update sequence

The contraction kernel's epilogue can now also weight the freshly computed tile of T by the row-major 'fast' factor and write per-tile partial sums. A small finish kernel then reduces those partials into the next mode's MTTKRP, replacing a separate pass that reads T back from memory. Permuted tensor copies now choose between two layouts per mode based on the update sequence, so the fused case lines up with the next mode in the sweep. The pinned readback buffer and event are also cached across calls instead of being allocated each solve. The added register array and shuffle reduction in the epilogue may lower occupancy of the contraction kernel.

```diff
diff --git a/matlab-code_amd/csrc/contract.h b/matlab-code_amd/csrc/contract.h
--- a/matlab-code_amd/csrc/contract.h
+++ b/matlab-code_amd/csrc/contract.h
@@ -17,6 +17,8 @@
   size_t elem_size() const { return prec == AOADMM_PREC_F32 ? 4 : 8; }
 };
 
+struct SysBuild;
+
 struct ContractPlan {
   int64_t nbatch, batch_stride, M, ld, C;
   int R;
@@ -26,6 +28,8 @@
   bool on_xp = false;
   bool on_xq = false;
   bool on_xc = false;
+  int fast = -1, slow = -1;
+  int64_t fpad = 0;
   int64_t trows() const { return nbatch * M; }
   size_t t_bytes() const { return (size_t)nchunk * trows() * R * (tprec == AOADMM_PREC_F32 ? 4 : 8); }
   size_t frag_bytes(int prec) const;
@@ -40,12 +44,23 @@
 
 ContractPlan make_lead_plan(int64_t M, int64_t ld, int64_t C, int R);
 
+struct FusedFirst {
+  const double* WT;
+  double* part;
+  int64_t F, Fpad, S;
+};
+bool fused_first_ok(const ContractPlan& pl, int prec, int64_t Fpad);
+size_t fused_part_bytes(const ContractPlan& pl);
+bool launch_fused_finish(const double* part, const ContractPlan& pl, int64_t Fpad, int64_t S, double scale, double* out,
+                         int64_t ldOut, hipStream_t s, const SysBuild* sys = nullptr);
+
 void launch_contract(const void* X, int prec, const ContractPlan& pl, const double* F, int64_t ldF,
                      void* frag_ws, void* T, hipStream_t s, hipEvent_t ev0 = nullptr,
-                     hipEvent_t ev1 = nullptr);
+                     hipEvent_t ev1 = nullptr,
+                     const FusedFirst* fuse = nullptr);
+void factor_rowmajor(const double* F, int64_t ldF, int64_t rows, int R, double* Ft, hipStream_t s);
 
 size_t reduce_factor_scratch_bytes(int64_t rows, int R);
-struct SysBuild;
 bool launch_reduce_inner(const void* T, int tprec, int nchunk, int64_t trows, int64_t A, int64_t Apad,
                          int64_t B, int R, const double* Fa, int64_t ldFa, double scale,
                          double* out, int64_t ldOut, double* ft_scratch, hipStream_t s,
diff --git a/matlab-code_amd/csrc/contract.hip b/matlab-code_amd/csrc/contract.hip
--- a/matlab-code_amd/csrc/contract.hip
+++ b/matlab-code_amd/csrc/contract.hip
@@ -21,6 +21,9 @@
   int64_t tiles_per_batch, ntiles, batch_stride, M, ld, C, Cg, trows;
   int groups_per_chunk, R;
   int flush_every;
+  const double* WT;
+  double* part;
+  int64_t F, Fpad, S;
 };
 
 typedef float f32x2 __attribute__((ext_vector_type(2)));
@@ -273,12 +276,54 @@
             if (e < ne) tl[(64 * h + 4 * r16 + v) * a.R + 16 * NT + e] = accE[h][v][e >> 1][e & 1];
     }
   }
+  constexpr int kFuseRows = 43;
+  const bool fuse = L2 && a.part != nullptr;
+  double wgt[kFuseRows];
+  int fR = 1, fnrg = 1, frg = 0, fr = 0, nlo = kTileRows;
+  if (fuse) {
+    fR = a.R; fnrg = 64 / fR;
+    if (fnrg < 3) fnrg = 3;
+    frg = lane / fR; fr = lane - frg * fR;
+    const int64_t grow = b * a.M + m0;
+    const int64_t s0 = grow / a.Fpad, f0 = grow - s0 * a.Fpad;
+    if (a.Fpad - f0 < kTileRows) nlo = (int)(a.Fpad - f0);
+#pragma unroll
+    for (int it = 0; it < kFuseRows; ++it) {
+      const int row = frg + it * fnrg;
+      const bool up = row >= nlo;
+      const int64_t f = f0 + row - (up ? a.Fpad : 0);
+      const bool live = frg < fnrg && row < kTileRows && f < a.F && s0 + (up ? 1 : 0) < a.S;
+      const double w = a.WT[(live ? f : 0) * fR + fr];
+      wgt[it] = live ? w : 0.0;
+    }
+  }
   {
     const int64_t rows_here = (a.M - m0 < kTileRows) ? a.M - m0 : kTileRows;
     const int n16 = (int)(rows_here * a.R / 4);
     f32x4* dst = reinterpret_cast<f32x4*>(reinterpret_cast<float*>(a.T) + ((int64_t)chunk * a.trows + b * a.M + m0) * a.R);
     const f32x4* src = reinterpret_cast<const f32x4*>(tl);
     for (int c = lane; c < n16; c += 64) __builtin_nontemporal_store(src[c], dst + c);
+  }
+  if (fuse) {
+    double lo = 0.0, hi = 0.0;
+#pragma unroll
+    for (int it = 0; it < kFuseRows; ++it) {
+      const int row = frg + it * fnrg;
+      const double t = (double)tl[(row < kTileRows ? row : kTileRows - 1) * fR + fr];
+      const bool up = row >= nlo;
+      lo = __builtin_fma(t, up ? 0.0 : wgt[it], lo);
+      hi = __builtin_fma(t, up ? wgt[it] : 0.0, hi);
+    }
+    double tlo = lo, thi = hi;
+    for (int k = 1; k < fnrg; ++k) {
+      tlo += __shfl(lo, (lane + k * fR) & 63);
+      thi += __shfl(hi, (lane + k * fR) & 63);
+    }
+    if (lane < fR) {
+      double* pp = a.part + (((int64_t)chunk * a.ntiles + wt) * 2) * fR + lane;
+      pp[0] = tlo;
+      if (nlo < kTileRows) pp[fR] = thi;
+    }
   }
 }
 
@@ -701,9 +746,18 @@
   AO_KERNEL_CHECK();
 }
 
+bool fused_first_ok(const ContractPlan& pl, int prec, int64_t Fpad) {
+  return prec == AOADMM_PREC_F32 && !pl.lead && pl.R >= 1 && pl.R <= 20 && pl.M % kTileRows == 0 && Fpad >= kTileRows &&
+         Fpad % 4 == 0;
+}
+size_t fused_part_bytes(const ContractPlan& pl) {
+  return (size_t)pl.nchunk * pl.nbatch * cdiv(pl.M, kTileRows) * 2 * pl.R * sizeof(double);
+}
+
 void launch_contract(const void* X, int prec, const ContractPlan& pl, const double* F, int64_t ldF,
-                     void* frag_ws, void* T, hipStream_t s, hipEvent_t ev0, hipEvent_t ev1) {
+                     void* frag_ws, void* T, hipStream_t s, hipEvent_t ev0, hipEvent_t ev1, const FusedFirst* fuse) {
   AO_REQUIRE(pl.tprec == prec, "contraction plan and tensor precision disagree");
+  AO_REQUIRE(fuse == nullptr || fused_first_ok(pl, prec, fuse->Fpad), "internal: this pass cannot carry a fused MTTKRP");
   AO_REQUIRE(pl.R >= 1 && pl.R <= kMaxRank, "rank %d outside [1,%d]", pl.R, kMaxRank);
   if (pl.lead) {
     AO_REQUIRE(prec == AOADMM_PREC_F32, "leading-mode contraction exists for fp32 tensors only");
@@ -719,6 +773,8 @@
   a.trows = pl.trows();
   a.groups_per_chunk = (int)cdiv(Cg, pl.nchunk);
   a.R = pl.R;
+  a.WT = nullptr; a.part = nullptr; a.F = a.Fpad = a.S = 0;
+  if (fuse) { a.WT = fuse->WT; a.part = fuse->part; a.F = fuse->F; a.Fpad = fuse->Fpad; a.S = fuse->S; }
   AO_REQUIRE(a.ntiles > 0 && pl.C > 0, "empty contraction");
   dim3 grid((unsigned)cdiv(a.ntiles, 4), (unsigned)pl.nchunk);
   AO_REQUIRE(cdiv(a.ntiles, 4) < (int64_t)2147483647, "tensor too large for one launch");
@@ -775,7 +831,7 @@
   const int64_t a = idx - (int64_t)r * rows;
   Ft[a * R + r] = F[a + ldF * r];
 }
-static void factor_rowmajor(const double* F, int64_t ldF, int64_t rows, int R, double* Ft, hipStream_t s) {
+void factor_rowmajor(const double* F, int64_t ldF, int64_t rows, int R, double* Ft, hipStream_t s) {
   factor_rowmajor_k<<<(unsigned)cdiv(rows * R, 256), 256, 0, s>>>(F, ldF, rows, R, Ft);
   AO_KERNEL_CHECK();
 }
@@ -1086,6 +1142,37 @@
   return sys != nullptr;
 }
 
+__global__ __launch_bounds__(256) void fused_fin_k(const double* __restrict__ part, int nchunk, int64_t ntiles, int64_t Fpad,
+                                                   int64_t S, int R, double scale, double* __restrict__ out, int64_t ldOut,
+                                                   int has_sys, SysBuild sys) {
+  if (has_sys && blockIdx.x == 0) { sys_build_rider(sys); return; }
+  const int64_t idx = ((int64_t)blockIdx.x - has_sys) * blockDim.x + threadIdx.x;
+  if (idx >= S * R) return;
+  const int64_t sidx = idx / R;
+  const int r = (int)(idx - sidx * R);
+  const int64_t row_lo = sidx * Fpad;
+  const int64_t t0 = row_lo / kTileRows, t1 = (row_lo + Fpad - 1) / kTileRows;
+  double tot = 0.0;
+  for (int ch = 0; ch < nchunk; ++ch) {
+    const double* pc = part + (int64_t)ch * ntiles * 2 * R + r;
+#pragma unroll 4
+    for (int64_t t = t0; t <= t1; ++t) tot += pc[(2 * t + (t * kTileRows < row_lo ? 1 : 0)) * R];
+  }
+  out[sidx + ldOut * r] = scale * tot;
+}
+
+bool launch_fused_finish(const double* part, const ContractPlan& pl, int64_t Fpad, int64_t S, double scale, double* out,
+                         int64_t ldOut, hipStream_t s, const SysBuild* sys) {
+  if (!sys_can_ride(sys)) sys = nullptr;
+  const int hs = sys ? 1 : 0;
+  const int64_t ntiles = pl.nbatch * cdiv(pl.M, kTileRows);
+  AO_REQUIRE(S * Fpad <= ntiles * kTileRows, "internal: fused MTTKRP over more rows than the pass has");
+  fused_fin_k<<<(unsigned)(cdiv(S * pl.R, 256) + hs), 256, 0, s>>>(part, pl.nchunk, ntiles, Fpad, S, pl.R, scale, out, ldOut, hs,
+                                                                 sys ? *sys : SysBuild());
+  AO_KERNEL_CHECK();
+  return sys != nullptr;
+}
+
 template <typename TT, int RMAX>
 __global__ __launch_bounds__(256) void small_mttkrp_k(SmallMttkrp a, int has_sys, SysBuild sys) {
   extern __shared__ double sf[];
diff --git a/matlab-code_amd/csrc/misc.hip b/matlab-code_amd/csrc/misc.hip
--- a/matlab-code_amd/csrc/misc.hip
+++ b/matlab-code_amd/csrc/misc.hip
@@ -250,30 +250,42 @@
     *reinterpret_cast<VT*>(D + (m / MB) * MB * K + k * MB + m % MB) = v;
   }
 }
-template <typename T, int WHICH>
-__global__ __launch_bounds__(256) void block_permute_k(const T* __restrict__ X, T* __restrict__ D, int64_t I, int64_t Ip,
-                                                      int64_t J, int64_t K, int64_t Tp, int64_t MB) {
+template <typename T, int FORM>
+__global__ __launch_bounds__(256) void block_permute_k(const T* __restrict__ X, T* __restrict__ D, int64_t I, int64_t nT,
+                                                      int64_t st, int64_t su, int64_t Tp, int64_t C, int64_t MB) {
   __shared__ T tile[32][33];
   const int64_t u = blockIdx.z;
   const int64_t i0 = (int64_t)blockIdx.x * 32, t0 = (int64_t)blockIdx.y * 32;
   const int tx = threadIdx.x & 31, ty = threadIdx.x >> 5;
-  const int64_t nT = WHICH == 1 ? J : K;
-  const int64_t st = WHICH == 1 ? Ip : Ip * J, su = WHICH == 1 ? Ip * J : Ip;
 #pragma unroll
   for (int q = 0; q < 4; ++q) {
     const int64_t i = i0 + tx, t = t0 + ty + 8 * q;
     tile[ty + 8 * q][tx] = (i < I && t < nT) ? X[i + st * t + su * u] : (T)0;
   }
   __syncthreads();
-  const int64_t C = WHICH == 1 ? I : J;
 #pragma unroll
   for (int q = 0; q < 4; ++q) {
     const int64_t t = t0 + tx, i = i0 + ty + 8 * q;
     if (t < Tp && i < I) {
-      const int64_t m = WHICH == 1 ? t + Tp * u : t + Tp * i;
-      const int64_t c = WHICH == 1 ? i : u;
+      const int64_t m = FORM == 1 ? t + Tp * u : t + Tp * i;
+      const int64_t c = FORM == 1 ? i : u;
       D[(m / MB) * MB * C + c * MB + m % MB] = tile[tx][ty + 8 * q];
     }
+  }
+}
+template <typename T>
+__global__ __launch_bounds__(256) void block_copy_ik_k(const T* __restrict__ X, T* __restrict__ D, int64_t Ip, int64_t J,
+                                                      int64_t K, int64_t Mpad, int64_t MB) {
+  const int64_t j = blockIdx.y;
+  constexpr int V = 16 / sizeof(T);
+  typedef T VT __attribute__((ext_vector_type(V)));
+  for (int64_t m = ((int64_t)blockIdx.x * 256 + threadIdx.x) * V; m < Mpad; m += (int64_t)gridDim.x * 256 * V) {
+    VT v;
+#pragma unroll
+    for (int e = 0; e < V; ++e) v[e] = (T)0;
+    const int64_t k = m / Ip, i = m - k * Ip;
+    if (k < K) v = *reinterpret_cast<const VT*>(X + i + Ip * (j + J * k));
+    *reinterpret_cast<VT*>(D + (m / MB) * MB * J + j * MB + m % MB) = v;
   }
 }
 bool block_layout_copy(const void* X, void* D, int which, int prec, int64_t I, int64_t Ip, int64_t J, int64_t K,
@@ -292,15 +304,32 @@
     AO_KERNEL_CHECK();
     return true;
   }
-  const int64_t nU = which == 1 ? K : J, C = which == 1 ? I : J;
-  const int64_t M = which == 1 ? Tp * K : Tp * I, Mpad = round_up(M, MB);
+  if (which == 5) {
+    if (J > 65535) return false;
+    const int64_t Mpad = round_up(Ip * K, MB);
+    const int V = (int)(16 / es);
+    int64_t gx = cdiv(Mpad, (int64_t)256 * V);
+    if (gx > 65535) gx = 65535;
+    const dim3 grid((unsigned)gx, (unsigned)J);
+    if (prec == AOADMM_PREC_F32) block_copy_ik_k<float><<<grid, 256, 0, s>>>((const float*)X, (float*)D, Ip, J, K, Mpad, MB);
+    else block_copy_ik_k<double><<<grid, 256, 0, s>>>((const double*)X, (double*)D, Ip, J, K, Mpad, MB);
+    AO_KERNEL_CHECK();
+    return true;
+  }
+  AO_REQUIRE(which >= 1 && which <= 4, "block_layout_copy: unknown order %d", which);
+  const bool tj = which == 1 || which == 3;
+  const int form = (which == 1 || which == 4) ? 1 : 2;
+  const int64_t nT = tj ? J : K, nU = tj ? K : J;
+  const int64_t st = tj ? Ip : Ip * J, su = tj ? Ip * J : Ip;
+  const int64_t C = form == 1 ? I : nU;
+  const int64_t M = form == 1 ? Tp * nU : Tp * I, Mpad = round_up(M, MB);
   if (nU > 65535 || cdiv(Tp, 32) > 65535) return false;
   if (Mpad > M)
     AO_HIP(hipMemsetAsync((char*)D + (size_t)(Mpad / MB - 1) * MB * C * es, 0, (size_t)MB * C * es, s));
   const dim3 grid((unsigned)cdiv(I, 32), (unsigned)cdiv(Tp, 32), (unsigned)nU);
-#define AO_BP(TT, W) block_permute_k<TT, W><<<grid, 256, 0, s>>>((const TT*)X, (TT*)D, I, Ip, J, K, Tp, MB)
-  if (prec == AOADMM_PREC_F32) { if (which == 1) AO_BP(float, 1); else AO_BP(float, 2); }
-  else { if (which == 1) AO_BP(double, 1); else AO_BP(double, 2); }
+#define AO_BP(TT, W) block_permute_k<TT, W><<<grid, 256, 0, s>>>((const TT*)X, (TT*)D, I, nT, st, su, Tp, C, MB)
+  if (prec == AOADMM_PREC_F32) { if (form == 1) AO_BP(float, 1); else AO_BP(float, 2); }
+  else { if (form == 1) AO_BP(double, 1); else AO_BP(double, 2); }
 #undef AO_BP
   AO_KERNEL_CHECK();
   return true;
diff --git a/matlab-code_amd/csrc/solver.h b/matlab-code_amd/csrc/solver.h
--- a/matlab-code_amd/csrc/solver.h
+++ b/matlab-code_amd/csrc/solver.h
@@ -37,6 +37,10 @@
   bool has_xq = false, xq_refused = false;
   DevBuf Xc;
   bool has_xc = false, xc_refused = false;
+  bool exch[3] = {false, false, false};
+  DevBuf fpart;
+  int fused_mode = -1;
+  uint64_t fused_version = 0;
   int nd = 0;
   int64_t dims[8] = {0};
   int64_t full0 = 0;
@@ -207,6 +211,7 @@
   void adopt_ksharded_xp(CpBlock& b, const void* slab, int64_t k0, int64_t kloc);
   bool want_ksharded_xp(const CpBlock& b, int64_t K, int64_t* k0, int64_t* kloc) const;
   void drop_permuted_copies(CpBlock& b);
+  void choose_copy_orders(CpBlock& b, int p);
   void maybe_release_natural(TensorInfo& t);
   bool prefetch_next_contraction(const aoadmm_options& opt);
   void block_mttkrp(CpBlock& b, int pos, const FactorRef* facs, int R, double scale, double* out,
@@ -247,6 +252,9 @@
   hipStream_t stream_ = nullptr;
   hipStream_t side_ = nullptr;
   hipEvent_t side_ev_ = nullptr;
+  void* pin_p_ = nullptr;
+  size_t pin_bytes_ = 0;
+  hipEvent_t pin_ev_ = nullptr;
   int n_modes_ = 0, n_tensors_ = 0, n_couplings_ = 0;
   bool model_done_ = false;
   bool has_ridge_ = false;
@@ -283,7 +291,7 @@
   AdmmCtl* ctl_of_coupling(int c) { return ctls_.as<AdmmCtl>() + n_modes_ + c; }
   void sparse_mttkrp(CpBlock& b, int pos, const FactorRef* facs, int R, double scale, double* out, int64_t ldOut);
   void timed_contract(const void* X, int prec, const ContractPlan& pl, const double* F, int64_t ldF,
-                      void* frag, void* T);
+                      void* frag, void* T, const FusedFirst* fuse = nullptr);
 };
 
 }
diff --git a/matlab-code_amd/csrc/solver.hip b/matlab-code_amd/csrc/solver.hip
--- a/matlab-code_amd/csrc/solver.hip
+++ b/matlab-code_amd/csrc/solver.hip
@@ -52,6 +52,8 @@
   for (hipEvent_t e : event_pool_) (void)hipEventDestroy(e);
   if (comm_) (void)ncclCommDestroy(comm_);
   if (side_ev_) (void)hipEventDestroy(side_ev_);
+  if (pin_ev_) (void)hipEventDestroy(pin_ev_);
+  if (pin_p_) (void)hipHostFree(pin_p_);
   if (side_) (void)hipStreamDestroy(side_);
   if (stream_) (void)hipStreamDestroy(stream_);
 }
@@ -553,6 +555,16 @@
   if (nd == 3) { (void)ensure_permuted_copy2(b); (void)ensure_blocked_copy(b); }
 }
 
+void Engine::choose_copy_orders(CpBlock& b, int p) {
+  std::vector<int> seq = p >= 0 ? update_sequence(p) : std::vector<int>();
+  if (seq.size() != 3) seq = {0, 1, 2};
+  for (int c = 0; c < 3; ++c) {
+    int at = 0;
+    for (int i = 0; i < 3; ++i) if (seq[i] == c) at = i;
+    b.exch[c] = !sharded() && seq[(at + 1) % 3] == (c + 1) % 3;
+  }
+}
+
 void Engine::tensor_upload(int p, const double* data, int prec, int64_t row0, int64_t local_rows) {
   require_usable();
   AO_REQUIRE(model_done_, "call aoadmm_model_end first");
@@ -563,6 +575,7 @@
   if (t.blk.sparse) { t.blk.coo.clear(); t.blk.sparse = false; }
   int64_t dims[8];
   for (int i = 0; i < t.nmodes; ++i) dims[i] = modes_[t.modes[i]].rows;
+  choose_copy_orders(t.blk, p);
   if (local_rows < 0) {
     int64_t I = dims[0];
     int64_t per = cdiv(I, world_);
@@ -699,6 +712,7 @@
   b.cached_mode = -1;
   b.has_xp = false; b.xp_refused = false; b.has_xq = false; b.xq_refused = false; b.has_xc = false; b.xc_refused = false;
   b.xp_ksharded = false;
+  choose_copy_orders(b, p);
   {
     int64_t k0 = 0, kloc = 0;
     if (want_ksharded_xp(b, K, &k0, &kloc)) {
@@ -827,6 +841,7 @@
     a.walk = fused_c == 1 ? 1 : 2;
     fpl = fused_c == 2 ? make_plan(1, 0, a.Ipad * J, a.Ipad * J, K, a.R, b.X.prec)
                        : make_plan(K, a.Ipad * J, a.Ipad, a.Ipad, J, a.R, b.X.prec);
+    fpl.fast = 0; fpl.slow = fused_c == 2 ? 1 : 2; fpl.fpad = a.Ipad;
     fpl.nchunk = em_cp_fused_chunks(a, b.X.prec);
     b.T.ensure(fpl.t_bytes());
     a.T = b.T.p;
@@ -844,7 +859,7 @@
   }
   allreduce(em_slot(p), 4);
   if (update) b.cached_mode = -1;
-  if (fused_c >= 0) { b.cached_mode = fused_c; b.cached_version = facs[fused_c].version; b.plan = fpl; }
+  if (fused_c >= 0) { b.cached_mode = fused_c; b.cached_version = facs[fused_c].version; b.plan = fpl; b.fused_mode = -1; }
 }
 
 struct StateLoc {
@@ -979,7 +994,7 @@
 }
 
 void Engine::timed_contract(const void* X, int prec, const ContractPlan& pl, const double* F, int64_t ldF,
-                            void* frag, void* T) {
+                            void* frag, void* T, const FusedFirst* fuse) {
   KernelStats& ks = kstats_[pl.lead ? 1 : 0];
   hipEvent_t e0 = nullptr, e1 = nullptr;
   static const bool no_events = getenv("AOADMM_NO_PASS_EVENTS") != nullptr;
@@ -991,7 +1006,7 @@
       e1 = take_event();
     }
   }
-  launch_contract(X, prec, pl, F, ldF, frag, T, stream_, e0, e1);
+  launch_contract(X, prec, pl, F, ldF, frag, T, stream_, e0, e1, fuse);
   if (e0) { ks.pending.emplace_back(e0, e1); ks.timed++; }
   ks.launches++;
   ks.bytes += pl.algorithmic_bytes(prec);
@@ -1075,12 +1090,13 @@
   if (b.has_xp) return true;
   if (b.xp_refused || !allow_xp_ || b.has_mask || b.nd != 3) return false;
   const int64_t I = b.dims[0], J = b.dims[1], K = b.dims[2];
-  const int64_t Jp = round_up(J, b.X.prec == AOADMM_PREC_F32 ? 4 : 2);
-  const size_t bytes = blocked_bytes(Jp * K, I, b.X.elem_size());
+  const int64_t Jp = pad_of(b.X.prec, J), Kp = pad_of(b.X.prec, K);
+  const bool ex = b.exch[0];
+  const size_t bytes = blocked_bytes(ex ? Kp * J : Jp * K, I, b.X.elem_size());
   if (!room_for(bytes)) { b.xp_refused = true; return false; }
   b.Xp.alloc(bytes);
   b.Jp = Jp;
-  if (!block_layout_copy(b.X.data.p, b.Xp.p, 1, b.X.prec, I, b.X.pad0, J, K, Jp, stream_)) {
+  if (!block_layout_copy(b.X.data.p, b.Xp.p, ex ? 4 : 1, b.X.prec, I, b.X.pad0, J, K, ex ? Kp : Jp, stream_)) {
     b.Xp.release(); b.xp_refused = true; return false;
   }
   b.has_xp = true;
@@ -1091,12 +1107,13 @@
   if (b.has_xq) return true;
   if (b.xq_refused || !ensure_permuted_copy(b)) return false;
   const int64_t I = b.dims[0], J = b.dims[1], K = b.dims[2];
-  const int64_t Kp = round_up(K, b.X.prec == AOADMM_PREC_F32 ? 4 : 2);
-  const size_t bytes = blocked_bytes(Kp * I, J, b.X.elem_size());
+  const int64_t Kp = pad_of(b.X.prec, K);
+  const bool ex = b.exch[1];
+  const size_t bytes = blocked_bytes(ex ? b.X.pad0 * K : Kp * I, J, b.X.elem_size());
   if (!room_for(bytes)) { b.xq_refused = true; return false; }
   b.Xq.alloc(bytes);
   b.Kp = Kp;
-  if (!block_layout_copy(b.X.data.p, b.Xq.p, 2, b.X.prec, I, b.X.pad0, J, K, Kp, stream_)) {
+  if (!block_layout_copy(b.X.data.p, b.Xq.p, ex ? 5 : 2, b.X.prec, I, b.X.pad0, J, K, Kp, stream_)) {
     b.Xq.release(); b.xq_refused = true; return false;
   }
   b.has_xq = true;
@@ -1107,10 +1124,12 @@
   if (b.has_xc) return true;
   if (b.xc_refused || !allow_xp_ || b.has_mask || b.nd != 3) return false;
   const int64_t I = b.dims[0], J = b.dims[1], K = b.dims[2];
-  const size_t bytes = blocked_bytes(b.X.pad0 * J, K, b.X.elem_size());
+  const int64_t Jp = pad_of(b.X.prec, J);
+  const bool ex = b.exch[2];
+  const size_t bytes = blocked_bytes(ex ? Jp * I : b.X.pad0 * J, K, b.X.elem_size());
   if (!room_for(bytes)) { b.xc_refused = true; return false; }
   b.Xc.alloc(bytes);
-  if (!block_layout_copy(b.X.data.p, b.Xc.p, 0, b.X.prec, I, b.X.pad0, J, K, 0, stream_)) {
+  if (!block_layout_copy(b.X.data.p, b.Xc.p, ex ? 3 : 0, b.X.prec, I, b.X.pad0, J, K, Jp, stream_)) {
     b.Xc.release(); b.xc_refused = true; return false;
   }
   b.has_xc = true;
@@ -1159,33 +1178,58 @@
     const int64_t MB = kRowBlockElems;
     return make_plan(round_up(M, MB) / MB, MB * C, MB, MB, C, R, prec);
   };
+  const int64_t Jp = pad_of(prec, J), Kp = pad_of(prec, K);
+  auto roles = [&](int fast, int slow, int64_t fpad) { pl.fast = fast; pl.slow = slow; pl.fpad = fpad; };
   if (c == 2) {
     if (use_cache && ensure_blocked_copy(b)) {
-      pl = blocked_plan(Ip * J, K);
+      pl = blocked_plan(b.exch[2] ? Jp * I : Ip * J, K);
       pl.on_xc = true;
+      if (b.exch[2]) roles(1, 0, Jp); else roles(0, 1, Ip);
     } else {
       pl = make_plan(1, 0, Ip * J, Ip * J, K, R, prec);
+      roles(0, 1, Ip);
     }
   } else if (c == 1) {
     if (use_cache && ensure_permuted_copy2(b)) {
-      pl = blocked_plan(b.Kp * I, J);
+      pl = blocked_plan(b.exch[1] ? Ip * K : Kp * I, J);
       pl.on_xq = true;
+      if (b.exch[1]) roles(0, 2, Ip); else roles(2, 0, Kp);
     } else {
       pl = make_plan(K, Ip * J, Ip, Ip, J, R, prec);
+      roles(0, 2, Ip);
     }
   } else {
     Fc = facs[0].p + (sharded() ? b.row0 : 0);
     if (ensure_permuted_copy(b)) {
       if (b.xp_ksharded) { pl = blocked_plan(b.Jp * b.xp_kloc, b.full0); Fc = facs[0].p; }
-      else pl = blocked_plan(b.Jp * K, I);
+      else pl = blocked_plan(b.exch[0] ? Kp * J : Jp * K, I);
       pl.on_xp = true;
+      if (b.exch[0] && !b.xp_ksharded) roles(2, 1, Kp); else roles(1, 2, Jp);
     } else {
       pl = make_lead_plan(J * K, Ip, I, R);
+      roles(1, 2, J);
     }
   }
   b.T.ensure(pl.t_bytes()); b.frag.ensure(pl.frag_bytes(prec));
+  FusedFirst ff;
+  const FusedFirst* fuse = nullptr;
+  b.fused_mode = -1;
+  if ((pl.on_xc || pl.on_xp || pl.on_xq) && !sharded() && pos == pl.slow && fused_first_ok(pl, prec, pl.fpad)) {
+    const int64_t ext[3] = {I, J, K};
+    ff.F = ext[pl.fast]; ff.Fpad = pl.fpad; ff.S = ext[pl.slow];
+    ff.WT = facs[pl.fast].pT;
+    if (!ff.WT) {
+      b.ft.ensure(reduce_factor_scratch_bytes(ff.F, R));
+      factor_rowmajor(facs[pl.fast].p, facs[pl.fast].ld, ff.F, R, b.ft.d(), stream_);
+      ff.WT = b.ft.d();
+    }
+    b.fpart.ensure(fused_part_bytes(pl));
+    ff.part = b.fpart.d();
+    fuse = &ff;
+    b.fused_mode = pos; b.fused_version = facs[pl.fast].version;
+  }
   timed_contract(pl.on_xp ? b.Xp.p : (pl.on_xq ? b.Xq.p : (pl.on_xc ? b.Xc.p : b.X.data.p)), prec, pl, Fc, facs[c].ld, b.frag.p,
-                 b.T.p);
+                 b.T.p, fuse);
   b.cached_mode = c; b.cached_version = facs[c].version; b.plan = pl;
 }
 
@@ -1282,11 +1326,11 @@
     const int c = b.cached_mode;
     const ContractPlan& pl = b.plan;
     const bool ksh = sharded && pl.on_xp && b.xp_ksharded;
-    int ia = c == 0 ? 1 : 0, ib = c == 2 ? 1 : 2;
-    if (pl.on_xq) { ia = 2; ib = 0; }
+    const int ia = pl.fast, ib = pl.slow;
+    AO_REQUIRE(ia >= 0 && ib >= 0 && ia != c && ib != c && ia != ib, "internal: partial contraction without row roles");
     const int64_t ext[3] = {I, J, ksh ? b.xp_kloc : K};
     const int64_t An = ext[ia], Bn = ext[ib];
-    const int64_t Apad = pl.on_xq ? b.Kp : (ia == 0 ? Ip : (pl.on_xp ? b.Jp : J));
+    const int64_t Apad = pl.fpad;
     auto fac_p = [&](int m) { return m == 0 ? F0 : (m == 2 && ksh ? facs[2].p + b.xp_k0 : facs[m].p); };
     auto fac_pT = [&](int m) -> const double* {
       if (!facs[m].pT) return nullptr;
@@ -1294,9 +1338,10 @@
       return facs[m].pT + ((m == 0 && sharded) ? b.row0 * R : 0);
     };
     if (ksh && pos == 2) own_rows_buffer(1, K, b.xp_k0);
+    const bool fused = b.fused_mode == pos && pos == ib && !this->sharded() && facs[ia].version == b.fused_version;
     KernelStats& rs = kstats_[2];
     hipEvent_t e0 = nullptr, e1 = nullptr;
-    if (profile_ && profile_reductions_) {
+    if (!fused && profile_ && profile_reductions_) {
       if (rs.pending.size() >= 512) fold_finished(rs);
       if (rs.pending.size() < 4096) {
         e0 = take_event();
@@ -1304,7 +1349,10 @@
         AO_HIP(hipEventRecord(e0, stream_));
       }
     }
-    if (pos == ia) {
+    if (fused) {
+      const bool rode = launch_fused_finish(b.fpart.d(), pl, Apad, Bn, scale, out_local, ld_local, stream_, sys);
+      if (sys_done) *sys_done = rode;
+    } else if (pos == ia) {
       b.scratch.ensure(reduce_outer_scratch_bytes(An, Bn, R));
       b.ft.ensure(reduce_factor_scratch_bytes(Bn, R));
       const bool rode = launch_reduce_outer(b.T.p, pl.tprec, pl.nchunk, pl.trows(), An, Apad, Bn, R, fac_p(ib), facs[ib].ld, scale,
@@ -1322,8 +1370,10 @@
       rs.pending.emplace_back(e0, e1);
       rs.timed++;
     }
-    rs.launches++;
-    rs.bytes += (double)pl.t_bytes();
+    if (!fused) {
+      rs.launches++;
+      rs.bytes += (double)pl.t_bytes();
+    }
   } else {
     const int N = b.nd;
     const int c = pos == N - 1 ? N - 2 : N - 1;
@@ -2912,17 +2962,19 @@
   }
   const int nctl = n_modes_ + n_couplings_;
   const int nslots = n_modes_ * kSlotsPerMode + 2 * n_tensors_;
-  struct Pinned {
-    void* p = nullptr; hipEvent_t ev = nullptr;
-    ~Pinned() { if (p) (void)hipHostFree(p); if (ev) (void)hipEventDestroy(ev); }
-  } pin;
+  struct { void* p; hipEvent_t ev; } pin;
   const char* rb_base = readback_.as<char>();
   auto in_arena = [&](const DevBuf& d) {
     return !d.owned && static_cast<const char*>(d.p) >= rb_base && static_cast<const char*>(d.p) + d.bytes <= rb_base + readback_.bytes;
   };
   AO_REQUIRE(in_arena(slots_) && in_arena(ctls_), "read-back arena: slots / loop-control blocks are not views of it");
-  AO_HIP(hipHostMalloc(&pin.p, readback_.bytes, hipHostMallocDefault));
-  AO_HIP(hipEventCreateWithFlags(&pin.ev, hipEventDisableTiming));
+  if (pin_bytes_ < readback_.bytes) {
+    if (pin_p_) { (void)hipHostFree(pin_p_); pin_p_ = nullptr; pin_bytes_ = 0; }
+    AO_HIP(hipHostMalloc(&pin_p_, readback_.bytes, hipHostMallocDefault));
+    pin_bytes_ = readback_.bytes;
+  }
+  if (!pin_ev_) AO_HIP(hipEventCreateWithFlags(&pin_ev_, hipEventDisableTiming));
+  pin.p = pin_p_; pin.ev = pin_ev_;
   char* hb = static_cast<char*>(pin.p);
   double* hs = reinterpret_cast<double*>(hb + (slots_.as<char>() - rb_base));
   double* hem = hs + (em_slot(0) - slots_.d());
```

New measurement: 130.5 (median of 5 runs). No clear change (+0.8%).
